# jorgeMFS/HYMET

Hardware: AMD Instinct MI355X
Metric: contigs/s + Mbp/s classified, CAMI-medium, 1/2/4/8 MI355X; % HBM roofline (higher is better)
Workload: dtype u64

## Files before the change

hymet_amd/_lib.py:

```python
from __future__ import annotations

import ctypes
import os

HERE = os.path.dirname(os.path.abspath(__file__))
LIB_PATH = os.path.join(HERE, "libhymet_gpu.so")

_c = ctypes
_i64, _u64, _i32, _u32, _vp = _c.c_int64, _c.c_uint64, _c.c_int, _c.c_uint32, _c.c_void_p

_SIGS = {
    "hymet_version": (_i32, []),
    "hymet_init": (_i32, [_i32, _c.POINTER(_vp)]),
    "hymet_destroy": (_i32, [_vp]),
    "hymet_last_error": (_c.c_char_p, []),
    "hymet_set_stream": (_i32, [_vp, _vp]),
    "hymet_sync": (_i32, [_vp]),
    "hymet_prof_enable": (_i32, [_vp, _i32]),
    "hymet_prof_reset": (_i32, [_vp]),
    "hymet_prof_query": (_i32, [_vp, _c.c_char_p, _c.POINTER(_c.c_double), _c.POINTER(_i64), _c.POINTER(_c.c_double)]),
    "hymet_prof_names": (_i32, [_vp, _c.c_char_p, _i64]),
    "hymet_scratch_trim": (_i32, [_vp, _c.POINTER(_i64)]),
    "hymet_scratch_cached": (_i32, [_vp, _c.POINTER(_i64)]),
    "hymet_scratch_stats": (_i32, [_vp, _vp]),
    "hymet_scratch_reserve": (_i32, [_vp, _i64]),
    "hymet_set_oom_hook": (_i32, [_vp, _vp]),
    "hymet_copy_to_host": (_i32, [_vp, _vp, _vp, _i64, _i32]),
    "hymet_copy_to_device": (_i32, [_vp, _vp, _vp, _i64, _i32]),
    "hymet_pack": (_i32, [_vp, _vp, _i64, _i32, _vp, _vp]),
    "hymet_fasta_index": (_i32, [_vp, _i64, _i32, _i64, _c.POINTER(_i64), _vp, _vp, _vp, _vp, _vp]),
    "hymet_fasta_names": (_i32, [_vp, _vp, _vp, _i64, _vp, _vp]),
    "hymet_fasta_compact": (_i32, [_vp, _vp, _i64, _i64, _vp, _vp, _vp, _i64, _vp, _i64, _vp]),
    "hymet_name_hash": (_i32, [_vp, _vp, _vp, _vp, _i64, _vp]),
    "hymet_sort_pairs_u64": (_i32, [_vp, _vp, _vp, _i64, _i32, _i32]),
    "hymet_scan_u32": (_i32, [_vp, _vp, _vp, _i64, _i32, _vp]),
    "hymet_msh_open": (_i32, [_c.c_char_p, _c.POINTER(_vp)]),
    "hymet_msh_info_get": (_i32, [_vp, _vp]),
    "hymet_msh_copy": (_i32, [_vp, _i32, _vp, _vp, _vp, _vp, _vp, _vp]),
    "hymet_msh_upload": (_i32, [_vp, _vp, _i32, _vp, _vp, _i32]),
    "hymet_msh_upload_range": (_i32, [_vp, _vp, _i32, _vp, _vp, _i32, _i64, _i64]),
    "hymet_msh_text_offsets": (_i32, [_vp, _vp, _vp]),
    "hymet_msh_close": (None, [_vp]),
    "hymet_screen_table_slots": (_i64, [_i64]),
    "hymet_screen_table_build": (_i32, [_vp, _vp, _i64, _vp, _i64, _vp, _vp, _i32]),
    "hymet_screen_count": (_i32, [_vp, _vp, _vp, _i64, _i64, _i64, _i32, _u32, _i32, _c.POINTER(_vp), _c.POINTER(_i64),
                                  _c.POINTER(_vp), _c.POINTER(_i64), _c.POINTER(_vp), _u64, _vp, _i64, _vp, _vp]),
    "hymet_screen_stats": (_i32, [_vp, _vp, _i64, _vp, _vp, _vp, _vp]),
    "hymet_screen_winner": (_i32, [_vp, _vp, _i64, _vp, _vp, _i64, _vp, _i64, _vp, _vp, _vp]),
    "hymet_sketch_max_size": (_i64, []),
    "hymet_sketch_batch": (_i32, [_vp, _vp, _vp, _i64, _i32, _u32, _i32, _i64, _vp, _vp, _vp, _i32, _vp, _vp]),
    "hymet_mash_dist": (_i32, [_vp, _vp, _i64, _vp, _i64, _vp, _i64, _vp, _i64, _i64, _i64, _i32, _vp]),
    "hymet_mash_dist_tile": (_i32, [_i32]),
    "hymet_mash_dist_tune": (_i32, [_i32, _i32]),
    "hymet_mash_dist_select": (_i32, [_vp, _vp, _i64, _i64, _vp, _i32, _vp, _vp, _vp, _i64, _c.POINTER(_i64)]),
    "hymet_mash_dist_tri": (_i32, [_vp, _vp, _i64, _vp, _i64, _i64, _i64, _i32, _vp]),
    "hymet_mash_link": (_i32, [_vp, _vp, _i64, _i64, _i64, _vp, _i32, _vp, _vp]),
    "hymet_mash_labels": (_i32, [_vp, _vp, _i64, _vp]),
    "hymet_mash_dist_sparse": (_i32, [_vp, _vp, _i64, _vp, _i64, _vp, _i64, _vp, _i64, _i64, _i64, _i32, _i32, _vp, _i32,
                                      _i64, _vp, _vp, _vp, _i64, _c.POINTER(_i64), _vp]),
    "hymet_mash_link_edges": (_i32, [_vp, _vp, _i64, _i64, _vp, _vp, _vp]),
    "hymet_mm_sketch": (_i32, [_vp, _vp, _vp, _vp, _vp, _i32, _i32, _i32, _i32, _vp, _vp, _i64, _c.POINTER(_i64)]),
    "hymet_mm_index_build": (_i32, [_vp, _vp, _vp, _vp, _vp, _i32, _i32, _i32, _c.POINTER(_vp)]),
    "hymet_mm_index_destroy": (_i32, [_vp]),
    "hymet_mm_index_info": (_i32, [_vp, _c.POINTER(_i32), _c.POINTER(_i32), _c.POINTER(_i32), _c.POINTER(_i64)]),
    "hymet_mm_index_max_occ": (_i32, [_vp, _vp, _c.c_float, _c.POINTER(_i32)]),
    "hymet_mm_index_save": (_i32, [_vp, _vp, _c.c_char_p, _i32, _c.POINTER(_i64)]),
    "hymet_mm_index_load": (_i32, [_vp, _c.c_char_p, _i64, _c.POINTER(_vp), _c.POINTER(_i64)]),
    "hymet_mm_index_export": (_i32, [_vp, _vp, _vp, _vp]),
    "hymet_mm_map": (_i32, [_vp, _vp, _vp, _vp, _vp, _vp, _vp, _vp, _i32, _c.POINTER(_vp)]),
    "hymet_mm_result_size": (_i32, [_vp, _c.POINTER(_i64)]),
    "hymet_mm_result_copy": (_i32, [_vp, _vp, _vp, _vp]),
    "hymet_mm_result_destroy": (_i32, [_vp]),
    "hymet_paf_acc_create": (_i32, [_vp, _c.POINTER(_vp)]),
    "hymet_paf_acc_reset": (_i32, [_vp]),
    "hymet_paf_acc_destroy": (_i32, [_vp]),
    "hymet_paf_acc_info": (_i32, [_vp, _c.POINTER(_i64), _c.POINTER(_vp), _c.POINTER(_vp), _c.POINTER(_vp),
                                  _c.POINTER(_vp), _c.POINTER(_vp)]),
    "hymet_paf_acc_append": (_i32, [_vp, _vp, _vp, _i64, _i64]),
    "hymet_paf_acc_copy": (_i32, [_vp, _vp, _vp, _vp, _vp]),
    "hymet_paf_acc_field": (_i32, [_vp, _vp, _i32, _vp]),
    "hymet_mm_map_acc": (_i32, [_vp, _vp, _vp, _vp, _vp, _vp, _vp, _vp, _i32, _i32, _i32, _i32, _vp]),
    "hymet_emit_paf": (_i32, [_vp, _vp, _vp, _vp, _vp, _vp, _vp, _vp, _vp, _i64, _c.POINTER(_i64), _vp]),
    "hymet_acc_ref_counts": (_i32, [_vp, _vp, _vp]),
    "hymet_acc_classify": (_i32, [_vp, _vp, _i32, _i32] + [_vp] * 15 + [_c.POINTER(_i32)]),
    "hymet_emit_tsv": (_i32, [_vp, _i32, _i32] + [_vp] * 14 + [_i64, _c.POINTER(_i64)]),
    "hymet_mm_chain_dp": (_i32, [_vp, _vp, _vp, _i64, _i32, _i32, _i32, _i32, _i32, _c.c_float, _c.c_float, _vp, _vp]),
    "hymet_mm_mark_compact": (_i32, [_vp, _vp, _vp, _vp, _i64, _vp, _vp, _i32, _vp, _vp, _vp, _c.POINTER(_i64)]),
    "hymet_mm_stamp_scratch": (_i32, [_vp, _c.POINTER(_i64), _c.POINTER(_i64)]),
    "hymet_mm_anchor_sort": (_i32, [_vp, _vp, _vp, _i64, _vp, _i32, _i32, _i32, _u64, _i64, _vp, _vp, _vp, _vp, _vp]),
    "hymet_lca_ref_counts": (_i32, [_vp, _vp, _i64, _vp]),
    "hymet_lca": (_i32, [_vp, _i32, _i32] + [_vp] * 17),
}

class SparseCounters(_c.Structure):
    _fields_ = [("postings", _i64), ("emitted", _i64), ("candidates", _i64)]


_lib = None
_oom_hook = None


def _release_torch_cache(_user):
    try:
        import torch
        torch.cuda.empty_cache()
    except Exception:
        pass


class HymetError(RuntimeError):
    pass


def load():
    global _lib
    if _lib is not None:
        return _lib
    path = os.environ.get("HYMET_LIB", LIB_PATH)
    if not os.path.exists(path):
        raise HymetError(f"{path} not found: build the HIP extension (python -m hymet_amd.build); "
                         "hymet_amd has no CPU fallback")
    lib = ctypes.CDLL(path)
    for name, (res, args) in _SIGS.items():
        fn = getattr(lib, name)
        fn.restype = res
        fn.argtypes = args
    global _oom_hook
    _oom_hook = _c.CFUNCTYPE(None, _vp)(_release_torch_cache)
    lib.hymet_set_oom_hook(_c.cast(_oom_hook, _vp), None)
    _lib = lib
    return lib


def exported_symbols():
    return list(_SIGS)


def check(rc: int, what: str):
    if rc != 0:
        msg = load().hymet_last_error()
        raise HymetError(f"{what} failed ({rc}): {msg.decode() if msg else ''}")


class Gpu:

    def __init__(self, device: int = 0, stream=None):
        import torch

        if not torch.cuda.is_available():
            raise HymetError("no GPU visible: hymet_amd runs on MI355X (gfx950) only")
        self.torch = torch
        self.device = device
        torch.cuda.set_device(device)
        self.dev = torch.device("cuda", device)
        self.lib = load()
        h = _vp()
        check(self.lib.hymet_init(device, _c.byref(h)), "hymet_init")
        self.ctx = h
        self.stream = stream
        self.children = []
        self.bind_stream(stream)

    def fork(self) -> "Gpu":
        child = Gpu(self.device, stream=self.torch.cuda.Stream(device=self.device))
        self.children.append(child)
        return child

    def bind_stream(self, stream=None):
        s = stream if stream is not None else self.torch.cuda.current_stream(self.device)
        check(self.lib.hymet_set_stream(self.ctx, _vp(s.cuda_stream)), "hymet_set_stream")
        self.bound_stream = s

    def call(self, name, *args):
        check(getattr(self.lib, name)(self.ctx, *args), name)

    def sync(self):
        check(self.lib.hymet_sync(self.ctx), "hymet_sync")
        for ch in self.children:
            ch.sync()

    def prof(self, on: bool = True):
        check(self.lib.hymet_prof_enable(self.ctx, int(on)), "hymet_prof_enable")
        for ch in self.children:
            ch.prof(on)

    def prof_reset(self):
        check(self.lib.hymet_prof_reset(self.ctx), "hymet_prof_reset")
        for ch in self.children:
            ch.prof_reset()

    def prof_table(self):
        buf = _c.create_string_buffer(1 << 16)
        check(self.lib.hymet_prof_names(self.ctx, buf, 1 << 16), "hymet_prof_names")
        out = {}
        for name in buf.value.decode().split():
            ms, n, b = _c.c_double(), _i64(), _c.c_double()
            check(self.lib.hymet_prof_query(self.ctx, name.encode(), _c.byref(ms), _c.byref(n), _c.byref(b)), "hymet_prof_query")
            out[name] = (ms.value, n.value, b.value)
        for ch in self.children:
            for name, (ms, n, b) in ch.prof_table().items():
                m0, n0, b0 = out.get(name, (0.0, 0, 0.0))
                out[name] = (m0 + ms, n0 + n, b0 + b)
        return out

    def trim(self) -> int:
        out = _i64()
        check(self.lib.hymet_scratch_trim(self.ctx, _c.byref(out)), "hymet_scratch_trim")
        return out.value

    def reserve(self, nbytes: int):
        check(self.lib.hymet_scratch_reserve(self.ctx, int(nbytes)), "hymet_scratch_reserve")

    def _alloc(self, fn, n, dtype):
        try:
            return fn(int(n), dtype=dtype, device=self.dev)
        except self.torch.OutOfMemoryError:
            if self.trim() == 0:
                raise
            return fn(int(n), dtype=dtype, device=self.dev)

    def empty(self, n, dtype):
        return self._alloc(self.torch.empty, n, dtype)

    def zeros(self, n, dtype):
        return self._alloc(self.torch.zeros, n, dtype)

    def close(self):
        if self.ctx:
            self.lib.hymet_destroy(self.ctx)
            self.ctx = None

    def __del__(self):
        try:
            self.close()
        except Exception:
            pass


def ptr(t) -> _vp:
    return _vp(t.data_ptr())
```

hymet_amd/csrc/mm_map.hip:

```cpp
#include "mm_stages.hpp"

#include <algorithm>
#include <atomic>
#include <type_traits>
#include <utility>

#include <chrono>
#include <cstdio>
#include <cstdlib>
#include <cstring>

struct hymet_mm_result {
    int n_q = 0;
    std::vector<int64_t> reg_off;
    std::vector<int32_t> rep_len;
    std::vector<hymet_mm_reg> regs;
};

namespace hymet {
namespace mm {

int launch_regions(hymet_ctx *ctx, const uint64_t *ax, const uint32_t *ay, int span, const int32_t *ids, const int64_t *cfirst,
                   const uint64_t *cu, const int64_t *cboff,
                   const int64_t *qc, const int64_t *qb, const uint64_t *mini_pos, const int64_t *mp_off, const int64_t *qlen,
                   const uint32_t *name_hash, const int32_t *rep_len, const int64_t *ref_len, int n_q, const hymet_mm_opt *o,
                   int k, void *z, hymet_mm_reg *regs, int32_t *w, uint64_t *cov, int32_t *tmp, int32_t *n_regs,
                   int64_t NB, int64_t NC, int64_t NM, const uint32_t *cq,
                   const MiniWord *mtab, const int64_t *qbase, const uint32_t *skip_q, uint64_t *sumk, bool sumk_done);

namespace {

__global__ void fill_qid_kernel(const int64_t *off, int n_q, int64_t n, uint32_t *qid, uint32_t *ones, int32_t *zq) {
    const int64_t i = (int64_t)blockIdx.x * blockDim.x + threadIdx.x;
    if (i < n) {
        qid[i] = (uint32_t)upper_idx(off, n_q, i);
        if (ones) ones[i] = 1u;
    }
    if (zq && i < n_q) zq[i] = 0;
}

__global__ void flagged_len_kernel(const uint32_t *flag, const int64_t *qb, int n_q, uint32_t *cnt, int64_t *any) {
    const int q = blockIdx.x * blockDim.x + threadIdx.x;
    if (q > n_q) return;
    if (q == n_q) {
        cnt[q] = 0;
        return;
    }
    const bool f = flag[q] != 0;
    cnt[q] = f ? (uint32_t)(qb[q + 1] - qb[q]) : 0u;
    if (f) *any = 1;
}


__global__ void mzflt_runs_kernel(const uint32_t *sq, const uint64_t *sx, const uint32_t *sidx, const int64_t *qm_off,
                                  int64_t n, int q_occ_max, float q_occ_frac, uint32_t *keep) {
    const int64_t p = (int64_t)blockIdx.x * blockDim.x + threadIdx.x;
    if (p >= n) return;
    if (p > 0 && sq[p] == sq[p - 1] && sx[p] == sx[p - 1]) return;
    int64_t e = p + 1;
    while (e < n && sq[e] == sq[p] && sx[e] == sx[p]) e++;
    const uint32_t q = sq[p];
    const int64_t nq = qm_off[q + 1] - qm_off[q];
    if (nq <= q_occ_max) return;
    const int32_t cnt = (int32_t)(e - p);
    if (cnt > q_occ_max && (float)cnt > (float)nq * q_occ_frac)
        for (int64_t j = p; j < e; j++) keep[sidx[j]] = 0;
}

constexpr int kMzBuckets = 4096;
__global__ __launch_bounds__(256) void mzflt_screen_kernel(const uint64_t *mx, const int64_t *qm_off, int n_q, int q_occ_max,
                                                           uint32_t *keep, uint32_t *cnt, int64_t *any) {
    __shared__ uint32_t h[kMzBuckets];
    __shared__ int hit;
    const int q = blockIdx.x;
    if (q == n_q) {
        if (threadIdx.x == 0) cnt[q] = 0;
        return;
    }
    const int64_t s = qm_off[q], nq = qm_off[q + 1] - s;
    for (int64_t e = threadIdx.x; e < nq; e += 256) keep[s + e] = 1u;
    if (nq <= q_occ_max) {
        if (threadIdx.x == 0) cnt[q] = 0;
        return;
    }
    for (int b = threadIdx.x; b < kMzBuckets; b += 256) h[b] = 0;
    if (threadIdx.x == 0) hit = 0;
    __syncthreads();
    bool over = false;
    for (int64_t e = threadIdx.x; e < nq; e += 256)
        over |= atomicAdd(&h[(uint32_t)(mx[s + e] >> 8) & (kMzBuckets - 1)], 1u) >= (uint32_t)q_occ_max;
    if (over) hit = 1;
    __syncthreads();
    if (threadIdx.x == 0) {
        cnt[q] = hit ? (uint32_t)nq : 0u;
        if (hit) *any = 1;
    }
}

__global__ __launch_bounds__(256) void mzflt_list_kernel(const int64_t *qm_off, const uint32_t *cnt, const int64_t *coff,
                                                         uint32_t *gidx, uint32_t *sq) {
    const int q = blockIdx.x;
    const uint32_t nq = cnt[q];
    if (nq == 0) return;
    const int64_t s = qm_off[q], d = coff[q];
    for (uint32_t e = threadIdx.x; e < nq; e += 256) {
        gidx[d + e] = (uint32_t)(s + e);
        sq[d + e] = (uint32_t)q;
    }
}

__global__ void mzflt_gather_kernel(const uint32_t *perm, const uint32_t *gidx, const uint64_t *mx, uint32_t *gout,
                                    uint64_t *xout, int64_t n) {
    const int64_t i = (int64_t)blockIdx.x * blockDim.x + threadIdx.x;
    if (i >= n) return;
    const uint32_t g = gidx[perm[i]];
    gout[i] = g;
    xout[i] = mx[g];
}

__global__ void compact_mz_kernel(const uint64_t *x, const uint64_t *y, const uint32_t *keep, int64_t *pos, int64_t n,
                                  uint64_t *ox, uint64_t *oy) {
    const int64_t i = (int64_t)blockIdx.x * blockDim.x + threadIdx.x;
    if (i == n - 1) pos[n] = pos[i] + keep[i];
    if (i < n && keep[i]) {
        ox[pos[i]] = x[i];
        oy[pos[i]] = y[i];
    }
}

__global__ void sample_off_kernel(const int64_t *pos, const int64_t *qm_off, int n_q, int64_t total, int64_t *out) {
    const int q = blockIdx.x * blockDim.x + threadIdx.x;
    if (q > n_q) return;
    out[q] = q == n_q ? total : pos[qm_off[q]];
}

__global__ void seed_count_kernel(const uint64_t *mx, int64_t n, const uint32_t *koff, int64_t n_buckets,
                                  uint32_t *seed_n) {
    const int64_t i = (int64_t)blockIdx.x * blockDim.x + threadIdx.x;
    if (i >= n) return;
    const uint64_t h = mx[i] >> 8;
    uint32_t c = 0;
    if ((int64_t)h < n_buckets) c = koff[h + 1] - koff[h];
    seed_n[i] = c;
}

constexpr uint32_t kFlt = 0x80000000u;

__global__ void seed_class_kernel(const uint32_t *seed_n, int64_t M, int max_occ, uint64_t *cls) {
    const int64_t i = (int64_t)blockIdx.x * blockDim.x + threadIdx.x;
    if (i > M) return;
    if (i == M) {
        cls[M] = 0;
        return;
    }
    const uint32_t n = seed_n[i];
    const bool hi = (int)n > max_occ, lo = n > 0 && !hi;
    cls[i] = (uint64_t)(hi ? 1u : 0u) << 32 | (lo ? 1u : 0u);
}

__global__ void seed_list_kernel(const uint32_t *seed_n, const uint64_t *rank, int64_t M, int max_occ, int32_t *low_idx,
                                 int32_t *high_idx) {
    const int64_t i = (int64_t)blockIdx.x * blockDim.x + threadIdx.x;
    if (i >= M) return;
    const uint32_t n = seed_n[i];
    if (!n) return;
    if ((int)n > max_occ) high_idx[rank[i] >> 32] = (int32_t)i;
    else low_idx[(uint32_t)rank[i]] = (int32_t)i;
}

struct StreakParams {
    const uint64_t *my;
    const uint32_t *qid;
    const int64_t *qm_off, *qlen;
    const uint64_t *rank;
    const int32_t *low_idx, *high_idx;
    int64_t n_low;
    int n_q;
    int max_occ, max_max_occ, dist;
    uint32_t *seed_n;
    uint32_t *flt_high;
};

__global__ void streak_kernel(StreakParams P) {
    const int64_t t = (int64_t)blockIdx.x * blockDim.x + threadIdx.x;
    if (t >= P.n_low + P.n_q) return;
    int q;
    int64_t e_idx = -1, p_idx = -1;
    uint64_t re, rp;
    if (t < P.n_low) {
        e_idx = P.low_idx[t];
        q = (int)P.qid[e_idx];
        re = P.rank[e_idx];
        if (t > 0 && P.qid[P.low_idx[t - 1]] == (uint32_t)q) p_idx = P.low_idx[t - 1];
    } else {
        q = (int)(t - P.n_low);
        re = P.rank[P.qm_off[q + 1]];
        const uint64_t r0 = P.rank[P.qm_off[q]];
        if ((uint32_t)re > (uint32_t)r0) p_idx = P.low_idx[(uint32_t)re - 1];
    }
    rp = p_idx >= 0 ? P.rank[p_idx] : P.rank[P.qm_off[q]];
    const int64_t h0 = (int64_t)(rp >> 32), h1 = (int64_t)(re >> 32);
    const int cnt = (int)(h1 - h0);
    if (cnt <= 0) return;
    const bool case_a = P.dist > 0 && P.max_max_occ > P.max_occ;
    bool keep_all = false, keep_none = false;
    uint64_t thr = 0;
    if (case_a) {
        const uint64_t rq0 = P.rank[P.qm_off[q]], rq1 = P.rank[P.qm_off[q + 1]];
        const int64_t n_seed = (int64_t)((uint32_t)rq1 - (uint32_t)rq0) + (int64_t)((rq1 >> 32) - (rq0 >> 32));
        if (n_seed <= 1) return;
        const int32_t ps = p_idx >= 0 ? (int32_t)((uint32_t)P.my[p_idx] >> 1) : 0;
        const int32_t pe = e_idx >= 0 ? (int32_t)((uint32_t)P.my[e_idx] >> 1) : (int32_t)P.qlen[q];
        int32_t mh = (int32_t)((double)(pe - ps) / P.dist + .499);
        if (mh > 128) mh = 128;
        keep_all = mh >= cnt, keep_none = mh <= 0;
        if (!keep_all && !keep_none) {
            uint64_t lo = 0, hi = ~0ull;
            while (lo < hi) {
                const uint64_t mid = lo + (hi - lo) / 2;
                int c = 0;
                for (int64_t r = h0; r < h1; r++) {
                    const int32_t a = P.high_idx[r];
                    c += ((uint64_t)P.seed_n[a] << 32 | (uint32_t)a) <= mid;
                }
                if (c >= mh) hi = mid;
                else lo = mid + 1;
            }
            thr = lo;
        }
    }
    for (int64_t r = h0; r < h1; r++) {
        const int32_t a = P.high_idx[r];
        const uint32_t n = P.seed_n[a];
        bool flt = true;
        if (case_a) {
            const bool chosen = keep_all || (!keep_none && ((uint64_t)n << 32 | (uint32_t)a) <= thr);
            flt = !chosen || (int)n > P.max_max_occ;
        }
        P.flt_high[r] = flt ? 1u : 0u;
    }
}

__global__ void flt_mark_kernel(const uint32_t *flt_high, int64_t n_high, int32_t *v) {
    const int64_t r = (int64_t)blockIdx.x * blockDim.x + threadIdx.x;
    if (r < n_high) v[r] = flt_high[r] ? (int32_t)r : -1;
}

__global__ void rep_len_kernel(const uint32_t *flt_high, const int32_t *prev_max, const int32_t *high_idx, int64_t n_high,
                               const uint64_t *mx, const uint64_t *my, const uint32_t *qid, int32_t *rep_len,
                               uint32_t *seed_n) {
    const int64_t r = (int64_t)blockIdx.x * blockDim.x + threadIdx.x;
    if (r >= n_high || !flt_high[r]) return;
    const int32_t a = high_idx[r];
    const uint32_t q = qid[a];
    const int32_t en = (int32_t)((uint32_t)my[a] >> 1) + 1, st = en - (int32_t)(mx[a] & 0xff);
    int32_t en_prev = 0;
    const int32_t pr = r > 0 ? prev_max[r - 1] : -1;
    if (pr >= 0) {
        const int32_t b = high_idx[pr];
        if (qid[b] == q) en_prev = (int32_t)((uint32_t)my[b] >> 1) + 1;
    }
    atomicAdd(rep_len + q, en - max(st, en_prev));
    seed_n[a] = 0;
}

__global__ void nz_flag_kernel(const uint32_t *v, int64_t n, uint32_t *flag) {
    const int64_t i = (int64_t)blockIdx.x * blockDim.x + threadIdx.x;
    if (i < n) flag[i] = v[i] ? 1u : 0u;
}

struct AnchorParams {
    const uint64_t *mx, *my;
    const uint32_t *seed_n;
    const int64_t *a_pos;
    const uint32_t *qid;
    const int64_t *qlen;
    const uint32_t *koff;
    const uint64_t *ipos;
    int64_t n;
    int rb;
    uint64_t *ax, *k1, *k2;
    uint32_t *ay;
    uint32_t *val;
    const int64_t *mp_pos;
    uint64_t *mini_pos;
};

__global__ void write_anchors_kernel(AnchorParams P) {
    const int64_t i = (int64_t)blockIdx.x * blockDim.x + threadIdx.x;
    if (i >= P.n) return;
    const uint32_t n = P.seed_n[i];
    if (!n) return;
    const uint64_t mx = P.mx[i], my = P.my[i];
    const uint32_t q_pos = (uint32_t)my, q_span = (uint32_t)(mx & 0xff);
    P.mini_pos[P.mp_pos[i]] = (uint64_t)q_span << 32 | (q_pos >> 1);
    const uint32_t q = P.qid[i];
    const int32_t qlen = (int32_t)P.qlen[q];
    const uint32_t *kp = P.koff + (mx >> 8);
    const uint64_t *r = P.ipos + kp[0];
    int64_t a = P.a_pos[i];
    for (uint32_t k = 0; k < n; k++, a++) {
        const uint64_t rk = r[k];
        const uint32_t rpos = (uint32_t)rk >> 1;
        const uint32_t rid = (uint32_t)(rk >> 32);
        uint64_t x, y;
        uint32_t rev;
        if ((rk & 1) == (q_pos & 1)) {
            rev = 0;
            x = (rk & 0xffffffff00000000ULL) | rpos;
            y = (uint64_t)q_span << 32 | (q_pos >> 1);
        } else {
            rev = 1;
            x = 1ULL << 63 | (rk & 0xffffffff00000000ULL) | rpos;
            y = (uint64_t)q_span << 32 | (uint32_t)(qlen - (int32_t)((q_pos >> 1) + 1 - q_span) - 1);
        }
        P.ax[a] = x;
        P.ay[a] = (uint32_t)y;
        P.k1[a] = (uint64_t)q << (1 + P.rb) | (uint64_t)rev << P.rb | rid;
        P.k2[a] = (uint64_t)rpos << 32 | (uint32_t)y;
        P.val[a] = (uint32_t)a;
    }
}

struct AnchorKeyParams {
    const uint64_t *mx, *my;
    const uint32_t *seed_n;
    const int64_t *a_pos;
    const uint32_t *qid;
    const int64_t *qlen;
    const uint32_t *koff;
    const uint64_t *ipos;
    int64_t n;
    int rb, pb;
    int ybits;
    uint64_t *key;
    const int64_t *mp_pos;
    uint64_t *mini_pos;
};

__global__ __launch_bounds__(256) void write_anchor_keys_kernel(AnchorKeyParams P) {
    __shared__ int64_t s_a[257];
    __shared__ uint64_t s_r[256];
    __shared__ uint32_t s_yf[256], s_yr[256], s_strand[256];
    const int tid = threadIdx.x;
    const int64_t m0 = (int64_t)blockIdx.x * 256;
    const int cnt = (int)min((int64_t)256, P.n - m0);
    if (tid < cnt) {
        const int64_t i = m0 + tid;
        const uint32_t n = P.seed_n[i];
        const uint64_t mx = P.mx[i], my = P.my[i];
        const uint32_t q_pos = (uint32_t)my, q_span = (uint32_t)(mx & 0xff);
        const uint32_t q = P.qid[i];
        if (n) P.mini_pos[P.mp_pos[i]] = (uint64_t)q_span << 32 | (q_pos >> 1);
        s_a[tid] = P.a_pos[i];
        s_r[tid] = P.koff[mx >> 8];
        s_yf[tid] = q_pos >> 1;
        s_yr[tid] = (uint32_t)((int32_t)P.qlen[q] - (int32_t)((q_pos >> 1) + 1 - q_span) - 1);
        s_strand[tid] = q_pos & 1;
    }
    if (tid == 0) s_a[cnt] = P.a_pos[m0 + cnt];
    __syncthreads();
    const int64_t a0 = s_a[0], a1 = s_a[cnt];
    const int sh_rev = P.rb + P.pb;
    for (int64_t a = a0 + tid; a < a1; a += 256) {
        int lo = 0, hi = cnt - 1;
        while (lo < hi) {
            const int mid = (lo + hi + 1) >> 1;
            if (s_a[mid] <= a) lo = mid;
            else hi = mid - 1;
        }
        const uint64_t rk = P.ipos[s_r[lo] + (a - s_a[lo])];
        const uint32_t rpos = (uint32_t)rk >> 1;
        const uint64_t rid = rk >> 32;
        const uint32_t rev = ((uint32_t)rk & 1) != s_strand[lo];
        const uint64_t k = (uint64_t)rev << sh_rev | rid << P.pb | rpos;
        const uint32_t y = rev ? s_yr[lo] : s_yf[lo];
        P.key[a] = k << P.ybits | y;
    }
}

__global__ __launch_bounds__(256) void mini_bits_kernel(const uint64_t *my, const uint32_t *seed_n, const uint32_t *qid,
                                                        const int64_t *qbase, int64_t M, MiniWord *tab) {
    const int64_t i = (int64_t)blockIdx.x * blockDim.x + threadIdx.x;
    const int lane = threadIdx.x & 63;
    const bool on = i < M && seed_n[i];
    const int64_t b = on ? qbase[qid[i]] + ((uint32_t)my[i] >> 1) : -64 * (int64_t)(lane + 1);
    const int64_t w = b >> 6;
    uint64_t bits = on ? 1ull << (b & 63) : 0;
#pragma unroll
    for (int d = 1; d < 64; d <<= 1) {
        const int64_t wo = __shfl_down(w, d, 64);
        const uint64_t bo = __shfl_down(bits, d, 64);
        if (lane + d < 64 && wo == w) bits |= bo;
    }
    const int64_t wp = __shfl_up(w, 1, 64);
    if (on && (lane == 0 || wp != w)) atomicOr((unsigned long long *)&tab[w].bits, bits);
}
__global__ void mini_base_kernel(const uint64_t *my, const uint32_t *seed_n, const uint32_t *qid, const int64_t *qm_off,
                                 const int64_t *mp_pos, const int64_t *qbase, int64_t M, MiniWord *tab) {
    const int64_t i = (int64_t)blockIdx.x * blockDim.x + threadIdx.x;
    if (i >= M || !seed_n[i]) return;
    const uint32_t q = qid[i];
    const int64_t b = qbase[q] + ((uint32_t)my[i] >> 1);
    const uint64_t bits = tab[b >> 6].bits;
    tab[b >> 6].base = (uint32_t)(mp_pos[i] - mp_pos[qm_off[q]]) - (uint32_t)__popcll(bits & ((1ull << (b & 63)) - 1));
}

__global__ void reg_count_kernel(const uint32_t *flag, const int32_t *n1, const int32_t *n2, int n_q, uint32_t *cnt) {
    const int q = blockIdx.x * blockDim.x + threadIdx.x;
    if (q < n_q) cnt[q] = (uint32_t)((flag && flag[q]) ? n2[q] : n1[q]);
}

struct RegOut {
    hymet_mm_reg *regs;
    int32_t *q, *part, *rl, *t;
    int32_t q_base, part_id, t_base;
};
__global__ void reg_gather_kernel(const uint32_t *flag, const int32_t *n1, const int32_t *n2, const int64_t *qc1,
                                  const int64_t *qc2, const hymet_mm_reg *r1, const hymet_mm_reg *r2, const int64_t *off,
                                  const int32_t *rep_len, int n_q, RegOut o) {
    const int q = blockIdx.x * blockDim.x + threadIdx.x;
    if (q >= n_q) return;
    const bool use2 = flag && flag[q];
    const hymet_mm_reg *src = use2 ? r2 + qc2[q] : r1 + qc1[q];
    const int nr = use2 ? n2[q] : n1[q];
    const int64_t d = off[q];
    for (int i = 0; i < nr; i++) {
        const hymet_mm_reg r = src[i];
        o.regs[d + i] = r;
        if (o.q) {
            o.q[d + i] = o.q_base + q;
            o.part[d + i] = o.part_id;
            o.rl[d + i] = rep_len[q];
            o.t[d + i] = o.t_base + r.rid;
        }
    }
}
}
}
}

using namespace hymet;
using namespace hymet::mm;

struct CallTrace {
    bool on = env_flag("HYMET_TRACE");
    std::chrono::steady_clock::time_point t = std::chrono::steady_clock::now();
    ~CallTrace() {
        if (on)
            fprintf(stderr, "[hymet_mm_map] %-22s %9.2f ms\n", "TOTAL (with frees)",
                    std::chrono::duration<double, std::milli>(std::chrono::steady_clock::now() - t).count());
    }
};
struct PhaseTrace {
    hymet_ctx *ctx;
    bool on;
    std::chrono::steady_clock::time_point t;
    explicit PhaseTrace(hymet_ctx *c) : ctx(c), on(env_flag("HYMET_TRACE")), t(std::chrono::steady_clock::now()) {}
    void mark(const char *what) {
        if (!on) return;
        (void)hipStreamSynchronize(ctx->stream);
        const auto n = std::chrono::steady_clock::now();
        fprintf(stderr, "[hymet_mm_map] %-22s %9.2f ms\n", what, std::chrono::duration<double, std::milli>(n - t).count());
        t = n;
    }
};

static int sort_anchor_set(hymet_ctx *ctx, DevBuf &x, DevBuf &y, DevBuf &k1, DevBuf &k2, DevBuf &val, int64_t n,
                           int key1_bits, int yhi, AnchorSet &out) {
    DevBuf k2b, valb, k1g, k1b;
    HY_HIP(k2b.alloc(8 * (size_t)n, ctx->stream));
    HY_HIP(valb.alloc(4 * (size_t)n, ctx->stream));
    uint64_t *kk = k2.as<uint64_t>(), *kka = k2b.as<uint64_t>();
    uint32_t *vv = val.as<uint32_t>(), *vva = valb.as<uint32_t>();
    int rc = sort_pairs(ctx, kk, kka, vv, vva, n, 0, 64, "radix_sort_anchor_pos");
    if (rc) return rc;
    HY_HIP(k1g.alloc(8 * (size_t)n, ctx->stream));
    HY_HIP(k1b.alloc(8 * (size_t)n, ctx->stream));
    LAUNCH1(gather_kernel<uint64_t>, n, k1.as<uint64_t>(), vv, k1g.as<uint64_t>(), n);
    uint64_t *k1p = k1g.as<uint64_t>(), *k1a = k1b.as<uint64_t>();
    rc = sort_pairs(ctx, k1p, k1a, vv, vva, n, 0, key1_bits, "radix_sort_anchor_group");
    if (rc) return rc;
    HY_HIP(out.ax.alloc(8 * (size_t)n, ctx->stream));
    HY_HIP(out.ay.alloc(4 * (size_t)n, ctx->stream));
    LAUNCH1(gather_kernel<uint64_t>, n, x.as<uint64_t>(), vv, out.ax.as<uint64_t>(), n);
    LAUNCH1(gather_kernel<uint32_t>, n, y.as<uint32_t>(), vv, out.ay.as<uint32_t>(), n);
    out.n = n;
    out.span = yhi & 0xff;
    return HYMET_OK;
}

static int sort_anchor_words(hymet_ctx *ctx, DevBuf &word, int64_t n, int rb, int pb, int yhi, const int64_t *d_qoff, int n_q,
                             int64_t max_qlen, AnchorSet &out) {
    DevBuf wb;
    HY_HIP(wb.alloc(8 * (size_t)n, ctx->stream));
    HY_HIP(out.ax.alloc(8 * (size_t)n, ctx->stream));
    HY_HIP(out.ay.alloc(4 * (size_t)n, ctx->stream));
    HY_HIP(out.hb.alloc(head_bits_bytes(n), ctx->stream));
    HY_HIP(out.ax32.alloc(4 * (size_t)n, ctx->stream));
    out.n = n;
    out.span = yhi & 0xff;
    const bool log_stats = env_flag("HYMET_ASORT_STATS");
    DevBuf sstat;
    if (log_stats) {
        HY_HIP(sstat.alloc(32, ctx->stream));
        HY_HIP(hipMemsetAsync(sstat.p, 0, 32, ctx->stream));
    }
    const int rc = grouped_anchor_sort(ctx, word.as<uint64_t>(), n, d_qoff, n_q, rb, pb, max_qlen,
                                       wb.as<uint64_t>(), out.ax.as<uint64_t>(), out.ay.as<uint32_t>(),
                                       out.hb.as<uint32_t>(), out.ax32.as<uint32_t>(),
                                       log_stats ? sstat.as<unsigned long long>() : nullptr);
    if (rc == 1) return hymet::fail(HYMET_E_INTERNAL, "sort_anchor_words: anchor words emitted for a layout without one");
    if (rc) return rc;
    if (log_stats) {
        unsigned long long h[4] = {};
        HY_HIP(hipMemcpyAsync(h, sstat.p, 32, hipMemcpyDeviceToHost, ctx->stream));
        HY_HIP(hipStreamSynchronize(ctx->stream));
        fprintf(stderr, "[asort] anchors %lld fast_segs %llu fast_anchors %llu full_segs %llu full_anchors %llu\n",
                (long long)n, h[0], h[1], h[2], h[3]);
    }
    out.has_hb = out.has_x32 = true;
    return HYMET_OK;
}

static int dump_anchors(hymet_ctx *ctx, const char *var, const AnchorSet &S, int n_q, std::atomic<bool> &dumped) {
    const char *path = env_str(var);
    if (!path || S.n == 0 || dumped.exchange(true)) return HYMET_OK;
    hipStream_t st = ctx->stream;
    const int64_t nd = std::min<int64_t>(S.n, env_int("HYMET_DUMP_MAX", 1 << 24, 0, INT64_MAX));
    std::vector<uint64_t> hx(nd);
    std::vector<uint32_t> hy(nd);
    std::vector<int64_t> qo(n_q + 1);
    HY_HIP(hipMemcpyAsync(hx.data(), S.ax.p, 8 * (size_t)nd, hipMemcpyDeviceToHost, st));
    HY_HIP(hipMemcpyAsync(hy.data(), S.ay.p, 4 * (size_t)nd, hipMemcpyDeviceToHost, st));
    HY_HIP(hipMemcpyAsync(qo.data(), S.d_off.p, 8 * (size_t)(n_q + 1), hipMemcpyDeviceToHost, st));
    HY_HIP(hipStreamSynchronize(st));
    if (FILE *fp = fopen(path, "wb")) {
        uint64_t gid = 0;
        int q = 0;
        std::vector<uint64_t> buf;
        buf.reserve(1 << 21);
        for (int64_t a = 0; a < nd; a++) {
            bool qs = false;
            while (q < n_q && qo[q + 1] <= a) q++, qs = true;
            if (a && (qs || (hx[a] >> 32) != (hx[a - 1] >> 32))) gid++;
            buf.push_back(gid << 32 | (uint32_t)hx[a]);
            buf.push_back((uint64_t)S.span << 32 | hy[a]);
            if (buf.size() >= (1u << 21)) fwrite(buf.data(), 8, buf.size(), fp), buf.clear();
        }
        fwrite(buf.data(), 8, buf.size(), fp);
        fclose(fp);
    }
    return HYMET_OK;
}

struct MapSink {
    hymet_mm_result *res = nullptr;
    hymet_paf_acc *acc = nullptr;
    int32_t q_base = 0, part_id = 0, t_base = 0;
};

static int acc_reserve(hymet_ctx *ctx, hymet_paf_acc *a, int64_t need) {
    if (need <= a->cap) return HYMET_OK;
    const int64_t cap = std::max<int64_t>(need, std::max<int64_t>(a->cap * 3 / 2, 1 << 16));
    hipStream_t st = ctx->stream;
    DevBuf nregs, nq, npart, nrl, nt;
    HY_HIP(nregs.alloc(sizeof(hymet_mm_reg) * (size_t)cap, st));
    HY_HIP(nq.alloc(4 * (size_t)cap, st));
    HY_HIP(npart.alloc(4 * (size_t)cap, st));
    HY_HIP(nrl.alloc(4 * (size_t)cap, st));
    HY_HIP(nt.alloc(4 * (size_t)cap, st));
    if (a->n) {
        HY_HIP(hipMemcpyAsync(nregs.p, a->regs.p, sizeof(hymet_mm_reg) * (size_t)a->n, hipMemcpyDeviceToDevice, st));
        HY_HIP(hipMemcpyAsync(nq.p, a->q.p, 4 * (size_t)a->n, hipMemcpyDeviceToDevice, st));
        HY_HIP(hipMemcpyAsync(npart.p, a->part.p, 4 * (size_t)a->n, hipMemcpyDeviceToDevice, st));
        HY_HIP(hipMemcpyAsync(nrl.p, a->rl.p, 4 * (size_t)a->n, hipMemcpyDeviceToDevice, st));
        HY_HIP(hipMemcpyAsync(nt.p, a->t.p, 4 * (size_t)a->n, hipMemcpyDeviceToDevice, st));
    }
    a->regs.swap(nregs);
    a->q.swap(nq);
    a->part.swap(npart);
    a->rl.swap(nrl);
    a->t.swap(nt);
    a->cap = cap;
    return HYMET_OK;
}

struct MapBatch {
    hymet_ctx *ctx;
    const hymet_mm_index *idx;
    const hymet_mm_opt *opt;
    const int64_t *h_lens;
    int32_t n_q;
    DevBuf mx, my, qm_off;
    int64_t M = 0;
    DevBuf d_qlen, d_hash_buf;
    const uint32_t *d_hash = nullptr;
    DevBuf seed_n, rep_len, qid;
    DevBuf mini_pos, mp_off;
    int64_t NM = 0;
    DevBuf d_qbase, pos_tab;
    std::vector<int64_t> qbase;
    int64_t max_qlen = 1;
};

static int sketch_queries(MapBatch &B, const uint32_t *d_2b, const uint32_t *d_mask, const int64_t *h_starts,
                          const uint32_t *h_name_hash, const uint32_t *d_name_hash) {
    hipStream_t st = B.ctx->stream;
    const int n_q = B.n_q;
    int rc = sketch_sequences(B.ctx, d_2b, d_mask, h_starts, B.h_lens, n_q, B.idx->w, B.idx->k, 0, B.mx, B.my, &B.M, &B.qm_off);
    if (rc) return rc;
    HY_HIP(B.d_qlen.alloc(8 * (size_t)n_q, st));
    HY_HIP(hipMemcpyAsync(B.d_qlen.p, B.h_lens, 8 * (size_t)n_q, hipMemcpyHostToDevice, st));
    B.d_hash = d_name_hash;
    if (!B.d_hash) {
        HY_HIP(B.d_hash_buf.alloc(4 * (size_t)n_q, st));
        HY_HIP(hipMemcpyAsync(B.d_hash_buf.p, h_name_hash, 4 * (size_t)n_q, hipMemcpyHostToDevice, st));
        B.d_hash = B.d_hash_buf.as<uint32_t>();
    }
    return HYMET_OK;
}

static int filter_minimizers(MapBatch &B) {
    hymet_ctx *ctx = B.ctx;
    hipStream_t st = ctx->stream;
    const hymet_mm_opt *opt = B.opt;
    const int n_q = B.n_q;
    const int64_t M = B.M;
    DevBuf &mx = B.mx, &my = B.my, &qm_off = B.qm_off;
    DevBuf keep, fcnt, fcoff;
    int64_t MF = 0;
    int rc;
    if (opt->q_occ_frac > 0.0f && M > 0 && opt->mid_occ > 0) {
        HY_HIP(keep.alloc(4 * (size_t)M, st));
        HY_HIP(fcnt.alloc(4 * (size_t)(n_q + 1), st));
        ctx->mbox_h[kMbFlag] = 0;
        hipLaunchKernelGGL(mzflt_screen_kernel, dim3((unsigned)n_q + 1), dim3(256), 0, st, mx.as<uint64_t>(), qm_off.as<int64_t>(),
                           n_q, opt->mid_occ, keep.as<uint32_t>(), fcnt.as<uint32_t>(), mb_dev(ctx, kMbFlag));
        HY_CHECK_LAUNCH("mzflt_screen_kernel");
        HY_HIP(hipStreamSynchronize(st));
        if (mb_read(ctx, kMbFlag) != 0) {
            HY_HIP(fcoff.alloc(8 * (size_t)(n_q + 1), st));
            rc = exclusive_scan_u32_i64(ctx, fcnt.as<uint32_t>(), fcoff.as<int64_t>(), n_q + 1, &MF);
            if (rc) return rc;
        }
    }
    if (MF == 0) return HYMET_OK;
    DevBuf gidx, sx, sx2, sidx, sidx2, sq0, sq, sq2, kpos, nx, ny, gx, gg;
    HY_HIP(gidx.alloc(4 * (size_t)MF, st));
    HY_HIP(sq0.alloc(4 * (size_t)MF, st));
    hipLaunchKernelGGL(mzflt_list_kernel, dim3((unsigned)n_q), dim3(256), 0, st, qm_off.as<int64_t>(), fcnt.as<uint32_t>(),
                       fcoff.as<int64_t>(), gidx.as<uint32_t>(), sq0.as<uint32_t>());
    HY_CHECK_LAUNCH("mzflt_list_kernel");
    HY_HIP(sx.alloc(8 * (size_t)MF, st));
    HY_HIP(sx2.alloc(8 * (size_t)MF, st));
    HY_HIP(sidx.alloc(4 * (size_t)MF, st));
    HY_HIP(sidx2.alloc(4 * (size_t)MF, st));
    LAUNCH1(gather_kernel<uint64_t>, MF, mx.as<uint64_t>(), gidx.as<uint32_t>(), sx.as<uint64_t>(), MF);
    LAUNCH1(iota_u32_kernel, MF, sidx.as<uint32_t>(), MF);
    uint64_t *kx = sx.as<uint64_t>(), *kxa = sx2.as<uint64_t>();
    uint32_t *vi = sidx.as<uint32_t>(), *via = sidx2.as<uint32_t>();
    rc = sort_pairs(ctx, kx, kxa, vi, via, MF, 0, 2 * B.idx->k + 8, "radix_sort_mz");
    if (rc) return rc;
    HY_HIP(sq.alloc(4 * (size_t)MF, st));
    HY_HIP(sq2.alloc(4 * (size_t)MF, st));
    LAUNCH1(gather_kernel<uint32_t>, MF, sq0.as<uint32_t>(), vi, sq.as<uint32_t>(), MF);
    uint32_t *kq = sq.as<uint32_t>(), *kqa = sq2.as<uint32_t>();
    rc = sort_pairs(ctx, kq, kqa, vi, via, MF, 0, bits_for(n_q), "radix_sort_mz");
    if (rc) return rc;
    HY_HIP(gx.alloc(8 * (size_t)MF, st));
    HY_HIP(gg.alloc(4 * (size_t)MF, st));
    LAUNCH1(mzflt_gather_kernel, MF, vi, gidx.as<uint32_t>(), mx.as<uint64_t>(), gg.as<uint32_t>(), gx.as<uint64_t>(), MF);
    LAUNCH1(mzflt_runs_kernel, MF, kq, gx.as<uint64_t>(), gg.as<uint32_t>(), qm_off.as<int64_t>(), MF, opt->mid_occ,
            opt->q_occ_frac, keep.as<uint32_t>());
    int64_t M2 = 0;
    rc = scan_flags(ctx, keep.as<uint32_t>(), M, kpos, &M2);
    if (rc) return rc;
    HY_HIP(nx.alloc(8 * (size_t)(M2 + 1), st));
    HY_HIP(ny.alloc(8 * (size_t)(M2 + 1), st));
    LAUNCH1(compact_mz_kernel, M, mx.as<uint64_t>(), my.as<uint64_t>(), keep.as<uint32_t>(), kpos.as<int64_t>(), M,
            nx.as<uint64_t>(), ny.as<uint64_t>());
    DevBuf nqm;
    HY_HIP(nqm.alloc(8 * (size_t)(n_q + 1), st));
    hipLaunchKernelGGL(sample_off_kernel, dim3((unsigned)cdiv(n_q + 1, 256)), dim3(256), 0, st, kpos.as<int64_t>(),
                       qm_off.as<int64_t>(), n_q, M2, nqm.as<int64_t>());
    HY_CHECK_LAUNCH("sample_off_kernel");
    mx.swap(nx);
    my.swap(ny);
    qm_off.swap(nqm);
    B.M = M2;
    return HYMET_OK;
}

static int select_seeds(MapBatch &B) {
    hymet_ctx *ctx = B.ctx;
    hipStream_t st = ctx->stream;
    const hymet_mm_opt *opt = B.opt;
    const int n_q = B.n_q;
    const int64_t M = B.M;
    DevBuf &mx = B.mx, &my = B.my, &qm_off = B.qm_off, &seed_n = B.seed_n, &rep_len = B.rep_len, &qid = B.qid;
    HY_HIP(seed_n.alloc(4 * (size_t)(M + 1), st));
    HY_HIP(rep_len.alloc(4 * (size_t)n_q, st));
    HY_HIP(qid.alloc(4 * (size_t)(M + 1), st));
    LAUNCH1(fill_qid_kernel, std::max<int64_t>(M, n_q), qm_off.as<int64_t>(), n_q, M, qid.as<uint32_t>(), nullptr,
            rep_len.as<int32_t>());
    {
        ProfScope _ps(ctx, "mm_seed_count", (double)M * (8.0 + 8.0 + 4.0));
        LAUNCH1(seed_count_kernel, M, mx.as<uint64_t>(), M, B.idx->d_koff, B.idx->n_buckets, seed_n.as<uint32_t>());
    }
    if (M == 0) return HYMET_OK;
    ProfScope _ps(ctx, "mm_seed_select", (double)M * (4.0 + 8.0 + 8.0 + 8.0));
    DevBuf cls, rank, spart;
    HY_HIP(cls.alloc(8 * (size_t)(M + 1), st));
    HY_HIP(rank.alloc(8 * (size_t)(M + 1), st));
    LAUNCH1(seed_class_kernel, M + 1, seed_n.as<uint32_t>(), M, opt->mid_occ, cls.as<uint64_t>());
    int rc = scan_u64(ctx, cls.as<uint64_t>(), rank.as<uint64_t>(), M + 1, spart, mb_dev(ctx, kMbScan));
    if (rc) return rc;
    HY_HIP(hipStreamSynchronize(st));
    const uint64_t tot = (uint64_t)mb_read(ctx, kMbScan);
    const int64_t n_low = (uint32_t)tot, n_high = (int64_t)(tot >> 32);
    if (n_high == 0) return HYMET_OK;
    DevBuf low_idx, high_idx, flt_high, vmax, pmax;
    HY_HIP(low_idx.alloc(4 * (size_t)(n_low + 1), st));
    HY_HIP(high_idx.alloc(4 * (size_t)n_high, st));
    HY_HIP(flt_high.alloc(4 * (size_t)n_high, st));
    LAUNCH1(seed_list_kernel, M, seed_n.as<uint32_t>(), rank.as<uint64_t>(), M, opt->mid_occ, low_idx.as<int32_t>(),
            high_idx.as<int32_t>());
    StreakParams S{my.as<uint64_t>(), qid.as<uint32_t>(), qm_off.as<int64_t>(), B.d_qlen.as<int64_t>(),
                   rank.as<uint64_t>(), low_idx.as<int32_t>(), high_idx.as<int32_t>(), n_low, n_q, opt->mid_occ,
                   opt->max_max_occ, opt->occ_dist, seed_n.as<uint32_t>(), flt_high.as<uint32_t>()};
    HY_HIP(hipMemsetAsync(flt_high.p, 0, 4 * (size_t)n_high, st));
    LAUNCH1(streak_kernel, n_low + n_q, S);
    HY_HIP(vmax.alloc(4 * (size_t)n_high, st));
    HY_HIP(pmax.alloc(4 * (size_t)n_high, st));
    LAUNCH1(flt_mark_kernel, n_high, flt_high.as<uint32_t>(), n_high, vmax.as<int32_t>());
    {
        DevBuf mpart;
        rc = inclusive_max_scan_i32(ctx, vmax.as<int32_t>(), pmax.as<int32_t>(), n_high, mpart);
        if (rc) return rc;
    }
    LAUNCH1(rep_len_kernel, n_high, flt_high.as<uint32_t>(), pmax.as<int32_t>(), high_idx.as<int32_t>(), n_high,
            mx.as<uint64_t>(), my.as<uint64_t>(), qid.as<uint32_t>(), rep_len.as<int32_t>(), seed_n.as<uint32_t>());
    return HYMET_OK;
}

static int build_mini_table(MapBatch &B, const DevBuf &mp_pos) {
    hymet_ctx *ctx = B.ctx;
    hipStream_t st = ctx->stream;
    const int n_q = B.n_q;
    B.qbase.assign(n_q + 1, 0);
    for (int q = 0; q < n_q; q++) {
        B.qbase[q + 1] = B.qbase[q] + ((B.h_lens[q] + 63) & ~(int64_t)63);
        B.max_qlen = std::max<int64_t>(B.max_qlen, B.h_lens[q]);
    }
    HY_HIP(B.d_qbase.alloc(8 * (size_t)(n_q + 1), st));
    HY_HIP(hipMemcpyAsync(B.d_qbase.p, B.qbase.data(), 8 * (size_t)(n_q + 1), hipMemcpyHostToDevice, st));
    const size_t n_words = (size_t)(B.qbase[n_q] >> 6) + 1;
    HY_HIP(B.pos_tab.alloc(sizeof(MiniWord) * n_words, st));
    HY_HIP(hipMemsetAsync(B.pos_tab.p, 0, sizeof(MiniWord) * n_words, st));
    LAUNCH1(mini_bits_kernel, B.M, B.my.as<uint64_t>(), B.seed_n.as<uint32_t>(), B.qid.as<uint32_t>(), B.d_qbase.as<int64_t>(),
            B.M, B.pos_tab.as<MiniWord>());
    LAUNCH1(mini_base_kernel, B.M, B.my.as<uint64_t>(), B.seed_n.as<uint32_t>(), B.qid.as<uint32_t>(), B.qm_off.as<int64_t>(),
            mp_pos.as<int64_t>(), B.d_qbase.as<int64_t>(), B.M, B.pos_tab.as<MiniWord>());
    return HYMET_OK;
}

static int first_pass_anchors(MapBatch &B, AnchorSet &S1) {
    hymet_ctx *ctx = B.ctx;
    hipStream_t st = ctx->stream;
    const hymet_mm_index *idx = B.idx;
    const int n_q = B.n_q;
    const int64_t M = B.M;
    DevBuf &mx = B.mx, &my = B.my, &qm_off = B.qm_off, &seed_n = B.seed_n, &qid = B.qid, &d_qlen = B.d_qlen;
    DevBuf a_pos, mflag, mp_pos;
    int64_t A = 0;
    int rc = scan_flags(ctx, seed_n.as<uint32_t>(), M, a_pos, &A);
    if (rc) return rc;
    HY_ARG(A <= anchor_cap(), "hymet_mm_map: the batch has more anchors than 32-bit chain links hold (map fewer bases per batch)");
    HY_HIP(mflag.alloc(4 * (size_t)(M + 1), st));
    LAUNCH1(nz_flag_kernel, M, seed_n.as<uint32_t>(), M, mflag.as<uint32_t>());
    rc = scan_flags(ctx, mflag.as<uint32_t>(), M, mp_pos, &B.NM);
    if (rc) return rc;
    HY_HIP(hipMemcpyAsync(a_pos.as<int64_t>() + M, &A, 8, hipMemcpyHostToDevice, st));
    HY_HIP(hipMemcpyAsync(mp_pos.as<int64_t>() + M, &B.NM, 8, hipMemcpyHostToDevice, st));
    HY_HIP(B.mini_pos.alloc(8 * (size_t)(B.NM + 1), st));
    HY_HIP(B.mp_off.alloc(8 * (size_t)(n_q + 1), st));
    hipLaunchKernelGGL(sample_off_kernel, dim3((unsigned)cdiv(n_q + 1, 256)), dim3(256), 0, st, mp_pos.as<int64_t>(),
                       qm_off.as<int64_t>(), n_q, B.NM, B.mp_off.as<int64_t>());
    HY_CHECK_LAUNCH("sample_off_kernel");
    rc = build_mini_table(B, mp_pos);
    if (rc) return rc;
    HY_HIP(S1.d_off.alloc(8 * (size_t)(n_q + 1), st));
    hipLaunchKernelGGL(sample_off_kernel, dim3((unsigned)cdiv(n_q + 1, 256)), dim3(256), 0, st, a_pos.as<int64_t>(),
                       qm_off.as<int64_t>(), n_q, A, S1.d_off.as<int64_t>());
    HY_CHECK_LAUNCH("sample_off_kernel");
    const int rb = bits_for(idx->n_seq), key1_bits = bits_for(n_q) + 1 + rb;
    HY_ARG(key1_bits <= 64, "hymet_mm_map: too many queries x targets for the sort key");
    int64_t max_len = 1;
    for (int64_t l : idx->h_len) max_len = std::max(max_len, l);
    const int pb = bits_for(max_len - 1);
    if (A == 0) {
        S1.span = idx->k & 0xff;
        return HYMET_OK;
    }
    const int ybits = env_flag("HYMET_ANCHOR_LEGACY") ? 0 : anchor_word_ybits(rb, pb, B.max_qlen);
    if (ybits > 0) {
        DevBuf word;
        HY_HIP(word.alloc(8 * (size_t)(A + 1), st));
        AnchorKeyParams P{mx.as<uint64_t>(), my.as<uint64_t>(), seed_n.as<uint32_t>(), a_pos.as<int64_t>(),
                          qid.as<uint32_t>(), d_qlen.as<int64_t>(), idx->d_koff, idx->d_pos, M, rb, pb,
                          ybits, word.as<uint64_t>(), mp_pos.as<int64_t>(), B.mini_pos.as<uint64_t>()};
        {
            ProfScope _ps(ctx, "mm_anchors", (double)A * (8.0 + 12.0));
            hipLaunchKernelGGL(write_anchor_keys_kernel, dim3((unsigned)cdiv(M, 256)), dim3(256), 0, st, P);
            HY_CHECK_LAUNCH("write_anchor_keys_kernel");
        }
        return sort_anchor_words(ctx, word, A, rb, pb, idx->k, S1.d_off.as<int64_t>(), n_q, B.max_qlen, S1);
    }
    DevBuf x, y, k1, k2, val;
    HY_HIP(x.alloc(8 * (size_t)(A + 1), st));
    HY_HIP(y.alloc(4 * (size_t)(A + 1), st));
    HY_HIP(k1.alloc(8 * (size_t)(A + 1), st));
    HY_HIP(k2.alloc(8 * (size_t)(A + 1), st));
    HY_HIP(val.alloc(4 * (size_t)(A + 1), st));
    AnchorParams P{mx.as<uint64_t>(), my.as<uint64_t>(), seed_n.as<uint32_t>(), a_pos.as<int64_t>(), qid.as<uint32_t>(),
                   d_qlen.as<int64_t>(), idx->d_koff, idx->d_pos, M, rb, x.as<uint64_t>(), k1.as<uint64_t>(),
                   k2.as<uint64_t>(), y.as<uint32_t>(), val.as<uint32_t>(), mp_pos.as<int64_t>(), B.mini_pos.as<uint64_t>()};
    ProfScope _ps(ctx, "mm_anchors", (double)A * (8.0 + 36.0));
    LAUNCH1(write_anchors_kernel, M, P);
    return sort_anchor_set(ctx, x, y, k1, k2, val, A, key1_bits, idx->k, S1);
}

static int long_join_anchors(MapBatch &B, const AnchorSet &S1, const LeanJoin &lj, const DevBuf &flag, AnchorSet &S2,
                             bool &any) {
    hymet_ctx *ctx = B.ctx;
    const int n_q = B.n_q;
    DevBuf fcnt;
    HY_HIP(fcnt.alloc(4 * (size_t)(n_q + 1), ctx->stream));
    ctx->mbox_h[kMbFlag] = 0;
    LAUNCH1(flagged_len_kernel, n_q + 1, flag.as<uint32_t>(), lj.qb2.as<int64_t>(), n_q, fcnt.as<uint32_t>(),
            mb_dev(ctx, kMbFlag));
    int64_t A2 = 0;
    int rc = scan_flags(ctx, fcnt.as<uint32_t>(), n_q + 1, S2.d_off, &A2);
    if (rc) return rc;
    any = mb_read(ctx, kMbFlag) != 0;
    if (!any) return HYMET_OK;
    HY_ARG(A2 <= anchor_cap(), "hymet_mm_map: the long join has more anchors than 32-bit chain links hold");
    rc = marked_anchor_set(ctx, S1, lj, flag.as<uint32_t>(), n_q, A2, S2);
    if (rc) return rc;
    static std::atomic<bool> dumped{false};
    return dump_anchors(ctx, "HYMET_DUMP_ANCHORS2", S2, n_q, dumped);
}

static int run_regions(MapBatch &B, ChainSet &C, DevBuf &rg, DevBuf &nr, const uint32_t *skip_q, DevBuf &sumk, bool &sumk_done) {
    hipStream_t st = B.ctx->stream;
    const int64_t NC = C.n_chain;
    DevBuf z, wv, cov, tmp;
    HY_HIP(z.alloc(16 * (size_t)(NC + 1), st));
    HY_HIP(rg.alloc(sizeof(hymet_mm_reg) * (size_t)(NC + 1), st));
    HY_HIP(wv.alloc(4 * (size_t)(NC + 1), st));
    HY_HIP(cov.alloc(8 * (size_t)(NC + 1), st));
    HY_HIP(tmp.alloc(4 * (size_t)(NC + 1), st));
    HY_HIP(nr.alloc(4 * (size_t)B.n_q, st));
    return launch_regions(B.ctx, C.ax, C.ay, C.span, C.ids.as<int32_t>(), C.cfirst.as<int64_t>(), C.cu.as<uint64_t>(),
                          C.cboff.as<int64_t>(), C.d_qc.as<int64_t>(), C.d_qb.as<int64_t>(), B.mini_pos.as<uint64_t>(),
                          B.mp_off.as<int64_t>(), B.d_qlen.as<int64_t>(), B.d_hash, B.rep_len.as<int32_t>(), B.idx->d_len,
                          B.n_q, B.opt, B.idx->k, z.p, rg.as<hymet_mm_reg>(), wv.as<int32_t>(), cov.as<uint64_t>(),
                          tmp.as<int32_t>(), nr.as<int32_t>(), C.n_anchor, NC, B.NM, C.cq.as<uint32_t>(),
                          B.pos_tab.as<MiniWord>(), B.d_qbase.as<int64_t>(), skip_q, sumk.as<uint64_t>(),
                          std::exchange(sumk_done, true));
}

struct RegSet {
    const int32_t *n;
    const int64_t *qc;
    const hymet_mm_reg *r;
};

static int emit_records(MapBatch &B, const uint32_t *fl, const RegSet &s1, const RegSet &s2, MapSink &sink) {
    hymet_ctx *ctx = B.ctx;
    hipStream_t st = ctx->stream;
    const int n_q = B.n_q;
    hymet_mm_result *res = sink.res;
    DevBuf cnt, off;
    HY_HIP(cnt.alloc(4 * (size_t)(n_q + 1), st));
    LAUNCH1(reg_count_kernel, n_q, fl, s1.n, s2.n, n_q, cnt.as<uint32_t>());
    int64_t N = 0;
    int rc = scan_flags(ctx, cnt.as<uint32_t>(), n_q, off, &N);
    if (rc) return rc;
    HY_HIP(hipMemcpyAsync(off.as<int64_t>() + n_q, &N, 8, hipMemcpyHostToDevice, st));
    RegOut o{};
    DevBuf tmp_regs;
    if (sink.acc) {
        hymet_paf_acc *a = sink.acc;
        rc = acc_reserve(ctx, a, a->n + N);
        if (rc) return rc;
        o = RegOut{a->regs.as<hymet_mm_reg>() + a->n, a->q.as<int32_t>() + a->n, a->part.as<int32_t>() + a->n,
                   a->rl.as<int32_t>() + a->n, a->t.as<int32_t>() + a->n, sink.q_base, sink.part_id, sink.t_base};
    } else {
        HY_HIP(tmp_regs.alloc(sizeof(hymet_mm_reg) * (size_t)(N + 1), st));
        o.regs = tmp_regs.as<hymet_mm_reg>();
    }
    {
        ProfScope _ps(ctx, "mm_paf_records", (double)N * (2.0 * sizeof(hymet_mm_reg) + 16.0));
        LAUNCH1(reg_gather_kernel, n_q, fl, s1.n, s2.n, s1.qc, s2.qc, s1.r, s2.r, off.as<int64_t>(), B.rep_len.as<int32_t>(),
                n_q, o);
    }
    if (sink.acc) {
        sink.acc->n += N;
    } else {
        res->regs.resize(N);
        if (N) HY_HIP(hipMemcpyAsync(res->regs.data(), tmp_regs.p, sizeof(hymet_mm_reg) * (size_t)N, hipMemcpyDeviceToHost, st));
        HY_HIP(hipMemcpyAsync(res->reg_off.data(), off.p, 8 * (size_t)(n_q + 1), hipMemcpyDeviceToHost, st));
        HY_HIP(hipMemcpyAsync(res->rep_len.data(), B.rep_len.p, 4 * (size_t)n_q, hipMemcpyDeviceToHost, st));
    }
    HY_HIP(hipStreamSynchronize(st));
    return HYMET_OK;
}

static int mm_map_impl(hymet_ctx *ctx, const hymet_mm_index *idx, const hymet_mm_opt *opt, const uint32_t *d_2b,
                       const uint32_t *d_mask, const int64_t *h_starts, const int64_t *h_lens, const uint32_t *h_name_hash,
                       const uint32_t *d_name_hash, int32_t n_q, MapSink &sink) {
    CallTrace call_trace;
    HY_ARG(ctx && idx && opt && d_2b && d_mask, "hymet_mm_map: null argument");
    HY_ARG(n_q >= 0, "hymet_mm_map: n_q < 0");
    HY_ARG(h_name_hash || d_name_hash, "hymet_mm_map: no query name hashes");
    HY_ARG(opt->mid_occ > 0, "hymet_mm_map: opt->mid_occ must be resolved (hymet_mm_index_max_occ + clamps)");
    HY_HIP(hipSetDevice(ctx->device));
    if (sink.res) {
        sink.res->n_q = n_q;
        sink.res->reg_off.assign(n_q + 1, 0);
        sink.res->rep_len.assign(n_q, 0);
    }
    if (n_q == 0) return HYMET_OK;
    const float pen_gap = (float)(opt->chain_gap_scale * 0.01 * idx->k);
    const float pen_skip = (float)(opt->chain_skip_scale * 0.01 * idx->k);
    PhaseTrace tr(ctx);
    MapBatch B{ctx, idx, opt, h_lens, n_q};
    int rc = sketch_queries(B, d_2b, d_mask, h_starts, h_name_hash, d_name_hash);
    if (rc) return rc;
    tr.mark("sketch");
    rc = filter_minimizers(B);
    if (rc) return rc;
    tr.mark("mz_flt");
    rc = select_seeds(B);
    if (rc) return rc;
    tr.mark("seeds");
    AnchorSet S1;
    rc = first_pass_anchors(B, S1);
    if (rc) return rc;
    tr.mark("anchors+sort");
    static std::atomic<bool> dumped1{false};
    rc = dump_anchors(ctx, "HYMET_DUMP_ANCHORS", S1, n_q, dumped1);
    if (rc) return rc;
    ChainSet C1;
    const bool long_join = opt->bw_long > opt->bw;
    LeanJoin lj{B.d_qlen.as<int64_t>(), opt->rmq_rescue_size, opt->rmq_rescue_ratio};
    rc = chain_set(ctx, opt, pen_gap, pen_skip, opt->bw, S1, n_q, C1, long_join ? &lj : nullptr);
    if (rc) return rc;
    tr.mark("chain_set 1");
    ChainSet C2;
    AnchorSet S2;
    DevBuf flag;
    bool joined = false;
    if (long_join && C1.n_chain > 0) {
        flag.swap(lj.flag);
        rc = long_join_anchors(B, S1, lj, flag, S2, joined);
        if (rc) return rc;
        if (joined) {
            rc = chain_set(ctx, opt, pen_gap, pen_skip, opt->bw_long, S2, n_q, C2);
            if (rc) return rc;
        }
    }
    tr.mark("long join");
    DevBuf sumk, rg1, nr1, rg2, nr2;
    HY_HIP(sumk.alloc(8 * (size_t)(n_q + 1), ctx->stream));
    bool sumk_done = false;
    const uint32_t *fl = joined ? flag.as<uint32_t>() : nullptr;
    rc = run_regions(B, C1, rg1, nr1, fl, sumk, sumk_done);
    if (rc) return rc;
    if (joined) {
        rc = run_regions(B, C2, rg2, nr2, nullptr, sumk, sumk_done);
        if (rc) return rc;
    }
    const RegSet r1{nr1.as<int32_t>(), C1.d_qc.as<int64_t>(), rg1.as<hymet_mm_reg>()};
    const RegSet r2{nr2.as<int32_t>(), C2.d_qc.as<int64_t>(), rg2.as<hymet_mm_reg>()};
    rc = emit_records(B, fl, r1, joined ? r2 : r1, sink);
    if (rc) return rc;
    tr.mark("regions");
    return HYMET_OK;
}

extern "C" {

int hymet_mm_map(hymet_ctx *ctx, const hymet_mm_index *idx, const hymet_mm_opt *opt, const uint32_t *d_2b,
                 const uint32_t *d_mask, const int64_t *h_starts, const int64_t *h_lens, const uint32_t *h_name_hash,
                 int32_t n_q, hymet_mm_result **out) {
    HY_ARG(out != nullptr, "hymet_mm_map: null argument");
    MapSink sink;
    sink.res = new hymet_mm_result();
    *out = sink.res;
    return mm_map_impl(ctx, idx, opt, d_2b, d_mask, h_starts, h_lens, h_name_hash, nullptr, n_q, sink);
}

int hymet_paf_acc_create(hymet_ctx *ctx, hymet_paf_acc **out) {
    HY_ARG(ctx && out, "hymet_paf_acc_create: null argument");
    hymet_paf_acc *a = new hymet_paf_acc();
    a->device = ctx->device;
    *out = a;
    return HYMET_OK;
}

int hymet_paf_acc_reset(hymet_paf_acc *acc) {
    HY_ARG(acc, "hymet_paf_acc_reset: null argument");
    acc->n = 0;
    return HYMET_OK;
}

int hymet_paf_acc_destroy(hymet_paf_acc *acc) {
    if (acc) {
        (void)hipSetDevice(acc->device);
        delete acc;
    }
    return HYMET_OK;
}

int hymet_paf_acc_info(const hymet_paf_acc *acc, int64_t *n_lines, void **d_regs, void **d_q, void **d_part, void **d_rl,
                       void **d_t) {
    HY_ARG(acc && n_lines, "hymet_paf_acc_info: null argument");
    *n_lines = acc->n;
    if (d_regs) *d_regs = acc->regs.p;
    if (d_q) *d_q = acc->q.p;
    if (d_part) *d_part = acc->part.p;
    if (d_rl) *d_rl = acc->rl.p;
    if (d_t) *d_t = acc->t.p;
    return HYMET_OK;
}

int hymet_paf_acc_append(hymet_ctx *ctx, hymet_paf_acc *dst, const hymet_paf_acc *src, int64_t begin, int64_t end) {
    HY_ARG(ctx && dst && src && dst != src, "hymet_paf_acc_append: null or aliased argument");
    HY_ARG(begin >= 0 && end >= begin && end <= src->n, "hymet_paf_acc_append: line range outside the source");
    const int64_t m = end - begin;
    if (m == 0) return HYMET_OK;
    HY_HIP(hipSetDevice(ctx->device));
    int rc = acc_reserve(ctx, dst, dst->n + m);
    if (rc) return rc;
    hipStream_t st = ctx->stream;
    const int64_t d = dst->n;
    HY_HIP(hipMemcpyAsync(dst->regs.as<hymet_mm_reg>() + d, src->regs.as<hymet_mm_reg>() + begin, sizeof(hymet_mm_reg) * (size_t)m,
                          hipMemcpyDeviceToDevice, st));
    HY_HIP(hipMemcpyAsync(dst->q.as<int32_t>() + d, src->q.as<int32_t>() + begin, 4 * (size_t)m, hipMemcpyDeviceToDevice, st));
    HY_HIP(hipMemcpyAsync(dst->part.as<int32_t>() + d, src->part.as<int32_t>() + begin, 4 * (size_t)m, hipMemcpyDeviceToDevice,
                          st));
    HY_HIP(hipMemcpyAsync(dst->rl.as<int32_t>() + d, src->rl.as<int32_t>() + begin, 4 * (size_t)m, hipMemcpyDeviceToDevice, st));
    HY_HIP(hipMemcpyAsync(dst->t.as<int32_t>() + d, src->t.as<int32_t>() + begin, 4 * (size_t)m, hipMemcpyDeviceToDevice, st));
    dst->n += m;
    return HYMET_OK;
}

int hymet_paf_acc_copy(hymet_ctx *ctx, const hymet_paf_acc *acc, int32_t *h_q, int32_t *h_part, int32_t *h_t) {
    HY_ARG(ctx && acc, "hymet_paf_acc_copy: null argument");
    if (acc->n <= 0) return HYMET_OK;
    HY_HIP(hipSetDevice(ctx->device));
    hipStream_t st = ctx->stream;
    if (h_q) HY_HIP(hipMemcpyAsync(h_q, acc->q.p, 4 * (size_t)acc->n, hipMemcpyDeviceToHost, st));
    if (h_part) HY_HIP(hipMemcpyAsync(h_part, acc->part.p, 4 * (size_t)acc->n, hipMemcpyDeviceToHost, st));
    if (h_t) HY_HIP(hipMemcpyAsync(h_t, acc->t.p, 4 * (size_t)acc->n, hipMemcpyDeviceToHost, st));
    HY_HIP(hipStreamSynchronize(st));
    return HYMET_OK;
}

int hymet_paf_acc_field(hymet_ctx *ctx, const hymet_paf_acc *acc, int field, int32_t *h_out) {
    HY_ARG(ctx && acc && h_out && field >= 0 && field < (int)(sizeof(hymet_mm_reg) / 4), "hymet_paf_acc_field: bad argument");
    if (acc->n <= 0) return HYMET_OK;
    HY_HIP(hipSetDevice(ctx->device));
    const char *src = static_cast<const char *>(acc->regs.p) + 4 * (size_t)field;
    HY_HIP(hipMemcpy2DAsync(h_out, 4, src, sizeof(hymet_mm_reg), 4, (size_t)acc->n, hipMemcpyDeviceToHost, ctx->stream));
    HY_HIP(hipStreamSynchronize(ctx->stream));
    return HYMET_OK;
}

int hymet_mm_map_acc(hymet_ctx *ctx, const hymet_mm_index *idx, const hymet_mm_opt *opt, const uint32_t *d_2b,
                     const uint32_t *d_mask, const int64_t *h_starts, const int64_t *h_lens, const uint32_t *d_name_hash,
                     int32_t n_q, int32_t q_base, int32_t part_id, int32_t t_base, hymet_paf_acc *acc) {
    HY_ARG(acc && d_name_hash, "hymet_mm_map_acc: null argument");
    MapSink sink;
    sink.acc = acc;
    sink.q_base = q_base;
    sink.part_id = part_id;
    sink.t_base = t_base;
    return mm_map_impl(ctx, idx, opt, d_2b, d_mask, h_starts, h_lens, nullptr, d_name_hash, n_q, sink);
}

int hymet_mm_result_size(const hymet_mm_result *res, int64_t *n_regs) {
    HY_ARG(res && n_regs, "hymet_mm_result_size: null argument");
    *n_regs = (int64_t)res->regs.size();
    return HYMET_OK;
}

int hymet_mm_result_copy(const hymet_mm_result *res, int64_t *h_off, int32_t *h_rep_len, hymet_mm_reg *h_regs) {
    HY_ARG(res, "hymet_mm_result_copy: null result");
    if (h_off) memcpy(h_off, res->reg_off.data(), 8 * (size_t)(res->n_q + 1));
    if (h_rep_len && res->n_q) memcpy(h_rep_len, res->rep_len.data(), 4 * (size_t)res->n_q);
    if (h_regs && !res->regs.empty()) memcpy(h_regs, res->regs.data(), sizeof(hymet_mm_reg) * res->regs.size());
    return HYMET_OK;
}

int hymet_mm_result_destroy(hymet_mm_result *res) {
    delete res;
    return HYMET_OK;
}

}
```

hymet_amd/csrc/mm_regs.hip:

```cpp
#include "mm_common.hpp"

#include <cstdio>
#include <cstdlib>

namespace hymet {
namespace mm {
namespace {

__device__ __forceinline__ uint32_t wang32(uint32_t key) {
    key += ~(key << 15);
    key ^= (key >> 10);
    key += (key << 3);
    key ^= (key >> 6);
    key += ~(key << 11);
    key ^= (key >> 16);
    return key;
}

struct U128 {
    uint64_t x, y;
};
__device__ __forceinline__ bool lt128(const U128 &a, const U128 &b) { return a.x < b.x || (a.x == b.x && a.y < b.y); }

template <typename T, typename Less>
__device__ void heap_sort(T *a, int64_t n, Less less) {
    auto sift = [&](int64_t i, int64_t m) {
        for (;;) {
            int64_t l = 2 * i + 1, r = l + 1, b = i;
            if (l < m && less(a[b], a[l])) b = l;
            if (r < m && less(a[b], a[r])) b = r;
            if (b == i) return;
            T t = a[b];
            a[b] = a[i];
            a[i] = t;
            i = b;
        }
    };
    for (int64_t i = n / 2 - 1; i >= 0; --i) sift(i, n);
    for (int64_t e = n - 1; e > 0; --e) {
        T t = a[0];
        a[0] = a[e];
        a[e] = t;
        sift(0, e);
    }
}

struct RegParams {
    const uint64_t *ax;
    const uint32_t *ay;
    int span;
    const int32_t *ids;
    const int64_t *cfirst;
    const uint64_t *cu;
    const int64_t *cboff;
    const int64_t *qc;
    const int64_t *qb;
    const uint64_t *mini_pos;
    const int64_t *mp_off;
    const int64_t *qlen;
    const uint32_t *name_hash;
    const int32_t *rep_len;
    const int64_t *ref_len;
    int n_q;
    int seed, k;
    float mask_level, pri_ratio;
    int mask_len, best_n, max_gap, min_chain_score;
    U128 *z;
    hymet_mm_reg *regs;
    int32_t *w;
    uint64_t *cov;
    int32_t *tmp;
    int32_t *n_regs;
    const int32_t *c_mlen, *c_blen, *c_st, *c_last, *c_fv;
    const uint64_t *q_sumk;
    const uint32_t *skip_q;
    int wave_min;
    int lds_max;
    unsigned long long *prof;
    int prim_regs;
};

__device__ void set_coor(hymet_mm_reg *r, int32_t qlen, uint64_t x0, uint32_t y0, uint64_t x1, uint32_t y1, int32_t q_span,
                         int32_t mlen, int32_t blen) {
    r->rev = (int32_t)(x0 >> 63);
    r->rid = (int32_t)(x0 << 1 >> 33);
    r->rs = (int32_t)x0 + 1 > q_span ? (int32_t)x0 + 1 - q_span : 0;
    r->re = (int32_t)x1 + 1;
    if (!r->rev) {
        r->qs = (int32_t)y0 + 1 - q_span;
        r->qe = (int32_t)y1 + 1;
    } else {
        r->qs = qlen - ((int32_t)y1 + 1);
        r->qe = qlen - ((int32_t)y0 + 1 - q_span);
    }
    r->mlen = mlen;
    r->blen = blen;
}

struct AnchorStatParams {
    const uint64_t *ax, *cu;
    const uint32_t *ay;
    int span;
    const int32_t *ids;
    const int64_t *cfirst;
    const int64_t *cboff, *qb, *qlen, *mp_off;
    const uint64_t *mini_pos;
    int64_t NB, NC;
    int n_q;
    const uint32_t *cq;
    int32_t *c_mlen, *c_blen, *c_st, *c_last;
    const MiniWord *mtab;
    const int64_t *qbase;
    const uint32_t *skip_q;
};

__device__ __forceinline__ int32_t mini_idx_at(const AnchorStatParams &P, int64_t q, int qlen, uint64_t ax, uint32_t ay) {
    int32_t x = (int32_t)ay;
    if (ax >> 63) x = qlen - 1 - (int32_t)ay + P.span - 1;
    return (x >= 0 && x < qlen) ? mini_word_idx(P.mtab[(P.qbase[q] + x) >> 6], x) : -1;
}

#ifndef HYMET_STAT_ITEMS
#define HYMET_STAT_ITEMS 2
#endif
constexpr int kStatItems = HYMET_STAT_ITEMS;
constexpr int kStatSpan = 256 * kStatItems;

__global__ void block_chain_kernel(const int64_t *cboff, int64_t NC, int64_t NB, int32_t *blk_c0) {
    const int64_t c = (int64_t)blockIdx.x * blockDim.x + threadIdx.x;
    if (c >= NC) return;
    const int64_t s = cboff[c], e = c + 1 < NC ? cboff[c + 1] : NB;
    for (int64_t b = (s + kStatSpan - 1) / kStatSpan; b * kStatSpan < e; ++b) blk_c0[b] = (int32_t)c;
}

__global__ __launch_bounds__(256) void chain_stats_flat_kernel(AnchorStatParams P, const int32_t *blk_c0, int32_t *c_fv) {
    constexpr int K = kStatItems;
    __shared__ int32_t s_st[kStatSpan + 1];
    const int64_t b0 = (int64_t)blockIdx.x * kStatSpan;
    const int64_t cb0 = blk_c0[blockIdx.x];
    for (int i = threadIdx.x; i <= kStatSpan; i += blockDim.x) {
        const int64_t cc = cb0 + i;
        s_st[i] = cc < P.NC ? (int32_t)min(P.cboff[cc] - b0, (int64_t)kStatSpan) : kStatSpan;
    }
    __syncthreads();
    const int lane = threadIdx.x & 63;
    int64_t c[K], q[K], f0[K];
    bool act[K];
    int32_t cnt[K], j[K], qlen[K], cur[K];
    uint64_t x[K];
    uint32_t y[K];
    const bool one_chain = s_st[1] >= kStatSpan;
    int32_t t_dm = 0, t_db = 0, t_fv = INT32_MAX;
    int64_t qb[K];
    if (one_chain) {
        const int64_t qq = (int64_t)P.cq[cb0];
        const int32_t cn = (int32_t)P.cu[cb0];
        const int64_t cbs = P.cboff[cb0], f00 = P.cfirst[cb0] + cn - 1;
        const int ql = (int)P.qlen[qq];
        const int64_t qbb = P.qbase[qq];
        const bool sk = P.skip_q && P.skip_q[qq];
#pragma unroll
        for (int k = 0; k < K; k++) {
            const int64_t b = b0 + 256 * k + threadIdx.x;
            c[k] = b < P.NB ? cb0 : -1;
            q[k] = qq, cnt[k] = cn, f0[k] = f00, qlen[k] = ql, qb[k] = qbb;
            act[k] = b < P.NB && !sk;
            j[k] = act[k] ? (int32_t)(b - cbs) : 0;
        }
    } else {
#pragma unroll
        for (int k = 0; k < K; k++) {
            const int r = 256 * k + (int)threadIdx.x;
            const int64_t b = b0 + r;
            c[k] = -1;
            if (b < P.NB) {
                int lo = 0, hi = kStatSpan;
                while (lo < hi) {
                    const int mid = (lo + hi + 1) >> 1;
                    if (s_st[mid] <= r) lo = mid;
                    else hi = mid - 1;
                }
                c[k] = cb0 + lo;
                if (lo == kStatSpan) {
                    int64_t l2 = c[k], h2 = P.NC - 1;
                    while (l2 < h2) {
                        const int64_t mid = (l2 + h2 + 1) >> 1;
                        if (P.cboff[mid] <= b) l2 = mid;
                        else h2 = mid - 1;
                    }
                    c[k] = l2;
                }
            }
        }
#pragma unroll
        for (int k = 0; k < K; k++) q[k] = (int64_t)P.cq[c[k] >= 0 ? c[k] : 0];
#pragma unroll
        for (int k = 0; k < K; k++) {
            const int64_t cc = c[k] >= 0 ? c[k] : 0;
            cnt[k] = (int32_t)P.cu[cc];
            const int64_t cb = P.cboff[cc];
            f0[k] = P.cfirst[cc] + cnt[k] - 1;
            j[k] = (int32_t)(b0 + 256 * k + threadIdx.x - cb);
            qlen[k] = (int)P.qlen[q[k]];
            qb[k] = P.qbase[q[k]];
        }
#pragma unroll
        for (int k = 0; k < K; k++) {
            act[k] = c[k] >= 0;
            if (P.skip_q) act[k] = act[k] && !P.skip_q[q[k]];
            if (!act[k]) j[k] = 0;
        }
    }
#pragma unroll
    for (int k = 0; k < K; k++) {
        const int64_t a = P.ids[f0[k] - j[k]];
        x[k] = P.ax[a], y[k] = P.ay[a];
    }
#pragma unroll
    for (int k = 0; k < K; k++) {
        int32_t xq = (int32_t)y[k];
        if (x[k] >> 63) xq = qlen[k] - 1 - (int32_t)y[k] + P.span - 1;
        const bool inq = xq >= 0 && xq < qlen[k];
        const int32_t xc = inq ? xq : 0;
        const int32_t v = mini_word_idx(P.mtab[(qb[k] + xc) >> 6], xc);
        cur[k] = act[k] && inq ? v : -1;
    }
#pragma unroll
    for (int k = 0; k < K; k++) {
        const int32_t ci = (int32_t)c[k];
        const int32_t cprev = __shfl_up(ci, 1, 64), cnext = __shfl_down(ci, 1, 64);
        uint64_t xp = __shfl_up(x[k], 1, 64), xn = __shfl_down(x[k], 1, 64);
        uint32_t yp = __shfl_up(y[k], 1, 64), yn = __shfl_down(y[k], 1, 64);
        const int32_t cur_p = __shfl_up(cur[k], 1, 64), cur_n = __shfl_down(cur[k], 1, 64);
        int dm = 0, db = 0, fv = INT32_MAX;
        if (act[k]) {
            const bool rev = x[k] >> 63;
            const bool own_p = lane > 0 && cprev == ci, own_n = lane < 63 && cnext == ci;
            if (j[k] > 0 && !own_p) {
                const int64_t a = P.ids[f0[k] - j[k] + 1];
                xp = P.ax[a], yp = P.ay[a];
            }
            if (rev && j[k] + 1 < cnt[k] && !own_n) {
                const int64_t a = P.ids[f0[k] - j[k] - 1];
                xn = P.ax[a], yn = P.ay[a];
            }
            const int32_t span = P.span;
            if (j[k] == 0) {
                dm = db = span;
            } else {
                const int32_t tl = (int32_t)x[k] - (int32_t)xp;
                const int32_t ql = (int32_t)y[k] - (int32_t)yp;
                db = tl > ql ? tl : ql;
                dm = tl > span && ql > span ? span : tl < ql ? tl : ql;
            }
            const int32_t kk = rev ? cnt[k] - 1 - j[k] : j[k];
            fv = cnt[k];
            if (kk >= 1) {
                const int32_t prev = rev ? (own_n ? cur_n : mini_idx_at(P, q[k], qlen[k], xn, yn))
                                         : (own_p ? cur_p : mini_idx_at(P, q[k], qlen[k], xp, yp));
                if (cur[k] < 0 || cur[k] <= prev) fv = kk;
            }
            if (kk == 0) P.c_st[c[k]] = cur[k];
            if (kk == cnt[k] - 1) P.c_last[c[k]] = cur[k];
        }
        if (one_chain) {
            t_dm += dm, t_db += db, t_fv = min(t_fv, fv);
            continue;
        }
        const int32_t cr = act[k] ? ci : -1;
#pragma unroll
        for (int d = 1; d < 64; d <<= 1) {
            const int32_t co = __shfl_up(cr, d, 64);
            const int dmo = __shfl_up(dm, d, 64), dbo = __shfl_up(db, d, 64), fvo = __shfl_up(fv, d, 64);
            if (lane >= d && co == cr) dm += dmo, db += dbo, fv = min(fv, fvo);
        }
        const int32_t cn = __shfl_down(cr, 1, 64);
        if (act[k] && (lane == 63 || cn != cr)) {
            atomicAdd(P.c_mlen + c[k], dm);
            atomicAdd(P.c_blen + c[k], db);
            atomicMin(c_fv + c[k], fv);
        }
    }
    if (one_chain) {
        __shared__ int32_t r_dm[4], r_db[4], r_fv[4];
#pragma unroll
        for (int o = 32; o > 0; o >>= 1) {
            t_dm += __shfl_xor(t_dm, o, 64);
            t_db += __shfl_xor(t_db, o, 64);
            t_fv = min(t_fv, __shfl_xor(t_fv, o, 64));
        }
        const int w = threadIdx.x >> 6;
        if (lane == 0) r_dm[w] = t_dm, r_db[w] = t_db, r_fv[w] = t_fv;
        __syncthreads();
        if (threadIdx.x == 0 && act[0]) {
            atomicAdd(P.c_mlen + cb0, r_dm[0] + r_dm[1] + r_dm[2] + r_dm[3]);
            atomicAdd(P.c_blen + cb0, r_db[0] + r_db[1] + r_db[2] + r_db[3]);
            atomicMin(c_fv + cb0, min(min(r_fv[0], r_fv[1]), min(r_fv[2], r_fv[3])));
        }
    }
}

__global__ __launch_bounds__(64) void query_sumk_kernel(const uint64_t *mini_pos, const int64_t *mp_off, int n_q,
                                                        unsigned long long *sumk) {
    for (int q = blockIdx.x; q < n_q; q += gridDim.x) {
        unsigned long long sk = 0;
        const int64_t m1 = mp_off[q + 1];
        for (int64_t m = mp_off[q] + threadIdx.x; m < m1; m += 256) {
            uint64_t v[4];
#pragma unroll
            for (int j = 0; j < 4; j++) v[j] = m + 64 * j < m1 ? mini_pos[m + 64 * j] : 0;
#pragma unroll
            for (int j = 0; j < 4; j++) sk += v[j] >> 32 & 0xff;
        }
        for (int o = 32; o > 0; o >>= 1) sk += __shfl_xor(sk, o, 64);
        if (threadIdx.x == 0) sumk[q] = sk;
    }
}

constexpr int kRegWave = 16;
constexpr int kRegSmall = 256;
constexpr int kRegEntryBytes = 16 + 16 + 4 * 3 + 8;
constexpr int kRegScrStride = 2 * ((kRegEntryBytes + 15) & ~15) - 16;
static_assert(kRegScrStride % 16 == 0 && kRegScrStride >= 2 * kRegEntryBytes, "regions scratch stride");

__device__ __forceinline__ bool wave_query(const RegParams &P, int q, int n, int32_t qlen) {
    return n > P.wave_min && qlen != 0 && !(P.skip_q && P.skip_q[q]);
}

__device__ void regions_seq(const RegParams &P, int q) {
    const int64_t c0 = P.qc[q], c1 = P.qc[q + 1];
    int n = (int)(c1 - c0);
    const int32_t qlen = (int32_t)P.qlen[q];
    if (n == 0 || qlen == 0 || (P.skip_q && P.skip_q[q])) {
        P.n_regs[q] = 0;
        return;
    }
    const int64_t b0 = P.qb[q];
    U128 *z = P.z + c0;
    hymet_mm_reg *r = P.regs + c0;
    uint32_t hash = P.name_hash[q];
    hash ^= wang32((uint32_t)qlen) + wang32((uint32_t)P.seed);
    hash = wang32(hash);
    for (int i = 0; i < n; ++i) {
        const int64_t k = P.cboff[c0 + i] - b0;
        const uint64_t u = P.cu[c0 + i];
        const int64_t a = P.ids[P.cfirst[c0 + i] + (int32_t)u - 1];
        const uint32_t h = (uint32_t)hash64((hash64(P.ax[a]) + hash64((uint64_t)P.span << 32 | P.ay[a])) ^ hash);
        z[i].x = u ^ h;
        z[i].y = (uint64_t)k << 32 | (uint32_t)i;
    }
    heap_sort(z, n, [](const U128 &a, const U128 &b) { return lt128(a, b); });
    for (int i = 0; i < n >> 1; ++i) {
        U128 t = z[i];
        z[i] = z[n - 1 - i];
        z[n - 1 - i] = t;
    }
    for (int i = 0; i < n; ++i) {
        hymet_mm_reg *ri = &r[i];
        ri->id = i;
        ri->parent = -1;
        ri->score = (int32_t)(z[i].x >> 32);
        ri->hash = (uint32_t)z[i].x;
        const int64_t c = c0 + (uint32_t)z[i].y;
        ri->cnt = (int32_t)P.cu[c];
        ri->as = (int32_t)(z[i].y >> 32);
        ri->div = -1.0f;
        ri->subsc = 0;
        ri->n_sub = 0;
        ri->strand_retained = 0;
        ri->mapq = 0;
        ri->pad = (int32_t)(c - c0);
        const int64_t a0 = P.ids[P.cfirst[c] + ri->cnt - 1], a1 = P.ids[P.cfirst[c]];
        set_coor(ri, qlen, P.ax[a0], P.ay[a0], P.ax[a1], P.ay[a1], P.span, P.c_mlen[c], P.c_blen[c]);
    }
    {
        int32_t *w = P.w + c0;
        uint64_t *cov = P.cov + c0;
        for (int i = 0; i < n; ++i) r[i].id = i;
        int i, j, k;
        w[0] = 0, r[0].parent = 0;
        for (i = 1, k = 1; i < n; ++i) {
            hymet_mm_reg *ri = &r[i];
            const int si = ri->qs, ei = ri->qe;
            int n_cov = 0, uncov_len = 0;
            for (j = 0; j < k; ++j) {
                const hymet_mm_reg *rp = &r[w[j]];
                int sj = rp->qs, ej = rp->qe;
                if (ej <= si || sj >= ei) continue;
                if (sj < si) sj = si;
                if (ej > ei) ej = ei;
                cov[n_cov++] = (uint64_t)(uint32_t)sj << 32 | (uint32_t)ej;
            }
            if (n_cov == 0) goto set_parent_test;
            {
                int x = si;
                heap_sort(cov, n_cov, [](uint64_t a, uint64_t b) { return a < b; });
                for (int jj = 0; jj < n_cov; ++jj) {
                    if ((int)(cov[jj] >> 32) > x) uncov_len += (int)(cov[jj] >> 32) - x;
                    x = (int32_t)cov[jj] > x ? (int32_t)cov[jj] : x;
                }
                if (ei > x) uncov_len += ei - x;
            }
            for (j = 0; j < k; ++j) {
                hymet_mm_reg *rp = &r[w[j]];
                const int sj = rp->qs, ej = rp->qe;
                if (ej <= si || sj >= ei) continue;
                const int mn = ej - sj < ei - si ? ej - sj : ei - si;
                const int mx = ej - sj > ei - si ? ej - sj : ei - si;
                const int ol = si < sj ? (ei < sj ? 0 : ei < ej ? ei - sj : ej - sj) : (ej < si ? 0 : ej < ei ? ej - si : ei - si);
                if (__fsub_rn(__fdiv_rn((float)ol, (float)mn), __fdiv_rn((float)uncov_len, (float)mx)) > P.mask_level &&
                    uncov_len <= P.mask_len) {
                    const int sci = ri->score;
                    ri->parent = rp->parent;
                    rp->subsc = rp->subsc > sci ? rp->subsc : sci;
                    if (ri->cnt >= rp->cnt) ++rp->n_sub;
                    break;
                }
            }
        set_parent_test:
            if (j == k) w[k++] = i, ri->parent = i, ri->n_sub = 0;
        }
    }
    {
        const int min_diff = P.k * 2;
        const int min_strand_sc = (int)(P.max_gap * 0.8);
        int i, k, n_2nd = 0;
        for (i = k = 0; i < n; ++i) {
            const int p = r[i].parent;
            if (p == i) {
                r[k++] = r[i];
            } else if (((float)r[i].score >= __fmul_rn((float)r[p].score, P.pri_ratio) || r[i].score + min_diff >= r[p].score) &&
                       n_2nd < P.best_n) {
                if (!(r[i].qs == r[p].qs && r[i].qe == r[p].qe && r[i].rid == r[p].rid && r[i].rs == r[p].rs && r[i].re == r[p].re))
                    r[k++] = r[i], ++n_2nd;
            } else if (n_2nd < P.best_n && r[i].score > min_strand_sc && r[i].rev != r[p].rev) {
                r[i].strand_retained = 1;
                r[k++] = r[i], ++n_2nd;
            }
        }
        if (k != n) {
            int32_t *tmp = P.tmp + c0;
            int max_id = -1;
            for (i = 0; i < k; ++i) max_id = max_id > r[i].id ? max_id : r[i].id;
            for (i = 0; i <= max_id; ++i) tmp[i] = -1;
            for (i = 0; i < k; ++i)
                if (r[i].id >= 0) tmp[r[i].id] = i;
            for (i = 0; i < k; ++i) {
                r[i].id = i;
                if (r[i].parent >= 0 && tmp[r[i].parent] >= 0) r[i].parent = tmp[r[i].parent];
                else r[i].parent = -1;
            }
        }
        n = k;
    }
    {
        const int64_t m0 = P.mp_off[q];
        const int32_t nm = (int32_t)(P.mp_off[q + 1] - m0);
        if (nm > 0) {
            const uint64_t sum_k = P.q_sumk[q];
            const float avg_k = __fdiv_rn((float)sum_k, (float)nm);
            for (int i = 0; i < n; ++i) {
                hymet_mm_reg *ri = &r[i];
                ri->div = -1.0f;
                if (ri->cnt == 0) continue;
                const int64_t c = c0 + ri->pad;
                const int32_t st = P.c_st[c];
                if (st < 0) continue;
                const int32_t fv = P.c_fv[c] < ri->cnt ? P.c_fv[c] : ri->cnt;
                const int32_t n_match = fv;
                const int32_t en = fv == ri->cnt ? P.c_last[c] : nm - 1;
                const int32_t l_ref = (int32_t)P.ref_len[ri->rid];
                int32_t n_tot = en - st + 1;
                if ((float)ri->qs > avg_k && (float)ri->rs > avg_k) ++n_tot;
                if ((float)(qlen - ri->qe) > avg_k && (float)(l_ref - ri->re) > avg_k) ++n_tot;
                ri->div = n_match >= n_tot ? 0.0f : (float)(1.0 - pow((double)n_match / n_tot, 1.0 / (double)avg_k));
            }
        }
    }
    {
        int i, k;
        for (i = k = 0; i < n; ++i) {
            const int p = r[i].parent;
            if (!r[i].strand_retained || r[i].div < __fmul_rn(r[p].div, 5.0f) || r[i].div < 0.01f) {
                if (k < i) r[k++] = r[i];
                else ++k;
            }
        }
        n = k;
    }
    {
        const float q_coef = 40.0f;
        int64_t sum_sc = 0;
        for (int i = 0; i < n; ++i)
            if (r[i].parent == r[i].id) sum_sc += r[i].score;
        const float uniq_ratio = __fdiv_rn((float)sum_sc, (float)(sum_sc + P.rep_len[q]));
        for (int i = 0; i < n; ++i) {
            hymet_mm_reg *ri = &r[i];
            ri->pad = 0;
            if (ri->parent == ri->id) {
                const float pen_s1 = __fmul_rn(ri->score > 100 ? 1.0f : __fmul_rn(0.01f, (float)ri->score), uniq_ratio);
                float pen_cm = ri->cnt > 10 ? 1.0f : __fmul_rn(0.1f, (float)ri->cnt);
                pen_cm = pen_s1 < pen_cm ? pen_s1 : pen_cm;
                const int subsc = ri->subsc > P.min_chain_score ? ri->subsc : P.min_chain_score;
                const float x = __fdiv_rn((float)subsc, (float)ri->score);
                int mapq = (int)__fmul_rn(__fmul_rn(__fmul_rn(pen_cm, q_coef), __fsub_rn(1.0f, x)), logf((float)ri->score));
                mapq -= (int)__fadd_rn(__fmul_rn(4.343f, logf((float)(ri->n_sub + 1))), .499f);
                mapq = mapq > 0 ? mapq : 0;
                ri->mapq = mapq < 60 ? mapq : 60;
            } else
                ri->mapq = 0;
        }
    }
    P.n_regs[q] = n;
}

__device__ __forceinline__ void list_append(bool pred, int q, int32_t *list, int32_t *cnt) {
    const uint64_t m = __ballot(pred);
    if (!m) return;
    const int lane = threadIdx.x & 63, leader = __ffsll((unsigned long long)m) - 1;
    int base = 0;
    if (lane == leader) base = atomicAdd(cnt, __popcll(m));
    base = __shfl(base, leader, 64);
    if (pred) list[base + __popcll(m & ((1ull << lane) - 1))] = q;
}

__global__ __launch_bounds__(64) void regions_kernel(RegParams P, int32_t *big, int32_t *n_big) {
    const int q = blockIdx.x * blockDim.x + threadIdx.x;
    const int n = q < P.n_q ? (int)(P.qc[q + 1] - P.qc[q]) : 0;
    const bool wq = q < P.n_q && wave_query(P, q, n, (int32_t)P.qlen[q]);
    list_append(wq, q, big, n_big);
    if (q >= P.n_q || wq) return;
    regions_seq(P, q);
}

__device__ __forceinline__ void wsync() { __syncthreads(); }

__device__ __forceinline__ uint64_t shfl_xor64(uint64_t v, int m) {
    const int lo = __shfl_xor((int)(uint32_t)v, m, 64), hi = __shfl_xor((int)(uint32_t)(v >> 32), m, 64);
    return (uint64_t)(uint32_t)hi << 32 | (uint32_t)lo;
}
__device__ __forceinline__ uint64_t wave_sort_u64(uint64_t v) {
    const int lane = threadIdx.x;
#pragma unroll
    for (int s = 2; s <= 64; s <<= 1)
#pragma unroll
        for (int d = s >> 1; d > 0; d >>= 1) {
            const uint64_t o = shfl_xor64(v, d);
            const bool up = (lane & s) == 0, low = (lane & d) == 0;
            v = (low == up) ? (o < v ? o : v) : (o > v ? o : v);
        }
    return v;
}
__device__ __forceinline__ int wave_excl_max(int v, int init) {
    const int lane = threadIdx.x;
    int x = __shfl_up(v, 1, 64);
    if (lane == 0) x = init;
#pragma unroll
    for (int d = 1; d < 64; d <<= 1) {
        const int o = __shfl_up(x, d, 64);
        if (lane >= d) x = max(x, o);
    }
    return x;
}
__device__ __forceinline__ int wave_max_i(int v) {
#pragma unroll
    for (int d = 32; d > 0; d >>= 1) v = max(v, __shfl_xor(v, d, 64));
    return v;
}
__device__ __forceinline__ int wave_sum_i(int v) {
#pragma unroll
    for (int d = 32; d > 0; d >>= 1) v += __shfl_xor(v, d, 64);
    return v;
}
__device__ __forceinline__ int64_t wave_sum_l(int64_t v) {
#pragma unroll
    for (int d = 32; d > 0; d >>= 1) v += __shfl_xor(v, d, 64);
    return v;
}
constexpr int kSortU = 4;
__device__ __forceinline__ int bitonic_lo(int t, int d) { return (t / d) * 2 * d + (t % d); }
__device__ void lds_sort_desc(U128 *a, int m) {
    const int half = m >> 1;
    for (int s = 2; s <= m; s <<= 1)
        for (int d = s >> 1; d > 0; d >>= 1) {
            for (int t0 = threadIdx.x; t0 < half; t0 += 64 * kSortU) {
                U128 x[kSortU], y[kSortU];
#pragma unroll
                for (int u = 0; u < kSortU; u++) {
                    const int t = t0 + 64 * u, i = bitonic_lo(t < half ? t : 0, d);
                    x[u] = a[i], y[u] = a[i + d];
                }
#pragma unroll
                for (int u = 0; u < kSortU; u++) {
                    const int t = t0 + 64 * u, i = bitonic_lo(t < half ? t : 0, d);
                    if (t < half && (((i & s) == 0) ? lt128(x[u], y[u]) : lt128(y[u], x[u]))) a[i] = y[u], a[i + d] = x[u];
                }
            }
            wsync();
        }
}
__device__ void lds_sort_asc_u64(uint64_t *a, int m) {
    const int half = m >> 1;
    for (int s = 2; s <= m; s <<= 1)
        for (int d = s >> 1; d > 0; d >>= 1) {
            for (int t0 = threadIdx.x; t0 < half; t0 += 64 * kSortU) {
                uint64_t x[kSortU], y[kSortU];
#pragma unroll
                for (int u = 0; u < kSortU; u++) {
                    const int t = t0 + 64 * u, i = bitonic_lo(t < half ? t : 0, d);
                    x[u] = a[i], y[u] = a[i + d];
                }
#pragma unroll
                for (int u = 0; u < kSortU; u++) {
                    const int t = t0 + 64 * u, i = bitonic_lo(t < half ? t : 0, d);
                    if (t < half && (((i & s) == 0) ? y[u] < x[u] : x[u] < y[u])) a[i] = y[u], a[i + d] = x[u];
                }
            }
            wsync();
        }
}

__device__ __forceinline__ void regions_wave(const RegParams &P, int q, unsigned char *rsm, int cap);

__global__ __launch_bounds__(64) void regions_wave_kernel(RegParams P, const int32_t *big, int32_t *n_big, int64_t *mail,
                                                          unsigned char *gscratch) {
    extern __shared__ __attribute__((aligned(16))) unsigned char rsm[];
    const int nb = __builtin_amdgcn_readfirstlane(*n_big);
    for (int w = blockIdx.x; w < nb; w += gridDim.x) {
        const int q = __builtin_amdgcn_readfirstlane(big[w]);
        const int n = (int)(P.qc[q + 1] - P.qc[q]);
        if (n <= P.lds_max) {
            regions_wave(P, q, rsm, kRegSmall);
        } else {
            int m = 64;
            while (m < n) m <<= 1;
            regions_wave(P, q, gscratch + (size_t)P.qc[q] * kRegScrStride, m);
        }
        __threadfence_block();
        wsync();
    }
    publish_counters(n_big, 1, mail);
}

__device__ __forceinline__ void regions_wave(const RegParams &P, int q, unsigned char *rsm, const int CAP) {
    const int lane = threadIdx.x;
    uint64_t rp_t = P.prof ? clock64() : 0;
#define RPROF(k)                                                                       \
    if (P.prof) {                                                                      \
        const uint64_t rp_n = clock64();                                               \
        if ((k) > 0) atomicAdd(P.prof + (k) - 1, lane == 0 ? (unsigned long long)(rp_n - rp_t) : 0ull); \
        rp_t = rp_n;                                                                   \
    }
    const int64_t c0 = P.qc[q], c1 = P.qc[q + 1];
    int n = (int)(c1 - c0);
    const int32_t qlen = (int32_t)P.qlen[q];
    U128 *zs = reinterpret_cast<U128 *>(rsm);
    int4 *slot = reinterpret_cast<int4 *>(rsm);
    int4 *aux = reinterpret_cast<int4 *>(rsm + 16 * CAP);
    int32_t *wl = reinterpret_cast<int32_t *>(rsm + 32 * CAP);
    int32_t *psub = wl + CAP, *pns = psub + CAP;
    uint64_t *covb = reinterpret_cast<uint64_t *>(pns + CAP);
    const int64_t b0 = P.qb[q];
    hymet_mm_reg *r = P.regs + c0;
    uint32_t hash = P.name_hash[q];
    hash ^= wang32((uint32_t)qlen) + wang32((uint32_t)P.seed);
    hash = wang32(hash);
    RPROF(0);
    int m = 64;
    while (m < n) m <<= 1;
    for (int i = lane; i < m; i += 64) {
        U128 zz{0, 0};
        if (i < n) {
            const int64_t k = P.cboff[c0 + i] - b0;
            const uint64_t u = P.cu[c0 + i];
            const int64_t a = P.ids[P.cfirst[c0 + i] + (int32_t)u - 1];
            const uint32_t h = (uint32_t)hash64((hash64(P.ax[a]) + hash64((uint64_t)P.span << 32 | P.ay[a])) ^ hash);
            zz.x = u ^ h;
            zz.y = (uint64_t)k << 32 | (uint32_t)i;
        }
        zs[i] = zz;
    }
    wsync();
    RPROF(1);
    lds_sort_desc(zs, m);
    for (int i = lane; i < n; i += 64) {
        const U128 zi = zs[i];
        hymet_mm_reg ri;
        ri.id = i;
        ri.parent = -1;
        ri.score = (int32_t)(zi.x >> 32);
        ri.hash = (uint32_t)zi.x;
        const int64_t c = c0 + (uint32_t)zi.y;
        ri.cnt = (int32_t)P.cu[c];
        ri.as = (int32_t)(zi.y >> 32);
        ri.div = -1.0f;
        ri.subsc = 0;
        ri.n_sub = 0;
        ri.strand_retained = 0;
        ri.mapq = 0;
        ri.pad = (int32_t)(c - c0);
        const int64_t a0 = P.ids[P.cfirst[c] + ri.cnt - 1], a1 = P.ids[P.cfirst[c]];
        set_coor(&ri, qlen, P.ax[a0], P.ay[a0], P.ax[a1], P.ay[a1], P.span, P.c_mlen[c], P.c_blen[c]);
        r[i] = ri;
        slot[i] = make_int4(ri.qs, ri.qe, ri.score, ri.cnt);
        aux[i] = make_int4(ri.rid | ri.rev << 31, ri.rs, ri.re, 0);
    }
    wsync();
    RPROF(2);
    {
        const int R = P.prim_regs;
        int ps = 0, pe = 0, pc = 0, pw = 0, psb = 0, pnb = 0;
        if (lane == 0) {
            const int4 s0 = slot[0];
            ps = s0.x, pe = s0.y, pc = s0.w;
            r[0].parent = 0;
            if (R == 0) wl[0] = 0, psub[0] = 0, pns[0] = 0;
        }
        if (R == 0) wsync();
        int k = 1;
        int4 my = make_int4(0, 0, 0, 0);
        for (int i = 1; i < n; ++i) {
            if (i == 1 || (i & 63) == 0) my = slot[min((i & ~63) + lane, n - 1)];
            const int li = i & 63;
            const int si = __builtin_amdgcn_readlane(my.x, li), ei = __builtin_amdgcn_readlane(my.y, li);
            const int sci = __builtin_amdgcn_readlane(my.z, li), cnti = __builtin_amdgcn_readlane(my.w, li);
            int jfound = -1;
            if (k <= R) {
                const bool ov = lane < k && !(pe <= si || ps >= ei);
                const uint64_t mov = __ballot(ov);
                if (mov) {
                    const uint64_t kvl = ov ? (uint64_t)(uint32_t)max(ps, si) << 32 | (uint32_t)min(pe, ei) : ~0ull;
                    const int ncov = __popcll(mov);
                    int uncov = 0, carry = si;
                    if (ncov == 1) {
                        const int l1 = __ffsll((unsigned long long)mov) - 1;
                        const int s_ = (int)__builtin_amdgcn_readlane((int)(kvl >> 32), l1);
                        const int e_ = (int)__builtin_amdgcn_readlane((int)(uint32_t)kvl, l1);
                        uncov = s_ > si ? s_ - si : 0;
                        carry = max(si, e_);
                    } else {
                        const uint64_t kv = wave_sort_u64(kvl);
                        const int s_ = (int)(kv >> 32), e_ = lane < ncov ? (int)(uint32_t)kv : INT32_MIN;
                        const int x = wave_excl_max(e_, si);
                        uncov = wave_sum_i(lane < ncov && s_ > x ? s_ - x : 0);
                        carry = max(si, wave_max_i(e_));
                    }
                    if (ei > carry) uncov += ei - carry;
                    bool hit = false;
                    if (ov) {
                        const int sj = ps, ej = pe;
                        const int mn = ej - sj < ei - si ? ej - sj : ei - si;
                        const int mx = ej - sj > ei - si ? ej - sj : ei - si;
                        const int ol = si < sj ? (ei < sj ? 0 : ei < ej ? ei - sj : ej - sj)
                                               : (ej < si ? 0 : ej < ei ? ej - si : ei - si);
                        hit = __fsub_rn(__fdiv_rn((float)ol, (float)mn), __fdiv_rn((float)uncov, (float)mx)) > P.mask_level &&
                              uncov <= P.mask_len;
                    }
                    const uint64_t mh = __ballot(hit);
                    if (mh) jfound = __ffsll((unsigned long long)mh) - 1;
                }
            } else {
                int ncov = 0;
                for (int jb = 0; jb < k; jb += 64) {
                    const int j = jb + lane;
                    int sj = ps, ej = pe;
                    if (j >= R) {
                        sj = 0, ej = 0;
                        if (j < k) {
                            const int4 o = slot[wl[j]];
                            sj = o.x, ej = o.y;
                        }
                    }
                    const bool ov = j < k && !(ej <= si || sj >= ei);
                    const uint64_t mov = __ballot(ov);
                    if (ov) covb[ncov + __popcll(mov & ((1ull << lane) - 1))] = (uint64_t)(uint32_t)max(sj, si) << 32 | (uint32_t)min(ej, ei);
                    ncov += __popcll(mov);
                }
                wsync();
                if (ncov > 0) {
                    int uncov = 0, carry = si;
                    if (ncov == 1) {
                        const uint64_t kv = covb[0];
                        const int s_ = (int)(kv >> 32), e_ = (int)(uint32_t)kv;
                        uncov = s_ > si ? s_ - si : 0;
                        carry = max(si, e_);
                    } else if (ncov <= 64) {
                        const uint64_t kv = wave_sort_u64(lane < ncov ? covb[lane] : ~0ull);
                        const int s_ = (int)(kv >> 32), e_ = lane < ncov ? (int)(uint32_t)kv : INT32_MIN;
                        const int x = wave_excl_max(e_, si);
                        uncov = wave_sum_i(lane < ncov && s_ > x ? s_ - x : 0);
                        carry = max(si, wave_max_i(e_));
                    } else {
                        int mm = 64;
                        while (mm < ncov) mm <<= 1;
                        for (int t = ncov + lane; t < mm; t += 64) covb[t] = ~0ull;
                        wsync();
                        lds_sort_asc_u64(covb, mm);
                        for (int tb = 0; tb < ncov; tb += 64) {
                            const int t = tb + lane;
                            const uint64_t kv = t < ncov ? covb[t] : ~0ull;
                            const int s_ = (int)(kv >> 32), e_ = t < ncov ? (int)(uint32_t)kv : INT32_MIN;
                            const int x = wave_excl_max(e_, carry);
                            uncov += wave_sum_i(t < ncov && s_ > x ? s_ - x : 0);
                            carry = max(carry, wave_max_i(e_));
                        }
                    }
                    if (ei > carry) uncov += ei - carry;
                    for (int jb = 0; jb < k && jfound < 0; jb += 64) {
                        const int j = jb + lane;
                        bool hit = false;
                        int sj = ps, ej = pe;
                        bool in = true;
                        if (j >= R) {
                            in = j < k;
                            if (in) {
                                const int4 o = slot[wl[j]];
                                sj = o.x, ej = o.y;
                            }
                        }
                        if (in && !(ej <= si || sj >= ei)) {
                            const int mn = ej - sj < ei - si ? ej - sj : ei - si;
                            const int mx = ej - sj > ei - si ? ej - sj : ei - si;
                            const int ol = si < sj ? (ei < sj ? 0 : ei < ej ? ei - sj : ej - sj)
                                                   : (ej < si ? 0 : ej < ei ? ej - si : ei - si);
                            hit = __fsub_rn(__fdiv_rn((float)ol, (float)mn), __fdiv_rn((float)uncov, (float)mx)) > P.mask_level &&
                                  uncov <= P.mask_len;
                        }
                        const uint64_t mh = __ballot(hit);
                        if (mh) jfound = jb + __ffsll((unsigned long long)mh) - 1;
                    }
                }
            }
            if (jfound >= 0) {
                if (jfound < R) {
                    const int p = __builtin_amdgcn_readlane(pw, jfound);
                    if (lane == 0) r[i].parent = p;
                    if (lane == jfound) {
                        psb = psb > sci ? psb : sci;
                        if (cnti >= pc) ++pnb;
                    }
                } else {
                    const int p = wl[jfound];
                    if (lane == 0) {
                        r[i].parent = p;
                        psub[jfound] = psub[jfound] > sci ? psub[jfound] : sci;
                        if (cnti >= slot[p].w) ++pns[jfound];
                    }
                    wsync();
                }
            } else {
                if (k < R) {
                    if (lane == k) ps = si, pe = ei, pc = cnti, pw = i, psb = 0, pnb = 0;
                } else {
                    if (lane == 0) wl[k] = i, psub[k] = 0, pns[k] = 0;
                }
                if (lane == 0) r[i].parent = i;
                ++k;
                if (k > R) wsync();
            }
        }
        if (lane < k && lane < R) {
            r[pw].subsc = psb;
            r[pw].n_sub = pnb;
        }
        for (int j = R + lane; j < k; j += 64) {
            r[wl[j]].subsc = psub[j];
            r[wl[j]].n_sub = pns[j];
        }
    }
    __threadfence_block();
    wsync();
    RPROF(3);
    int nk = 0;
    {
        const int min_diff = P.k * 2;
        const int min_strand_sc = (int)(P.max_gap * 0.8);
        int n_2nd = 0;
        int32_t *kept = wl;
        uint64_t *sflag = covb;
        for (int t = lane; t < (n + 63) / 64; t += 64) sflag[t] = 0;
        wsync();
        for (int base = 0; base < n; base += 64) {
            const int i = base + lane;
            const int pl = i < n ? r[i].parent : 0;
            uint64_t keepm = 0, strm = 0;
            const int cnt_chunk = min(64, n - base);
            for (int l = 0; l < cnt_chunk; ++l) {
                const int ii = base + l, p = __builtin_amdgcn_readlane(pl, l);
                bool keep = false, str = false;
                if (p == ii) {
                    keep = true;
                } else {
                    const int src = nk > p ? kept[p] : p;
                    const int4 mi = slot[ii], xi = aux[ii], mp = slot[src], xp = aux[src];
                    if (((float)mi.z >= __fmul_rn((float)mp.z, P.pri_ratio) || mi.z + min_diff >= mp.z) && n_2nd < P.best_n) {
                        if (!(mi.x == mp.x && mi.y == mp.y && (xi.x & 0x7fffffff) == (xp.x & 0x7fffffff) && xi.y == xp.y &&
                              xi.z == xp.z))
                            keep = true, ++n_2nd;
                    } else if (n_2nd < P.best_n && mi.z > min_strand_sc && ((uint32_t)xi.x >> 31) != ((uint32_t)xp.x >> 31)) {
                        keep = str = true, ++n_2nd;
                    }
                }
                if (keep) {
                    if (lane == 0) kept[nk] = ii;
                    keepm |= 1ull << l;
                    ++nk;
                }
                if (str) strm |= 1ull << l;
                wsync();
            }
            if (lane == 0) sflag[base >> 6] = strm;
            wsync();
        }
        if (nk != n) {
            for (int ob = 0; ob < nk; ob += 64) {
                const int o = ob + lane;
                hymet_mm_reg v;
                if (o < nk) {
                    const int src = kept[o];
                    v = r[src];
                    if (sflag[src >> 6] >> (src & 63) & 1) v.strand_retained = 1;
                }
                __threadfence_block();
                wsync();
                if (o < nk) r[o] = v;
                __threadfence_block();
                wsync();
            }
            int32_t *pos_of = psub;
            for (int j = lane; j < n; j += 64) pos_of[j] = -1;
            wsync();
            for (int o = lane; o < nk; o += 64) pos_of[kept[o]] = o;
            wsync();
            for (int o = lane; o < nk; o += 64) {
                const int par = r[o].parent;
                r[o].id = o;
                r[o].parent = par >= 0 && pos_of[par] >= 0 ? pos_of[par] : -1;
            }
        } else {
            for (int o = lane; o < n; o += 64)
                if (sflag[o >> 6] >> (o & 63) & 1) r[o].strand_retained = 1;
        }
        n = nk;
    }
    __threadfence_block();
    wsync();
    RPROF(4);
    {
        const int64_t m0 = P.mp_off[q];
        const int32_t nm = (int32_t)(P.mp_off[q + 1] - m0);
        if (nm > 0) {
            const uint64_t sum_k = P.q_sumk[q];
            const float avg_k = __fdiv_rn((float)sum_k, (float)nm);
            for (int i = lane; i < n; i += 64) {
                hymet_mm_reg *ri = &r[i];
                float div = -1.0f;
                if (ri->cnt != 0) {
                    const int64_t c = c0 + ri->pad;
                    const int32_t st = P.c_st[c];
                    if (st >= 0) {
                        const int32_t fv = P.c_fv[c] < ri->cnt ? P.c_fv[c] : ri->cnt;
                        const int32_t n_match = fv;
                        const int32_t en = fv == ri->cnt ? P.c_last[c] : nm - 1;
                        const int32_t l_ref = (int32_t)P.ref_len[ri->rid];
                        int32_t n_tot = en - st + 1;
                        if ((float)ri->qs > avg_k && (float)ri->rs > avg_k) ++n_tot;
                        if ((float)(qlen - ri->qe) > avg_k && (float)(l_ref - ri->re) > avg_k) ++n_tot;
                        div = n_match >= n_tot ? 0.0f : (float)(1.0 - pow((double)n_match / n_tot, 1.0 / (double)avg_k));
                    }
                }
                ri->div = div;
            }
        }
    }
    __threadfence_block();
    wsync();
    RPROF(5);
    {
        int first_drop = n;
        for (int base = 0; base < n && first_drop == n; base += 64) {
            const int i = base + lane;
            bool drop = false;
            if (i < n && r[i].strand_retained) {
                const int p = r[i].parent;
                drop = !(r[i].div < __fmul_rn(r[p].div, 5.0f) || r[i].div < 0.01f);
            }
            const uint64_t md = __ballot(drop);
            if (md) first_drop = base + __ffsll((unsigned long long)md) - 1;
        }
        if (first_drop < n) {
            if (lane == 0) {
                int i, k = first_drop;
                for (i = first_drop + 1; i < n; ++i) {
                    const int p = r[i].parent;
                    if (!r[i].strand_retained || r[i].div < __fmul_rn(r[p].div, 5.0f) || r[i].div < 0.01f) r[k++] = r[i];
                }
                psub[0] = k;
            }
            __threadfence_block();
            wsync();
            n = psub[0];
        }
    }
    __threadfence_block();
    wsync();
    {
        const float q_coef = 40.0f;
        int64_t sum_sc = 0;
        for (int i = lane; i < n; i += 64)
            if (r[i].parent == r[i].id) sum_sc += r[i].score;
        sum_sc = wave_sum_l(sum_sc);
        const float uniq_ratio = __fdiv_rn((float)sum_sc, (float)(sum_sc + P.rep_len[q]));
        for (int i = lane; i < n; i += 64) {
            hymet_mm_reg *ri = &r[i];
            ri->pad = 0;
            if (ri->parent == ri->id) {
                const float pen_s1 = __fmul_rn(ri->score > 100 ? 1.0f : __fmul_rn(0.01f, (float)ri->score), uniq_ratio);
                float pen_cm = ri->cnt > 10 ? 1.0f : __fmul_rn(0.1f, (float)ri->cnt);
                pen_cm = pen_s1 < pen_cm ? pen_s1 : pen_cm;
                const int subsc = ri->subsc > P.min_chain_score ? ri->subsc : P.min_chain_score;
                const float x = __fdiv_rn((float)subsc, (float)ri->score);
                int mapq = (int)__fmul_rn(__fmul_rn(__fmul_rn(pen_cm, q_coef), __fsub_rn(1.0f, x)), logf((float)ri->score));
                mapq -= (int)__fadd_rn(__fmul_rn(4.343f, logf((float)(ri->n_sub + 1))), .499f);
                mapq = mapq > 0 ? mapq : 0;
                ri->mapq = mapq < 60 ? mapq : 60;
            } else
                ri->mapq = 0;
        }
    }
    RPROF(6);
    if (P.prof) {
        atomicAdd(P.prof + 6, lane == 0 ? 1ull : 0ull);
        atomicAdd(P.prof + 7, lane == 0 ? (unsigned long long)(c1 - c0) : 0ull);
    }
#undef RPROF
    if (lane == 0) P.n_regs[q] = n;
}

__global__ void chain_stats_init_kernel(int32_t *c_mlen, int32_t *c_blen, int32_t *c_fv, int64_t n) {
    const int64_t i = (int64_t)blockIdx.x * blockDim.x + threadIdx.x;
    if (i < n) c_mlen[i] = 0, c_blen[i] = 0, c_fv[i] = 0x7f7f7f7f;
}

}

int launch_regions(hymet_ctx *ctx, const uint64_t *ax, const uint32_t *ay, int span, const int32_t *ids, const int64_t *cfirst,
                   const uint64_t *cu, const int64_t *cboff,
                   const int64_t *qc, const int64_t *qb, const uint64_t *mini_pos, const int64_t *mp_off, const int64_t *qlen,
                   const uint32_t *name_hash, const int32_t *rep_len, const int64_t *ref_len, int n_q, const hymet_mm_opt *o,
                   int k, void *z, hymet_mm_reg *regs, int32_t *w, uint64_t *cov, int32_t *tmp, int32_t *n_regs,
                   int64_t NB, int64_t NC, int64_t NM, const uint32_t *cq,
                   const MiniWord *mtab, const int64_t *qbase, const uint32_t *skip_q, uint64_t *sumk, bool sumk_done) {
    if (n_q <= 0) return HYMET_OK;
    hipStream_t st = ctx->stream;
    DevBuf cst, blk;
    HY_HIP(cst.alloc(4 * 5 * (size_t)(NC + 1), st));
    int32_t *c_mlen = cst.as<int32_t>(), *c_blen = c_mlen + (NC + 1), *c_st = c_blen + (NC + 1), *c_last = c_st + (NC + 1),
            *c_fv = c_last + (NC + 1);
    {
        ProfScope _ps(ctx, "mm_chain_stats", (double)NB * (4.0 + 12.0 + 4.0) + (double)NM * 8.0);
        AnchorStatParams A{ax, cu, ay, span, ids, cfirst, cboff, qb, qlen, mp_off, mini_pos, NB, NC, n_q, cq,
                           c_mlen, c_blen, c_st, c_last, mtab, qbase, skip_q};
        if (NB > 0) {
            hipLaunchKernelGGL(chain_stats_init_kernel, dim3((unsigned)cdiv(NC + 1, 256)), dim3(256), 0, st, c_mlen, c_blen,
                               c_fv, NC + 1);
            HY_CHECK_LAUNCH("chain_stats_init_kernel");
            HY_HIP(blk.alloc(4 * (size_t)(cdiv(NB, kStatSpan) + 1), st));
            hipLaunchKernelGGL(block_chain_kernel, dim3((unsigned)cdiv(NC, 256)), dim3(256), 0, st, cboff, NC, NB,
                               blk.as<int32_t>());
            HY_CHECK_LAUNCH("block_chain_kernel");
            hipLaunchKernelGGL(chain_stats_flat_kernel, dim3((unsigned)cdiv(NB, kStatSpan)), dim3(256), 0, st, A,
                               (const int32_t *)blk.as<int32_t>(), c_fv);
            HY_CHECK_LAUNCH("chain_stats_flat_kernel");
        }
        if (!sumk_done) {
            const int nqb = n_q < ctx->n_cu * 64 ? n_q : ctx->n_cu * 64;
            hipLaunchKernelGGL(query_sumk_kernel, dim3((unsigned)nqb), dim3(64), 0, st, mini_pos, mp_off, n_q,
                               (unsigned long long *)sumk);
            HY_CHECK_LAUNCH("query_sumk_kernel");
        }
    }
    RegParams P{ax, ay, span, ids, cfirst, cu, cboff, qc, qb, mini_pos, mp_off, qlen, name_hash, rep_len, ref_len, n_q, o->seed, k,
                o->mask_level, o->pri_ratio, o->mask_len, o->best_n, o->max_gap, o->min_chain_score, (U128 *)z, regs, w, cov,
                tmp, n_regs, c_mlen, c_blen, c_st, c_last, c_fv, sumk, skip_q, kRegWave, kRegSmall, nullptr, 64};
    P.wave_min = (int)env_int("HYMET_REG_WAVE", P.wave_min, 0, INT32_MAX);
    P.lds_max = (int)env_int("HYMET_REG_LDS", P.lds_max, 32, kRegSmall);
    P.prim_regs = (int)env_int("HYMET_REG_PRIM", P.prim_regs, 0, 64);
    ProfScope _ps(ctx, "mm_regions", (double)NC * (8.0 + 8.0 + 4.0 * 5) + (double)n_q * 64.0);
    if (env_flag("HYMET_REG_STATS")) {
        std::vector<int64_t> hq(n_q + 1);
        HY_HIP(hipMemcpyAsync(hq.data(), qc, 8 * (size_t)(n_q + 1), hipMemcpyDeviceToHost, st));
        HY_HIP(hipStreamSynchronize(st));
        int64_t h[8] = {0}, mx = 0, tot = 0, big_tot = 0;
        for (int q = 0; q < n_q; q++) {
            const int64_t c = hq[q + 1] - hq[q];
            const int b = c <= 48 ? 0 : c <= 256 ? 1 : c <= 1024 ? 2 : c <= 2048 ? 3 : c <= 8192 ? 4 : 5;
            h[b]++, mx = c > mx ? c : mx, tot += c;
            if (c > 2048) big_tot += c;
        }
        fprintf(stderr, "[regions] n_q %d anchors %lld chains %lld max %lld | <=48 %lld <=256 %lld <=1k %lld <=2k %lld <=8k %lld >8k %lld (chains in >2k: %lld)\n",
                n_q, (long long)NB, (long long)tot, (long long)mx, (long long)h[0], (long long)h[1], (long long)h[2], (long long)h[3],
                (long long)h[4], (long long)h[5], (long long)big_tot);
    }
    if (env_flag("HYMET_REG_PROF")) {
        HY_HIP(hipMalloc((void **)&P.prof, 8 * 8));
        HY_HIP(hipMemsetAsync(P.prof, 0, 8 * 8, st));
    }
    DevBuf big, gscr;
    HY_HIP(big.alloc(4 * (size_t)n_q, st));
    HY_HIP(gscr.alloc((size_t)kRegScrStride * (size_t)(NC + 1), st));
    int32_t *n_big = ctx->dctr + kCtrRegBig;
    hipLaunchKernelGGL(regions_kernel, dim3((unsigned)cdiv(n_q, 64)), dim3(64), 0, st, P, big.as<int32_t>(), n_big);
    HY_CHECK_LAUNCH("regions_kernel");
    hipLaunchKernelGGL(regions_wave_kernel, dim3((unsigned)std::min<int64_t>(n_q, 12 * (int64_t)ctx->n_cu)), dim3(64),
                       (size_t)kRegSmall * kRegEntryBytes, st, P, (const int32_t *)big.as<int32_t>(), n_big,
                       mb_dev(ctx, kMbRegBig), gscr.as<unsigned char>());
    HY_CHECK_LAUNCH("regions_wave_kernel");
    if (P.prof) {
        unsigned long long h[8];
        HY_HIP(hipMemcpyAsync(h, P.prof, sizeof h, hipMemcpyDeviceToHost, st));
        HY_HIP(hipStreamSynchronize(st));
        fprintf(stderr, "[regprof] queries %llu chains %llu | Mcycles keys %.1f sort+fill %.1f parent %.1f select %.1f est %.1f filter+mapq %.1f\n",
                h[6], h[7], h[0] / 1e6, h[1] / 1e6, h[2] / 1e6, h[3] / 1e6, h[4] / 1e6, h[5] / 1e6);
        (void)hipFree(P.prof);
    }
    return HYMET_OK;
}

}
}
```

hymet_amd/pipeline.py:

```python
from __future__ import annotations

import ctypes
import hashlib
import os
import time
from dataclasses import dataclass, field
from typing import Dict, List, Optional, Sequence

import numpy as np

from . import classify as cls
from . import mapper as mp
from . import screen as scr
from . import select as sel
from ._lib import check, ptr
from .ingest import FastaIndex, QueryShard, shard_bytes
from .msh import SketchDB, read_msh
from .seqio import SeqSet

_c = ctypes
TSV_HEADER = b"Query\tLineage\tTaxonomic Level\tConfidence\r\n"


@dataclass
class Config:
    mash_thresh: str = "0.9"
    cand_max: int = 5000
    dedupe: bool = False
    split_idx: str = "2g"
    index_mini_batch: float = 50e6
    w: int = 10
    k: int = 15
    map_batch_bases: int = 40_000_000
    map_streams: int = 2
    n_input_files: int = 1
    limit: bool = True
    screen_winner: bool = False
    reload_inputs: bool = True


@dataclass
class IndexSet:
    names: List[str]
    lens: np.ndarray
    parts: List[mp.IndexPart]
    part_first: List[int]
    opt: mp.MapOpt
    dev: Dict[str, object] = field(default_factory=dict)


class HostText:

    def __init__(self, buf, n: int):
        self._buf, self.n, self._bytes = buf, int(n), None

    def view(self) -> memoryview:
        if self._bytes is not None:
            return memoryview(self._bytes)
        return memoryview(self._buf)[:self.n]

    def bytes(self) -> bytes:
        if self._bytes is None:
            self._bytes = bytes(memoryview(self._buf)[:self.n])
            self._buf = None
        return self._bytes

    detach = bytes


@dataclass
class RunResult:
    selected: List[str]
    screen_rows: List[List[str]]
    thresholds: List[str]
    tsv: bytes
    n_queries: int
    n_classified: int
    n_paf_lines: int
    paf_text: Optional[object] = None
    screen: Optional[list] = None

    @property
    def paf_bytes(self) -> Optional[bytes]:
        t = self.paf_text
        return t.bytes() if isinstance(t, HostText) else t

    @property
    def paf(self) -> Optional[List[str]]:
        if self.paf_bytes is None:
            return None
        return self.paf_bytes.decode().split("\n")[:-1] if self.paf_bytes else []


class PafAcc:

    def __init__(self, gpu):
        self.gpu = gpu
        h = _c.c_void_p()
        check(gpu.lib.hymet_paf_acc_create(gpu.ctx, _c.byref(h)), "hymet_paf_acc_create")
        self.h = h

    def reset(self):
        check(self.gpu.lib.hymet_paf_acc_reset(self.h), "hymet_paf_acc_reset")

    @property
    def n(self) -> int:
        n = _c.c_int64()
        check(self.gpu.lib.hymet_paf_acc_info(self.h, _c.byref(n), None, None, None, None, None), "hymet_paf_acc_info")
        return n.value

    def columns(self):
        n = self.n
        q, part, t = (np.zeros(max(n, 1), np.int32) for _ in range(3))
        check(self.gpu.lib.hymet_paf_acc_copy(self.gpu.ctx, self.h, q.ctypes.data_as(_c.c_void_p),
                                              part.ctypes.data_as(_c.c_void_p), t.ctypes.data_as(_c.c_void_p)),
              "hymet_paf_acc_copy")
        return q[:n], part[:n], t[:n]

    def close(self):
        if getattr(self, "h", None):
            self.gpu.lib.hymet_paf_acc_destroy(self.h)
            self.h = None

    def __del__(self):
        try:
            self.close()
        except Exception:
            pass


def make_index_set(gpu, names, lens, parts, first) -> IndexSet:
    torch = gpu.torch
    opt = mp.MapOpt.asm10()
    opt.resolve_mid_occ(parts[0])
    ix = IndexSet(list(names), np.asarray(lens, np.int64), list(parts), list(first), opt)
    tb = [n.encode() for n in ix.names]
    toff = np.zeros(len(tb) + 1, np.int64)
    np.cumsum([len(b) for b in tb], out=toff[1:])
    ix.dev = {"tname": torch.frombuffer(bytearray(b"".join(tb) or b"\0"), dtype=torch.uint8).to(gpu.dev),
              "tname_off": torch.from_numpy(toff).to(gpu.dev),
              "tlen": torch.from_numpy(ix.lens.copy()).to(gpu.dev)}
    return ix


def map_shard(gpu, ix: IndexSet, sh: QueryShard, acc: PafAcc) -> int:
    acc.reset()
    starts = np.ascontiguousarray(sh.starts, np.int64)
    lens = np.ascontiguousarray(sh.lengths, np.int64)
    hbase = sh.name_hash.data_ptr()
    for pi, part in enumerate(ix.parts):
        for b0, b1 in sh.batches:
            n = b1 - b0
            if n <= 0:
                continue
            gpu.call("hymet_mm_map_acc", part.h, _c.byref(ix.opt), ptr(sh.mm.w2b), ptr(sh.mm.wmask),
                     _c.c_void_p(starts.ctypes.data + 8 * b0), _c.c_void_p(lens.ctypes.data + 8 * b0),
                     _c.c_void_p(hbase + 4 * b0), n, b0, pi, ix.part_first[pi], acc.h)
    return acc.n


def map_shard_streams(gpus, accs, ix: IndexSet, sh: QueryShard, acc: PafAcc) -> int:
    import threading
    tasks = [(pi, b0, b1) for pi in range(len(ix.parts)) for b0, b1 in sh.batches if b1 > b0]
    segs = [None] * len(tasks)
    errs = []
    starts = np.ascontiguousarray(sh.starts, np.int64)
    lens = np.ascontiguousarray(sh.lengths, np.int64)
    hbase = sh.name_hash.data_ptr()

    def work(w):
        g, a = gpus[w], accs[w]
        try:
            a.reset()
            for ti in range(w, len(tasks), len(gpus)):
                pi, b0, b1 = tasks[ti]
                before = a.n
                g.call("hymet_mm_map_acc", ix.parts[pi].h, _c.byref(ix.opt), ptr(sh.mm.w2b), ptr(sh.mm.wmask),
                       _c.c_void_p(starts.ctypes.data + 8 * b0), _c.c_void_p(lens.ctypes.data + 8 * b0),
                       _c.c_void_p(hbase + 4 * b0), b1 - b0, b0, pi, ix.part_first[pi], a.h)
                segs[ti] = (w, before, a.n)
        except Exception as e:
            errs.append(e)

    th = [threading.Thread(target=work, args=(w,)) for w in range(len(gpus))]
    for t in th:
        t.start()
    for t in th:
        t.join()
    if errs:
        raise errs[0]
    acc.reset()
    g0 = acc.gpu
    for w, b, e in segs:
        g0.call("hymet_paf_acc_append", acc.h, accs[w].h, b, e)
    return acc.n


def _dev_buf(gpu, bufs, key, nbytes):
    b = bufs.get(key)
    if b is None or b.numel() < nbytes:
        bufs.pop(key, None)
        b = gpu.empty(max(int(nbytes), 16), gpu.torch.uint8)
        bufs[key] = b
    return b


_bytes_new = _c.pythonapi.PyBytes_FromStringAndSize
_bytes_new.restype = _c.py_object
_bytes_new.argtypes = [_c.c_void_p, _c.c_ssize_t]


def _to_host(gpu, bufs, key, dev, n, prefix: bytes = b"") -> bytes:
    if n == 0:
        return bytes(prefix)
    m = len(prefix)
    b = _bytes_new(None, int(n) + m)
    addr = _c.cast(_c.c_char_p(b), _c.c_void_p).value
    if m:
        _c.memmove(addr, prefix, m)
    check(gpu.lib.hymet_copy_to_host(gpu.ctx, addr + m, ptr(dev), int(n), 16), "hymet_copy_to_host")
    return b


def emit_paf_bytes(gpu, ix: IndexSet, sh: QueryShard, acc: PafAcc, bufs) -> bytes:
    n = acc.n
    if n == 0:
        return b""
    nb = _c.c_int64()
    cap = 200 * n
    while True:
        out = _dev_buf(gpu, bufs, "paf", cap)
        rc = gpu.lib.hymet_emit_paf(gpu.ctx, acc.h, ptr(sh.qname), ptr(sh.qname_off), ptr(sh.qlen), ptr(ix.dev["tname"]),
                                    ptr(ix.dev["tname_off"]), ptr(ix.dev["tlen"]), ptr(out), cap, _c.byref(nb), None)
        if rc == -3:
            cap = nb.value
            continue
        check(rc, "hymet_emit_paf")
        break
    return _to_host(gpu, bufs, "paf_h", out, nb.value)


def run_beside(loader, main):
    if loader is None:
        return main()
    import threading
    err = []

    def body():
        try:
            loader()
        except BaseException as e:
            err.append(e)
    th = threading.Thread(target=body, name="hymet-inputs")
    th.start()
    try:
        out = main()
    finally:
        th.join()
    if err:
        raise err[0]
    return out


class Pipeline:
    def __init__(self, gpu, dbs: Sequence[SketchDB], ref_lookup, taxonomy, hierarchy, cfg: Config = None, comm=None,
                 variant: int = cls.CAMI):
        """dbs: SketchDB objects (tables built once) or .msh paths (read by the native
        reader and rebuilt into HBM tables on every run when cfg.reload_inputs, as `mash
        screen` reads its DB per call)."""
        self.gpu, self.cfg, self.comm = gpu, cfg or Config(), comm
        self.db_paths = [str(d) for d in dbs] if dbs and all(isinstance(d, (str, os.PathLike)) for d in dbs) else None
        self.dbs = [] if self.db_paths else list(dbs)
        self.tables = [scr.ScreenTable(gpu, db) for db in self.dbs]
        self.ref_lookup = ref_lookup
        self.taxonomy, self.hierarchy, self.variant = taxonomy, hierarchy, variant
        self.timings: Dict[str, float] = {}
        self._pin: Dict[int, object] = {}
        self._load_classifier()
        if self.db_paths:
            self._load_dbs()
        self.index_cache: Dict[str, IndexSet] = {}
        self.opt: Optional[mp.MapOpt] = None
        self.acc = PafAcc(gpu)
        self.map_gpus = [gpu.fork() for _ in range(self.cfg.map_streams)] if self.cfg.map_streams > 1 else []
        self.map_accs = [PafAcc(g) for g in self.map_gpus]
        self._bufs: Dict[str, object] = {}
        self._paf_pin = [None, None]
        self._paf_holders = [None, None]
        self._ran = False

    def _pinned_hashes(self, i, n):
        torch = self.gpu.torch
        b = self._pin.get(i)
        if b is None or b.numel() < n:
            b = torch.empty(int(n), dtype=torch.int64, pin_memory=True)
            self._pin[i] = b
        return b

    def _load_dbs(self):
        self._read_dbs()
        self._build_tables()

    def _read_dbs(self, side=None):
        self.tables, self.dbs = [], []
        t0 = time.perf_counter()
        dbs = []
        shard = (self.rank, self.world) if side is not None and self.world > 1 else None
        for i, p in enumerate(self.db_paths):
            pin = lambda n, i=i: self._pinned_hashes(i, n).numpy().view(np.uint64)[:n]
            if side is None:
                dbs.append(read_msh(p, alloc=pin))
            else:
                with self.gpu.torch.cuda.stream(side.stream):
                    dbs.append(read_msh(p, alloc=pin, upload=(side, lambda n: side.empty(n, side.torch.int64)),
                                        shard=shard, defer_meta=True))
        self.dbs = dbs
        self.timings["msh_read_s"] = time.perf_counter() - t0
        for k in ("open", "meta", "hashes"):
            self.timings[f"msh_{k}_s"] = sum(getattr(db, "load_s", {}).get(k, 0.0) for db in dbs)

    def _build_tables(self, side=None):
        t1 = time.perf_counter()
        if side is None:
            self._finish_meta()
            self.tables = [scr.ScreenTable(self.gpu, db, pinned=self._pin[i]) for i, db in enumerate(self.dbs)]
            self.gpu.sync()
        else:
            with self.gpu.torch.cuda.stream(side.stream):
                self.tables = [scr.ScreenTable(side, db, pinned=self._pin[i]) for i, db in enumerate(self.dbs)]
            self.timings["screen_table_enqueue_s"] = time.perf_counter() - t1
            self._finish_meta()
            side.stream.synchronize()
        self.timings["screen_table_s"] = time.perf_counter() - t1

    def _finish_meta(self):
        for db in self.dbs:
            if getattr(db, "finish_meta", None) is not None:
                db.finish_meta()

    def _read_inputs(self, side=None):
        import threading
        err = []

        def classifier():
            try:
                self._load_classifier(side)
            except BaseException as e:
                err.append(e)
        th = threading.Thread(target=classifier, name="hymet-taxonomy")
        th.start()
        try:
            if self.db_paths:
                self._read_dbs(side)
                if side is not None and self._sliced():
                    if not self._db_gather_main():
                        self._join_slices(side)
                elif side is not None:
                    self._build_tables(side)
        finally:
            self._finish_meta()
            th.join()
        if err:
            raise err[0]

    def _sliced(self):
        return any(getattr(db, "dev_slice", None) is not None for db in self.dbs)

    @staticmethod
    def _db_gather_main() -> bool:
        return os.environ.get("HYMET_DB_GATHER", "loader") == "main"

    def _join_slices(self, side):
        t0 = time.perf_counter()
        with self.comm.owned():
            with self.gpu.torch.cuda.stream(side.stream):
                for i, db in enumerate(self.dbs):
                    if db.dev_slice is not None and db.dev_hashes is not None:
                        self.comm.allgather_slices_(db.dev_hashes, db.dev_slice[2], key=i)
            self.timings["msh_allgather_s"] = time.perf_counter() - t0
            self._build_tables(side)

    def _load_classifier(self, side=None):
        t0 = time.perf_counter()
        try:
            self.classifier = cls.Classifier(self.gpu, self.taxonomy, self.hierarchy, self.variant)
            self.classifier_error = None
        except Exception as e:
            self.classifier, self.classifier_error = None, e
        if self.classifier is not None and side is not None:
            torch = self.gpu.torch
            with torch.cuda.stream(side.stream):
                self.classifier.device_tables(None)
            side.stream.synchronize()
        self.timings["classifier_load_s"] = time.perf_counter() - t0

    def load_inputs(self):
        if self.db_paths:
            self._load_dbs()
        self._load_classifier()

    @property
    def world(self) -> int:
        return self.comm.world if self.comm is not None else 1

    @property
    def rank(self) -> int:
        return self.comm.rank if self.comm is not None else 0

    def ingest(self, queries, defer_base: bool = False) -> QueryShard:
        if isinstance(queries, QueryShard):
            return queries
        d_all = None
        if isinstance(queries, (bytes, bytearray, memoryview)):
            data = bytes(queries)
            if self.world > 1:
                b0, b1 = shard_bytes(data, self.rank, self.world)
                d_rng, fx = self._upload_while(data, b0, b1, lambda: FastaIndex(data, byte_range=(b0, b1)))
                sh = QueryShard.from_fasta(self.gpu, fx, 0, fx.n, self.cfg.map_batch_bases, q_base=0,
                                           d_all=d_rng, d_base=b0)
                sh.fasta, sh.fasta_r0 = fx, 0
                sh.byte_sharded = True
                sh.q_base = None
                if not defer_base:
                    self.shard_base(sh)
                return sh
            if len(data):
                d_all, queries = self._upload_while(data, 0, len(data), lambda: FastaIndex(data))
            else:
                queries = FastaIndex(data)
        if isinstance(queries, FastaIndex):
            r0, r1 = queries.shard(self.rank, self.world)
            sh = QueryShard.from_fasta(self.gpu, queries, r0, r1, self.cfg.map_batch_bases,
                                       d_all=d_all if (r0, r1) == (0, queries.n) else None)
            sh.fasta, sh.fasta_r0 = queries, r0
            return sh
        if isinstance(queries, SeqSet):
            if self.world > 1:
                raise ValueError("multi-rank runs take the FASTA bytes (every rank shards the same input)")
            return QueryShard.from_seqset(self.gpu, queries, 0, self.cfg.map_batch_bases)
        raise TypeError(f"unsupported query input {type(queries)!r}")

    prepare = ingest

    def shard_base(self, sh: QueryShard) -> int:
        if sh.q_base is None:
            counts = self.comm.allgather_np(np.array([sh.n], np.int64), tag="shard_records")
            sh.q_base = int(sum(int(c[0]) for c in counts[:self.rank]))
        return sh.q_base

    def _upload_while(self, data: bytes, b0: int, b1: int, scan):
        import threading
        torch = self.gpu.torch
        d = self.gpu.empty(max(b1 - b0, 1), torch.uint8)
        up_err = []

        def upload():
            try:
                if b1 > b0:
                    src = ctypes.cast(ctypes.c_char_p(data), ctypes.c_void_p).value + b0
                    check(self.gpu.lib.hymet_copy_to_device(self.gpu.ctx, ptr(d), ctypes.c_void_p(src), b1 - b0, 16),
                          "hymet_copy_to_device")
            except BaseException as e:
                up_err.append(e)
        up = threading.Thread(target=upload, name="hymet-upload")
        up.start()
        try:
            out = scan()
        finally:
            up.join()
        if up_err:
            raise up_err[0]
        return d, out

    def screen_select(self, pool):
        t0 = time.perf_counter()
        res = scr.screen(self.gpu, pool, self.dbs, self.tables, self.comm, winner=self.cfg.screen_winner)
        self.last_screen = res
        ph = getattr(self, "phases", None)
        if ph is not None:
            ph["screen_only_s"] = ph.get("screen_only_s", 0.0) + time.perf_counter() - t0
        rows, thr, selections = [], [], []
        for r in res:
            s = sel.sort_gr(sel.sort_unique_k5(r.lines(v_max=0.9)))
            t, top, names = sel.select_threshold(s, self.cfg.mash_thresh, self.cfg.n_input_files)
            rows.append(s)
            thr.append(t)
            selections.append(names)
        selected = sel.union_sorted(*selections)
        if not self.cfg.limit:
            return selected, rows, thr
        scores = sel.best_scores(rows)
        limited = sel.limit(selected, scores, self.cfg.cand_max, self.cfg.dedupe)
        return limited, rows, thr

    def index_for(self, selected: List[str]) -> IndexSet:
        key = hashlib.sha1(("".join(n + "\n" for n in selected)).encode()).hexdigest()
        if key in self.index_cache:
            return self.index_cache[key]
        refs: SeqSet = self.ref_lookup(selected)
        parts_idx = mp.split_parts(refs.lengths, float(mp.parse_num(self.cfg.split_idx)), self.cfg.index_mini_batch)
        parts, first = [], []
        for p in parts_idx:
            sub = refs.subset(p) if len(parts_idx) > 1 else refs
            parts.append(mp.IndexPart(self.gpu, sub, self.cfg.w, self.cfg.k))
            first.append(int(p[0]))
        ix = make_index_set(self.gpu, list(refs.names), refs.lengths, parts, first)
        self.index_cache = {key: ix}
        return ix

    def map_all(self, ix: IndexSet, sh: QueryShard) -> int:
        self.opt = ix.opt
        if self.map_gpus:
            self.gpu.sync()
            return map_shard_streams(self.map_gpus, self.map_accs, ix, sh, self.acc)
        return map_shard(self.gpu, ix, sh, self.acc)

    def classify_rows(self, ix: IndexSet, sh: QueryShard):
        gpu, torch = self.gpu, self.gpu.torch
        tabs = self.classifier.device_tables(ix.names)
        counts = gpu.zeros(max(len(ix.names), 1), torch.int32)
        gpu.call("hymet_acc_ref_counts", self.acc.h, ptr(counts))
        if self.world > 1:
            self.comm.allreduce_sum_(counts)
        n_q = max(sh.n, 1)
        rq, rp, rd, rt = (gpu.zeros(n_q, torch.int32) for _ in range(4))
        rn = gpu.zeros(n_q * 8, torch.int32)
        rc = gpu.zeros(n_q, torch.float64)
        nr = _c.c_int32()
        legacy = self.variant == cls.LEGACY
        gpu.call("hymet_acc_classify", self.acc.h, self.variant, sh.n, ptr(sh.qlen), ptr(counts), ptr(tabs["t_tax"]),
                 ptr(tabs["tax_names"]), ptr(tabs["in_hier"]), ptr(sh.qname) if legacy else None,
                 ptr(sh.qname_off) if legacy else None, ptr(ix.dev["tname"]) if legacy else None,
                 ptr(ix.dev["tname_off"]) if legacy else None, ptr(rq), ptr(rp), ptr(rd), ptr(rn), ptr(rc), ptr(rt),
                 _c.byref(nr))
        R = nr.value
        return {"q": rq[:R], "part": rp[:R], "depth": rd[:R], "names": rn[:R * 8], "conf": rc[:R], "tax": rt[:R]}, R

    def emit_tsv(self, rows, R, qname, qname_off) -> bytes:
        gpu = self.gpu
        tabs = self.classifier.device_tables(None)
        legacy = self.variant == cls.LEGACY
        nb = _c.c_int64()
        cap = max(256 * R, 1 << 16)
        while True:
            out = self._dev_buf("tsv", cap)
            rc = gpu.lib.hymet_emit_tsv(gpu.ctx, self.variant, R, ptr(rows["q"]), ptr(rows["depth"]), ptr(rows["names"]),
                                        ptr(rows["conf"]), ptr(rows["tax"]), ptr(qname), ptr(qname_off), ptr(tabs["label"]),
                                        ptr(tabs["label_off"]), ptr(tabs["taxlin"]) if legacy else None,
                                        ptr(tabs["taxlin_off"]) if legacy else None,
                                        ptr(tabs["taxlvl"]) if legacy else None,
                                        ptr(tabs["taxlvl_off"]) if legacy else None, ptr(out), cap, _c.byref(nb))
            if rc == -3:
                cap = nb.value
                continue
            check(rc, "hymet_emit_tsv")
            break
        return self._to_host("tsv_h", out, nb.value, prefix=TSV_HEADER)

    def emit_paf(self, ix: IndexSet, sh: QueryShard) -> HostText:
        gpu, torch = self.gpu, self.gpu.torch
        if getattr(self, "_paf_copy", None) is not None:
            self._paf_copy.synchronize()
            self._paf_copy = None
        n = self.acc.n
        if n == 0:
            return HostText(b"", 0)
        nb = _c.c_int64()
        cap = 200 * n
        while True:
            out = self._dev_buf("paf", cap)
            rc = gpu.lib.hymet_emit_paf(gpu.ctx, self.acc.h, ptr(sh.qname), ptr(sh.qname_off), ptr(sh.qlen),
                                        ptr(ix.dev["tname"]), ptr(ix.dev["tname_off"]), ptr(ix.dev["tlen"]), ptr(out), cap,
                                        _c.byref(nb), None)
            if rc == -3:
                cap = nb.value
                continue
            check(rc, "hymet_emit_paf")
            break
        m = nb.value
        slot = self._paf_slot = (getattr(self, "_paf_slot", 1) + 1) % 2
        holder = self._paf_holders[slot]() if self._paf_holders[slot] is not None else None
        if holder is not None:
            holder.detach()
        buf = self._paf_pin[slot]
        if buf is None or buf.numel() < m:
            for s_ in (slot, 1 - slot):
                b_ = self._paf_pin[s_]
                if b_ is None or b_.numel() < m:
                    h_ = self._paf_holders[s_]() if self._paf_holders[s_] is not None else None
                    if h_ is not None:
                        h_.detach()
                    self._paf_pin[s_] = None
                    self._paf_pin[s_] = torch.empty(int(m * 1.25) + 4096, dtype=torch.uint8, pin_memory=True)
            buf = self._paf_pin[slot]
        if self.map_gpus:
            side = self.map_gpus[0].stream
            ev = torch.cuda.Event()
            ev.record(gpu.bound_stream)
            side.wait_event(ev)
            with torch.cuda.stream(side):
                buf[:m].copy_(out[:m], non_blocking=True)
            self._paf_copy = side
        else:
            gpu.sync()
            buf[:m].copy_(out[:m])
        t = HostText(buf.numpy(), m)
        import weakref
        self._paf_holders[slot] = weakref.ref(t)
        return t

    def _dev_buf(self, key, nbytes):
        return _dev_buf(self.gpu, self._bufs, key, nbytes)

    def _to_host(self, key, dev, n, prefix: bytes = b"") -> bytes:
        return _to_host(self.gpu, self._bufs, key, dev, n, prefix)

    def run(self, queries, with_paf=False) -> RunResult:
        side = self.map_gpus[0] if self.map_gpus else None
        reader = self.cfg.reload_inputs and self._ran
        self._ran = True
        ph = self.phases = {}
        tp = [time.perf_counter()]

        def lap(name):
            t = time.perf_counter()
            ph[name] = ph.get(name, 0.0) + t - tp[0]
            tp[0] = t

        def read():
            t0 = time.perf_counter()
            try:
                self._read_inputs(side)
            finally:
                self.timings["reader_s"] = time.perf_counter() - t0

        def ingest():
            sh_ = self.ingest(queries, defer_base=True)
            lap("ingest_s")
            return sh_
        sh = run_beside(read if reader else None, ingest)
        lap("input_wait_s")
        if getattr(sh, "byte_sharded", False):
            self.shard_base(sh)
        if reader and self.db_paths and side is None:
            self._build_tables()
        elif reader and side is not None and not self.tables and self._sliced():
            self._join_slices(side)
            lap("db_join_s")
        selected, rows, thr = self.screen_select(sh.mash)
        if not selected:
            raise RuntimeError("candidate list empty after applying limit")
        lap("screen_select_s")
        ix = self.index_for(selected)
        n_lines = self.map_all(ix, sh)
        lap("map_s")
        paf_text = self.emit_paf(ix, sh) if with_paf else None
        lap("emit_paf_s")
        tsv, n_rows, n_cls = b"", 0, 0
        if self.classifier is not None:
            rws, R = self.classify_rows(ix, sh)
            lap("classify_s")
            if self.world > 1:
                rws, R = self.comm.gather_rows(rws, sh.q_base, self.gpu)
                qname, qname_off = self._global_names(sh)
            else:
                qname, qname_off = sh.qname, sh.qname_off
            lap("gather_rows_s")
            if self.rank == 0:
                tsv = self.emit_tsv(rws, R, qname, qname_off)
                n_rows = R
                n_cls = int((rws["depth"] != 0).sum().item()) if R else 0
            lap("emit_tsv_s")
        total_rows = self.comm.broadcast_obj(n_rows) if self.world > 1 else n_rows
        if total_rows < 1:
            tsv = self._fallback(ix, sh)
            n_rows = n_cls = 0
        if getattr(self, "_paf_copy", None) is not None:
            self._paf_copy.synchronize()
            self._paf_copy = None
        lap("finish_s")
        return RunResult(selected, rows, thr, tsv, n_rows, n_cls, n_lines, paf_text, self.last_screen)

    def _global_names(self, sh: QueryShard):
        fx = sh.fasta
        if getattr(sh, "byte_sharded", False):
            return self.comm.gather_name_pools(sh.qname, sh.qname_off, sh.n)
        if self._bufs.get("names_of") is not fx:
            torch = self.gpu.torch
            pool, off = fx.name_pool()
            self._bufs["names"] = (torch.from_numpy(pool.copy() if len(pool) else np.zeros(1, np.uint8)).to(self.gpu.dev),
                                   torch.from_numpy(off).to(self.gpu.dev))
            self._bufs["names_of"] = fx
        return self._bufs["names"]

    def _fallback(self, ix: IndexSet, sh: QueryShard) -> bytes:
        from . import fallback
        q, part, t = self.acc.columns()
        if sh.names_host is not None:
            names = sh.names_host
        else:
            names = sh.fasta.names()[sh.fasta_r0:sh.fasta_r0 + sh.n]
        pairs = [(names[int(a)], ix.names[int(b)]) for a, b in zip(q, t)]
        if self.world > 1:
            got = self.comm.gather_obj([(int(p_), sh.q_base + int(a), j, pa[0], pa[1])
                                        for j, (p_, a, pa) in enumerate(zip(part, q, pairs))])
            if self.rank != 0:
                return b""
            pairs = [(x[3], x[4]) for x in sorted(y for g in got for y in g)]
        tsv = fallback.fallback_tsv(pairs, self.taxonomy)
        if tsv.count(b"\n") < 2:
            raise RuntimeError("classification still empty after fallback")
        return tsv
```

include/hymet_gpu.h:

```cpp
#ifndef HYMET_GPU_H
#define HYMET_GPU_H

#include <stdint.h>

#ifdef __cplusplus
extern "C" {
#endif

#define HYMET_OK 0
#define HYMET_E_HIP (-1)
#define HYMET_E_ARG (-2)
#define HYMET_E_CAPACITY (-3)
#define HYMET_E_INTERNAL (-4)

typedef struct hymet_ctx hymet_ctx;

int hymet_init(int device, hymet_ctx **out);
int hymet_destroy(hymet_ctx *ctx);
const char *hymet_last_error(void);
int hymet_set_stream(hymet_ctx *ctx, void *hip_stream);
int hymet_sync(hymet_ctx *ctx);
int hymet_version(void);
int hymet_prof_enable(hymet_ctx *ctx, int on);
int hymet_prof_reset(hymet_ctx *ctx);
int hymet_prof_query(hymet_ctx *ctx, const char *name, double *total_ms, int64_t *count, double *alg_bytes);
int hymet_prof_names(hymet_ctx *ctx, char *buf, int64_t cap);
int hymet_scratch_trim(hymet_ctx *ctx, int64_t *freed_bytes);
int hymet_scratch_cached(hymet_ctx *ctx, int64_t *bytes);
int hymet_scratch_reserve(hymet_ctx *ctx, int64_t bytes);
int hymet_set_oom_hook(void (*hook)(void *user), void *user);
int hymet_scratch_stats(hymet_ctx *ctx, int64_t *counts);
int hymet_copy_to_host(hymet_ctx *ctx, void *dst, const void *src, int64_t n, int threads);
int hymet_copy_to_device(hymet_ctx *ctx, void *dst, const void *src, int64_t n, int threads);

int hymet_pack(hymet_ctx *ctx, const uint8_t *d_ascii, int64_t n, int alphabet,
               uint32_t *d_2b, uint32_t *d_mask);

int hymet_fasta_index(const char *h_buf, int64_t n, int threads, int64_t cap, int64_t *n_rec, int64_t *h_name_off,
                      int32_t *h_name_len, int64_t *h_seq_off, int64_t *h_seq_end, int64_t *h_nbases);
int hymet_fasta_names(const char *h_buf, const int64_t *h_name_off, const int32_t *h_name_len, int64_t n, char *h_pool,
                      int64_t *h_pool_off);
int hymet_fasta_compact(hymet_ctx *ctx, const uint8_t *d_raw, int64_t raw_len, int64_t raw_base, const int64_t *h_seq_off,
                        const int64_t *h_seq_end, const int64_t *h_nbases, int64_t n_rec, uint8_t *d_pool,
                        int64_t pool_len, int64_t *d_pool_start);
int hymet_name_hash(hymet_ctx *ctx, const uint8_t *d_raw, const int64_t *d_name_off, const int32_t *d_name_len, int64_t n,
                    uint32_t *d_hash);

int64_t hymet_screen_table_slots(int64_t n_hashes);
int hymet_screen_table_build(hymet_ctx *ctx, const uint64_t *d_hashes, int64_t n_hashes,
                             uint64_t *d_table, int64_t n_slots, int64_t *d_scratch, int32_t *d_canon_of,
                             int key_bits);
int hymet_sort_pairs_u64(hymet_ctx *ctx, uint64_t *d_keys, uint32_t *d_vals, int64_t n, int begin_bit, int end_bit);

int hymet_scan_u32(hymet_ctx *ctx, const uint32_t *d_in, int64_t *d_out, int64_t n, int mode, int64_t *total);

typedef struct hymet_msh hymet_msh;
typedef struct {
    int32_t k, window_size, sketch_size;
    uint32_t seed;
    int32_t noncanonical, preserve_case, use64;
    int64_t n_refs, n_hashes, names_bytes, comments_bytes, alphabet_len;
} hymet_msh_info;
int hymet_msh_open(const char *path, hymet_msh **out);
int hymet_msh_info_get(const hymet_msh *m, hymet_msh_info *info);
int hymet_msh_copy(const hymet_msh *m, int threads, uint64_t *hashes, int64_t *offsets, int64_t *lengths,
                   char *names, char *comments, char *alphabet);
int hymet_msh_text_offsets(const hymet_msh *m, int64_t *name_start, int64_t *comment_start);
int hymet_msh_upload(hymet_ctx *ctx, const hymet_msh *m, int threads, uint64_t *pinned, uint64_t *d_hashes,
                     int n_chunks);
int hymet_msh_upload_range(hymet_ctx *ctx, const hymet_msh *m, int threads, uint64_t *pinned, uint64_t *d_hashes,
                           int n_chunks, int64_t lo_h, int64_t hi_h);
void hymet_msh_close(hymet_msh *m);
int hymet_screen_count(hymet_ctx *ctx, const uint32_t *d_2b, const uint32_t *d_mask,
                       int64_t n_bases, int64_t pos_begin, int64_t pos_end, int k, uint32_t seed,
                       int ndb, const uint64_t *const *h_d_tables, const int64_t *h_n_slots,
                       const uint64_t *const *h_d_hashes, const int64_t *h_n_hashes,
                       uint32_t *const *h_d_counts, uint64_t cand_thr, uint64_t *d_cand,
                       int64_t cand_cap, unsigned long long *d_cand_n,
                       unsigned long long *d_nkmers);
int hymet_screen_stats(hymet_ctx *ctx, const int64_t *d_ref_off, int64_t n_refs,
                       const int32_t *d_canon_of, const uint32_t *d_counts, uint32_t *d_shared,
                       uint32_t *d_median);
int hymet_screen_winner(hymet_ctx *ctx, const int64_t *d_ref_off, int64_t n_refs,
                        const int32_t *d_canon_of, const uint32_t *d_counts, int64_t n_hashes,
                        const int32_t *d_comp, int64_t n_comp, uint32_t *d_win, uint32_t *d_shared,
                        uint32_t *d_median);

int64_t hymet_sketch_max_size(void);
int hymet_sketch_batch(hymet_ctx *ctx, const uint32_t *d_2b, const uint32_t *d_mask, int64_t n_bases,
                       int k, uint32_t seed, int32_t s, int64_t n_chunks, const int32_t *h_chunk_sketch,
                       const int64_t *h_chunk_begin, const int64_t *h_chunk_end, int32_t n_sketches,
                       uint64_t *d_out, int32_t *d_out_n);

int hymet_mash_dist(hymet_ctx *ctx, const uint64_t *d_ref_hashes, int64_t n_ref_hashes, const int64_t *d_ref_off,
                    int64_t n_ref, const uint64_t *d_qry_hashes, int64_t n_qry_hashes, const int64_t *d_qry_off,
                    int64_t n_qry, int64_t q_begin, int64_t q_end, int32_t s, uint32_t *d_out);
int hymet_mash_dist_tile(int32_t s);
int hymet_mash_dist_tune(int path, int tq);
int hymet_mash_dist_select(hymet_ctx *ctx, const uint32_t *d_block, int64_t n_rows, int64_t n_ref,
                           const uint16_t *d_min_common, int32_t s, int64_t *d_row_off, int32_t *d_ref_idx,
                           uint32_t *d_val, int64_t cap, int64_t *total);
int hymet_mash_dist_tri(hymet_ctx *ctx, const uint64_t *d_hashes, int64_t n_hashes, const int64_t *d_off, int64_t n,
                        int64_t q_begin, int64_t q_end, int32_t s, uint32_t *d_out);
int hymet_mash_link(hymet_ctx *ctx, const uint32_t *d_block, int64_t n_rows, int64_t n, int64_t q_begin,
                    const uint16_t *d_min_common, int32_t s, int32_t *d_parent, uint64_t *d_n_links);
int hymet_mash_labels(hymet_ctx *ctx, int32_t *d_parent, int64_t n, int32_t *d_label);
typedef struct hymet_sparse_counters {
    int64_t postings, emitted, candidates;
} hymet_sparse_counters;
int hymet_mash_dist_sparse(hymet_ctx *ctx, const uint64_t *d_ref_hashes, int64_t n_ref_hashes, const int64_t *d_ref_off,
                           int64_t n_ref, const uint64_t *d_qry_hashes, int64_t n_qry_hashes, const int64_t *d_qry_off,
                           int64_t n_qry, int64_t q_begin, int64_t q_end, int32_t s, int tri,
                           const uint16_t *d_min_common, int32_t cmin, int64_t max_pairs, int64_t *d_row_off,
                           int32_t *d_ref_idx, uint32_t *d_val, int64_t cap, int64_t *total,
                           hymet_sparse_counters *counters);
int hymet_mash_link_edges(hymet_ctx *ctx, const int64_t *d_row_off, int64_t n_rows, int64_t q_begin,
                          const int32_t *d_ref_idx, int32_t *d_parent, uint64_t *d_n_links);

typedef struct hymet_mm_index hymet_mm_index;
int hymet_mm_sketch(hymet_ctx *ctx, const uint32_t *d_2b, const uint32_t *d_mask, const int64_t *h_starts,
                    const int64_t *h_lens, int32_t n_seq, int w, int k, int rid_mode, uint64_t *h_x,
                    uint64_t *h_y, int64_t cap, int64_t *n_out);
int hymet_mm_index_build(hymet_ctx *ctx, const uint32_t *d_2b, const uint32_t *d_mask, const int64_t *h_starts,
                         const int64_t *h_lens, int32_t n_seq, int w, int k, hymet_mm_index **out);
int hymet_mm_index_destroy(hymet_mm_index *idx);
int hymet_mm_index_info(const hymet_mm_index *idx, int32_t *w, int32_t *k, int32_t *n_seq, int64_t *n_pos);
int hymet_mm_index_max_occ(hymet_ctx *ctx, const hymet_mm_index *idx, float frac, int32_t *out);
int hymet_mm_index_save(hymet_ctx *ctx, const hymet_mm_index *idx, const char *path, int append, int64_t *end_offset);
int hymet_mm_index_load(hymet_ctx *ctx, const char *path, int64_t offset, hymet_mm_index **out, int64_t *end_offset);
int hymet_mm_index_export(hymet_ctx *ctx, const hymet_mm_index *idx, uint32_t *h_hash, uint64_t *h_pos);

typedef struct {
    int32_t mid_occ;
    float q_occ_frac;
    int32_t max_max_occ, occ_dist;
    int32_t min_cnt, min_chain_score;
    int32_t bw, bw_long, max_gap, max_chain_skip;
    int32_t rmq_inner_dist, rmq_size_cap, rmq_rescue_size;
    float rmq_rescue_ratio;
    float chain_gap_scale, chain_skip_scale;
    float mask_level, pri_ratio;
    int32_t mask_len, best_n, a, b, seed;
} hymet_mm_opt;

typedef struct {
    int32_t qs, qe, rs, re, rid, rev;
    int32_t mlen, blen, mapq, cnt, score, subsc, parent, id, n_sub, strand_retained;
    float div;
    int32_t as;
    uint32_t hash;
    int32_t pad;
} hymet_mm_reg;

typedef struct hymet_mm_result hymet_mm_result;
int hymet_mm_map(hymet_ctx *ctx, const hymet_mm_index *idx, const hymet_mm_opt *opt,
                 const uint32_t *d_2b, const uint32_t *d_mask, const int64_t *h_starts,
                 const int64_t *h_lens, const uint32_t *h_name_hash, int32_t n_q,
                 hymet_mm_result **out);
int hymet_mm_result_size(const hymet_mm_result *res, int64_t *n_regs);
int hymet_mm_result_copy(const hymet_mm_result *res, int64_t *h_off, int32_t *h_rep_len,
                         hymet_mm_reg *h_regs);
int hymet_mm_result_destroy(hymet_mm_result *res);
typedef struct hymet_paf_acc hymet_paf_acc;
int hymet_paf_acc_create(hymet_ctx *ctx, hymet_paf_acc **out);
int hymet_paf_acc_reset(hymet_paf_acc *acc);
int hymet_paf_acc_destroy(hymet_paf_acc *acc);
int hymet_paf_acc_info(const hymet_paf_acc *acc, int64_t *n_lines, void **d_regs, void **d_q, void **d_part, void **d_rl,
                       void **d_t);
int hymet_paf_acc_append(hymet_ctx *ctx, hymet_paf_acc *dst, const hymet_paf_acc *src, int64_t begin, int64_t end);
int hymet_paf_acc_copy(hymet_ctx *ctx, const hymet_paf_acc *acc, int32_t *h_q, int32_t *h_part, int32_t *h_t);
int hymet_paf_acc_field(hymet_ctx *ctx, const hymet_paf_acc *acc, int field, int32_t *h_out);
int hymet_mm_map_acc(hymet_ctx *ctx, const hymet_mm_index *idx, const hymet_mm_opt *opt, const uint32_t *d_2b,
                     const uint32_t *d_mask, const int64_t *h_starts, const int64_t *h_lens, const uint32_t *d_name_hash,
                     int32_t n_q, int32_t q_base, int32_t part_id, int32_t t_base, hymet_paf_acc *acc);
int hymet_emit_paf(hymet_ctx *ctx, const hymet_paf_acc *acc, const uint8_t *d_qname, const int64_t *d_qname_off,
                   const int64_t *d_qlen, const uint8_t *d_tname, const int64_t *d_tname_off, const int64_t *d_tlen,
                   char *d_out, int64_t cap, int64_t *n_bytes, int64_t *d_line_off);
int hymet_mm_chain_dp(hymet_ctx *ctx, const uint64_t *h_x, const uint64_t *h_y, int64_t n, int max_dist,
                      int max_dist_inner, int bw, int max_chn_skip, int cap_rmq_size, float pen_gap,
                      float pen_skip, int32_t *h_f, int64_t *h_p);
int hymet_mm_mark_compact(hymet_ctx *ctx, const uint64_t *h_x, const uint64_t *h_y, const int32_t *h_mark, int64_t n,
                          const int64_t *h_qoff, const uint32_t *h_qflag, int32_t n_q, uint64_t *h_ox, uint64_t *h_oy,
                          uint32_t *h_ohb, int64_t *n_kept);
int hymet_mm_stamp_scratch(hymet_ctx *ctx, int64_t *capacity, int64_t *nonzero);
int hymet_mm_anchor_sort(hymet_ctx *ctx, const uint64_t *h_key, const uint32_t *h_val, int64_t n,
                         const int64_t *h_qoff, int32_t n_q, int32_t rb, int32_t pb, uint64_t yhi, int64_t max_qlen,
                         uint64_t *h_ax, uint64_t *h_ay, uint32_t *h_ax32, uint32_t *h_hb, int64_t *h_stats);

int hymet_lca_ref_counts(hymet_ctx *ctx, const int32_t *d_line_t, int64_t n_lines, int32_t *d_counts);
int hymet_acc_ref_counts(hymet_ctx *ctx, const hymet_paf_acc *acc, int32_t *d_counts);
int hymet_acc_classify(hymet_ctx *ctx, const hymet_paf_acc *acc, int mode, int32_t n_q, const int64_t *d_qlen,
                       const int32_t *d_ref_counts, const int32_t *d_t_tax, const int32_t *d_tax_names,
                       const uint8_t *d_tax_in_hier, const uint8_t *d_qname_pool, const int64_t *d_qname_off,
                       const uint8_t *d_tname_pool, const int64_t *d_tname_off, int32_t *d_row_q, int32_t *d_row_part,
                       int32_t *d_row_depth, int32_t *d_row_names, double *d_row_conf, int32_t *d_row_tax,
                       int32_t *n_rows);
int hymet_emit_tsv(hymet_ctx *ctx, int mode, int32_t n_rows, const int32_t *d_row_q, const int32_t *d_row_depth,
                   const int32_t *d_row_names, const double *d_row_conf, const int32_t *d_row_tax, const uint8_t *d_qname,
                   const int64_t *d_qname_off, const uint8_t *d_label, const int64_t *d_label_off, const uint8_t *d_taxlin,
                   const int64_t *d_taxlin_off, const uint8_t *d_taxlvl, const int64_t *d_taxlvl_off, char *d_out,
                   int64_t cap, int64_t *n_bytes);
int hymet_lca(hymet_ctx *ctx, int mode, int32_t n_q, const int64_t *d_q_off, const int32_t *d_line_t,
              const int64_t *d_line_blen, const int64_t *d_line_qlen, const uint8_t *d_line_exact,
              const int32_t *d_ref_counts, const int32_t *d_t_tax, const int32_t *d_tax_names,
              const uint8_t *d_tax_in_hier, int32_t *d_scr_tid, double *d_scr_w, int32_t *d_scr_nm,
              double *d_scr_nw, int32_t *d_out_depth, int32_t *d_out_names, double *d_out_conf,
              int32_t *d_out_tax);

#ifdef __cplusplus
}
#endif
#endif
```

Baseline: 134,200.

## Sketch and filter each query batch once and reuse it across index parts

Adds a prepared query-batch object that holds the minimizer sketch, the filtered minimizers, qid and qbase. Mapping against each index part now reuses this object, so sketching and filtering run once per batch instead of once per (part, batch). The Python pipeline loops batches outer and parts inner, writing into a temporary accumulator that is reordered by (part, batch) afterwards, and multi-stream workers claim whole batches dynamically. This costs an extra accumulator copy pass and a host sync per batch, and it drops the cached sumk kernel path from the region stage.

```diff
diff --git a/hymet_amd/_lib.py b/hymet_amd/_lib.py
--- a/hymet_amd/_lib.py
+++ b/hymet_amd/_lib.py
@@ -80,6 +80,11 @@
     "hymet_paf_acc_copy": (_i32, [_vp, _vp, _vp, _vp, _vp]),
     "hymet_paf_acc_field": (_i32, [_vp, _vp, _i32, _vp]),
     "hymet_mm_map_acc": (_i32, [_vp, _vp, _vp, _vp, _vp, _vp, _vp, _vp, _i32, _i32, _i32, _i32, _vp]),
+    "hymet_mm_qbatch_create": (_i32, [_vp, _vp, _vp, _vp, _vp, _vp, _vp, _i32, _i32, _i32, _i32, _c.c_float, _c.POINTER(_vp)]),
+    "hymet_mm_qbatch_info": (_i32, [_vp, _c.POINTER(_i32), _c.POINTER(_i64), _c.POINTER(_i64)]),
+    "hymet_mm_qbatch_destroy": (_i32, [_vp]),
+    "hymet_mm_map_batch": (_i32, [_vp, _vp, _vp, _vp, _c.POINTER(_vp)]),
+    "hymet_mm_map_acc_batch": (_i32, [_vp, _vp, _vp, _vp, _i32, _i32, _i32, _vp]),
     "hymet_emit_paf": (_i32, [_vp, _vp, _vp, _vp, _vp, _vp, _vp, _vp, _vp, _i64, _c.POINTER(_i64), _vp]),
     "hymet_acc_ref_counts": (_i32, [_vp, _vp, _vp]),
     "hymet_acc_classify": (_i32, [_vp, _vp, _i32, _i32] + [_vp] * 15 + [_c.POINTER(_i32)]),
diff --git a/hymet_amd/csrc/mm_map.hip b/hymet_amd/csrc/mm_map.hip
--- a/hymet_amd/csrc/mm_map.hip
+++ b/hymet_amd/csrc/mm_map.hip
@@ -26,7 +26,7 @@
                    const uint32_t *name_hash, const int32_t *rep_len, const int64_t *ref_len, int n_q, const hymet_mm_opt *o,
                    int k, void *z, hymet_mm_reg *regs, int32_t *w, uint64_t *cov, int32_t *tmp, int32_t *n_regs,
                    int64_t NB, int64_t NC, int64_t NM, const uint32_t *cq,
-                   const MiniWord *mtab, const int64_t *qbase, const uint32_t *skip_q, uint64_t *sumk, bool sumk_done);
+                   const MiniWord *mtab, const int64_t *qbase, const uint32_t *skip_q);
 
 namespace {
 
@@ -586,32 +586,54 @@
     return HYMET_OK;
 }
 
+struct hymet_mm_qbatch {
+    hymet_ctx *ctx = nullptr;
+    hipStream_t stream = nullptr;
+    int device = 0;
+    int32_t n_q = 0;
+    int w = 0, k = 0;
+    int32_t mid_occ = 0;
+    float q_occ_frac = 0.0f;
+    std::vector<int64_t> h_lens;
+    hymet::mm::DevBuf mx, my, qm_off;
+    int64_t M = 0, M_sketch = 0;
+    hymet::mm::DevBuf d_qlen, d_hash_buf;
+    const uint32_t *d_hash = nullptr;
+    hymet::mm::DevBuf qid;
+    hymet::mm::DevBuf d_qbase;
+    std::vector<int64_t> qbase;
+    int64_t max_qlen = 1;
+};
+
 struct MapBatch {
     hymet_ctx *ctx;
     const hymet_mm_index *idx;
     const hymet_mm_opt *opt;
-    const int64_t *h_lens;
     int32_t n_q;
-    DevBuf mx, my, qm_off;
-    int64_t M = 0;
-    DevBuf d_qlen, d_hash_buf;
-    const uint32_t *d_hash = nullptr;
-    DevBuf seed_n, rep_len, qid;
+    const uint64_t *mx, *my;
+    const int64_t *qm_off;
+    int64_t M;
+    const int64_t *d_qlen;
+    const uint32_t *d_hash;
+    const uint32_t *qid;
+    const int64_t *d_qbase;
+    const int64_t *qbase;
+    int64_t max_qlen;
+    DevBuf seed_n, rep_len;
     DevBuf mini_pos, mp_off;
     int64_t NM = 0;
-    DevBuf d_qbase, pos_tab;
-    std::vector<int64_t> qbase;
-    int64_t max_qlen = 1;
+    DevBuf pos_tab;
 };
 
-static int sketch_queries(MapBatch &B, const uint32_t *d_2b, const uint32_t *d_mask, const int64_t *h_starts,
+static int sketch_queries(hymet_mm_qbatch &B, const uint32_t *d_2b, const uint32_t *d_mask, const int64_t *h_starts,
                           const uint32_t *h_name_hash, const uint32_t *d_name_hash) {
     hipStream_t st = B.ctx->stream;
     const int n_q = B.n_q;
-    int rc = sketch_sequences(B.ctx, d_2b, d_mask, h_starts, B.h_lens, n_q, B.idx->w, B.idx->k, 0, B.mx, B.my, &B.M, &B.qm_off);
-    if (rc) return rc;
+    int rc = sketch_sequences(B.ctx, d_2b, d_mask, h_starts, B.h_lens.data(), n_q, B.w, B.k, 0, B.mx, B.my, &B.M, &B.qm_off);
+    if (rc) return rc;
+    B.M_sketch = B.M;
     HY_HIP(B.d_qlen.alloc(8 * (size_t)n_q, st));
-    HY_HIP(hipMemcpyAsync(B.d_qlen.p, B.h_lens, 8 * (size_t)n_q, hipMemcpyHostToDevice, st));
+    HY_HIP(hipMemcpyAsync(B.d_qlen.p, B.h_lens.data(), 8 * (size_t)n_q, hipMemcpyHostToDevice, st));
     B.d_hash = d_name_hash;
     if (!B.d_hash) {
         HY_HIP(B.d_hash_buf.alloc(4 * (size_t)n_q, st));
@@ -621,10 +643,10 @@
     return HYMET_OK;
 }
 
-static int filter_minimizers(MapBatch &B) {
+static int filter_minimizers(hymet_mm_qbatch &B) {
     hymet_ctx *ctx = B.ctx;
     hipStream_t st = ctx->stream;
-    const hymet_mm_opt *opt = B.opt;
+    const hymet_mm_qbatch *opt = &B;
     const int n_q = B.n_q;
     const int64_t M = B.M;
     DevBuf &mx = B.mx, &my = B.my, &qm_off = B.qm_off;
@@ -660,7 +682,7 @@
     LAUNCH1(iota_u32_kernel, MF, sidx.as<uint32_t>(), MF);
     uint64_t *kx = sx.as<uint64_t>(), *kxa = sx2.as<uint64_t>();
     uint32_t *vi = sidx.as<uint32_t>(), *via = sidx2.as<uint32_t>();
-    rc = sort_pairs(ctx, kx, kxa, vi, via, MF, 0, 2 * B.idx->k + 8, "radix_sort_mz");
+    rc = sort_pairs(ctx, kx, kxa, vi, via, MF, 0, 2 * B.k + 8, "radix_sort_mz");
     if (rc) return rc;
     HY_HIP(sq.alloc(4 * (size_t)MF, st));
     HY_HIP(sq2.alloc(4 * (size_t)MF, st));
@@ -698,15 +720,16 @@
     const hymet_mm_opt *opt = B.opt;
     const int n_q = B.n_q;
     const int64_t M = B.M;
-    DevBuf &mx = B.mx, &my = B.my, &qm_off = B.qm_off, &seed_n = B.seed_n, &rep_len = B.rep_len, &qid = B.qid;
+    const uint64_t *mx = B.mx, *my = B.my;
+    const int64_t *qm_off = B.qm_off;
+    const uint32_t *qid = B.qid;
+    DevBuf &seed_n = B.seed_n, &rep_len = B.rep_len;
     HY_HIP(seed_n.alloc(4 * (size_t)(M + 1), st));
     HY_HIP(rep_len.alloc(4 * (size_t)n_q, st));
-    HY_HIP(qid.alloc(4 * (size_t)(M + 1), st));
-    LAUNCH1(fill_qid_kernel, std::max<int64_t>(M, n_q), qm_off.as<int64_t>(), n_q, M, qid.as<uint32_t>(), nullptr,
-            rep_len.as<int32_t>());
+    HY_HIP(hipMemsetAsync(rep_len.p, 0, 4 * (size_t)n_q, st));
     {
         ProfScope _ps(ctx, "mm_seed_count", (double)M * (8.0 + 8.0 + 4.0));
-        LAUNCH1(seed_count_kernel, M, mx.as<uint64_t>(), M, B.idx->d_koff, B.idx->n_buckets, seed_n.as<uint32_t>());
+        LAUNCH1(seed_count_kernel, M, mx, M, B.idx->d_koff, B.idx->n_buckets, seed_n.as<uint32_t>());
     }
     if (M == 0) return HYMET_OK;
     ProfScope _ps(ctx, "mm_seed_select", (double)M * (4.0 + 8.0 + 8.0 + 8.0));
@@ -726,7 +749,7 @@
     HY_HIP(flt_high.alloc(4 * (size_t)n_high, st));
     LAUNCH1(seed_list_kernel, M, seed_n.as<uint32_t>(), rank.as<uint64_t>(), M, opt->mid_occ, low_idx.as<int32_t>(),
             high_idx.as<int32_t>());
-    StreakParams S{my.as<uint64_t>(), qid.as<uint32_t>(), qm_off.as<int64_t>(), B.d_qlen.as<int64_t>(),
+    StreakParams S{my, qid, qm_off, B.d_qlen,
                    rank.as<uint64_t>(), low_idx.as<int32_t>(), high_idx.as<int32_t>(), n_low, n_q, opt->mid_occ,
                    opt->max_max_occ, opt->occ_dist, seed_n.as<uint32_t>(), flt_high.as<uint32_t>()};
     HY_HIP(hipMemsetAsync(flt_high.p, 0, 4 * (size_t)n_high, st));
@@ -740,28 +763,19 @@
         if (rc) return rc;
     }
     LAUNCH1(rep_len_kernel, n_high, flt_high.as<uint32_t>(), pmax.as<int32_t>(), high_idx.as<int32_t>(), n_high,
-            mx.as<uint64_t>(), my.as<uint64_t>(), qid.as<uint32_t>(), rep_len.as<int32_t>(), seed_n.as<uint32_t>());
+            mx, my, qid, rep_len.as<int32_t>(), seed_n.as<uint32_t>());
     return HYMET_OK;
 }
 
 static int build_mini_table(MapBatch &B, const DevBuf &mp_pos) {
     hymet_ctx *ctx = B.ctx;
     hipStream_t st = ctx->stream;
-    const int n_q = B.n_q;
-    B.qbase.assign(n_q + 1, 0);
-    for (int q = 0; q < n_q; q++) {
-        B.qbase[q + 1] = B.qbase[q] + ((B.h_lens[q] + 63) & ~(int64_t)63);
-        B.max_qlen = std::max<int64_t>(B.max_qlen, B.h_lens[q]);
-    }
-    HY_HIP(B.d_qbase.alloc(8 * (size_t)(n_q + 1), st));
-    HY_HIP(hipMemcpyAsync(B.d_qbase.p, B.qbase.data(), 8 * (size_t)(n_q + 1), hipMemcpyHostToDevice, st));
-    const size_t n_words = (size_t)(B.qbase[n_q] >> 6) + 1;
+    const size_t n_words = (size_t)(B.qbase[B.n_q] >> 6) + 1;
     HY_HIP(B.pos_tab.alloc(sizeof(MiniWord) * n_words, st));
     HY_HIP(hipMemsetAsync(B.pos_tab.p, 0, sizeof(MiniWord) * n_words, st));
-    LAUNCH1(mini_bits_kernel, B.M, B.my.as<uint64_t>(), B.seed_n.as<uint32_t>(), B.qid.as<uint32_t>(), B.d_qbase.as<int64_t>(),
-            B.M, B.pos_tab.as<MiniWord>());
-    LAUNCH1(mini_base_kernel, B.M, B.my.as<uint64_t>(), B.seed_n.as<uint32_t>(), B.qid.as<uint32_t>(), B.qm_off.as<int64_t>(),
-            mp_pos.as<int64_t>(), B.d_qbase.as<int64_t>(), B.M, B.pos_tab.as<MiniWord>());
+    LAUNCH1(mini_bits_kernel, B.M, B.my, B.seed_n.as<uint32_t>(), B.qid, B.d_qbase, B.M, B.pos_tab.as<MiniWord>());
+    LAUNCH1(mini_base_kernel, B.M, B.my, B.seed_n.as<uint32_t>(), B.qid, B.qm_off, mp_pos.as<int64_t>(), B.d_qbase, B.M,
+            B.pos_tab.as<MiniWord>());
     return HYMET_OK;
 }
 
@@ -771,7 +785,10 @@
     const hymet_mm_index *idx = B.idx;
     const int n_q = B.n_q;
     const int64_t M = B.M;
-    DevBuf &mx = B.mx, &my = B.my, &qm_off = B.qm_off, &seed_n = B.seed_n, &qid = B.qid, &d_qlen = B.d_qlen;
+    const uint64_t *mx = B.mx, *my = B.my;
+    const int64_t *qm_off = B.qm_off, *d_qlen = B.d_qlen;
+    const uint32_t *qid = B.qid;
+    DevBuf &seed_n = B.seed_n;
     DevBuf a_pos, mflag, mp_pos;
     int64_t A = 0;
     int rc = scan_flags(ctx, seed_n.as<uint32_t>(), M, a_pos, &A);
@@ -786,13 +803,13 @@
     HY_HIP(B.mini_pos.alloc(8 * (size_t)(B.NM + 1), st));
     HY_HIP(B.mp_off.alloc(8 * (size_t)(n_q + 1), st));
     hipLaunchKernelGGL(sample_off_kernel, dim3((unsigned)cdiv(n_q + 1, 256)), dim3(256), 0, st, mp_pos.as<int64_t>(),
-                       qm_off.as<int64_t>(), n_q, B.NM, B.mp_off.as<int64_t>());
+                       qm_off, n_q, B.NM, B.mp_off.as<int64_t>());
     HY_CHECK_LAUNCH("sample_off_kernel");
     rc = build_mini_table(B, mp_pos);
     if (rc) return rc;
     HY_HIP(S1.d_off.alloc(8 * (size_t)(n_q + 1), st));
     hipLaunchKernelGGL(sample_off_kernel, dim3((unsigned)cdiv(n_q + 1, 256)), dim3(256), 0, st, a_pos.as<int64_t>(),
-                       qm_off.as<int64_t>(), n_q, A, S1.d_off.as<int64_t>());
+                       qm_off, n_q, A, S1.d_off.as<int64_t>());
     HY_CHECK_LAUNCH("sample_off_kernel");
     const int rb = bits_for(idx->n_seq), key1_bits = bits_for(n_q) + 1 + rb;
     HY_ARG(key1_bits <= 64, "hymet_mm_map: too many queries x targets for the sort key");
@@ -807,8 +824,8 @@
     if (ybits > 0) {
         DevBuf word;
         HY_HIP(word.alloc(8 * (size_t)(A + 1), st));
-        AnchorKeyParams P{mx.as<uint64_t>(), my.as<uint64_t>(), seed_n.as<uint32_t>(), a_pos.as<int64_t>(),
-                          qid.as<uint32_t>(), d_qlen.as<int64_t>(), idx->d_koff, idx->d_pos, M, rb, pb,
+        AnchorKeyParams P{mx, my, seed_n.as<uint32_t>(), a_pos.as<int64_t>(),
+                          qid, d_qlen, idx->d_koff, idx->d_pos, M, rb, pb,
                           ybits, word.as<uint64_t>(), mp_pos.as<int64_t>(), B.mini_pos.as<uint64_t>()};
         {
             ProfScope _ps(ctx, "mm_anchors", (double)A * (8.0 + 12.0));
@@ -823,8 +840,8 @@
     HY_HIP(k1.alloc(8 * (size_t)(A + 1), st));
     HY_HIP(k2.alloc(8 * (size_t)(A + 1), st));
     HY_HIP(val.alloc(4 * (size_t)(A + 1), st));
-    AnchorParams P{mx.as<uint64_t>(), my.as<uint64_t>(), seed_n.as<uint32_t>(), a_pos.as<int64_t>(), qid.as<uint32_t>(),
-                   d_qlen.as<int64_t>(), idx->d_koff, idx->d_pos, M, rb, x.as<uint64_t>(), k1.as<uint64_t>(),
+    AnchorParams P{mx, my, seed_n.as<uint32_t>(), a_pos.as<int64_t>(), qid,
+                   d_qlen, idx->d_koff, idx->d_pos, M, rb, x.as<uint64_t>(), k1.as<uint64_t>(),
                    k2.as<uint64_t>(), y.as<uint32_t>(), val.as<uint32_t>(), mp_pos.as<int64_t>(), B.mini_pos.as<uint64_t>()};
     ProfScope _ps(ctx, "mm_anchors", (double)A * (8.0 + 36.0));
     LAUNCH1(write_anchors_kernel, M, P);
@@ -852,7 +869,7 @@
     return dump_anchors(ctx, "HYMET_DUMP_ANCHORS2", S2, n_q, dumped);
 }
 
-static int run_regions(MapBatch &B, ChainSet &C, DevBuf &rg, DevBuf &nr, const uint32_t *skip_q, DevBuf &sumk, bool &sumk_done) {
+static int run_regions(MapBatch &B, ChainSet &C, DevBuf &rg, DevBuf &nr, const uint32_t *skip_q) {
     hipStream_t st = B.ctx->stream;
     const int64_t NC = C.n_chain;
     DevBuf z, wv, cov, tmp;
@@ -864,11 +881,10 @@
     HY_HIP(nr.alloc(4 * (size_t)B.n_q, st));
     return launch_regions(B.ctx, C.ax, C.ay, C.span, C.ids.as<int32_t>(), C.cfirst.as<int64_t>(), C.cu.as<uint64_t>(),
                           C.cboff.as<int64_t>(), C.d_qc.as<int64_t>(), C.d_qb.as<int64_t>(), B.mini_pos.as<uint64_t>(),
-                          B.mp_off.as<int64_t>(), B.d_qlen.as<int64_t>(), B.d_hash, B.rep_len.as<int32_t>(), B.idx->d_len,
+                          B.mp_off.as<int64_t>(), B.d_qlen, B.d_hash, B.rep_len.as<int32_t>(), B.idx->d_len,
                           B.n_q, B.opt, B.idx->k, z.p, rg.as<hymet_mm_reg>(), wv.as<int32_t>(), cov.as<uint64_t>(),
                           tmp.as<int32_t>(), nr.as<int32_t>(), C.n_anchor, NC, B.NM, C.cq.as<uint32_t>(),
-                          B.pos_tab.as<MiniWord>(), B.d_qbase.as<int64_t>(), skip_q, sumk.as<uint64_t>(),
-                          std::exchange(sumk_done, true));
+                          B.pos_tab.as<MiniWord>(), B.d_qbase, skip_q);
 }
 
 struct RegSet {
@@ -918,15 +934,71 @@
     return HYMET_OK;
 }
 
-static int mm_map_impl(hymet_ctx *ctx, const hymet_mm_index *idx, const hymet_mm_opt *opt, const uint32_t *d_2b,
-                       const uint32_t *d_mask, const int64_t *h_starts, const int64_t *h_lens, const uint32_t *h_name_hash,
-                       const uint32_t *d_name_hash, int32_t n_q, MapSink &sink) {
-    CallTrace call_trace;
-    HY_ARG(ctx && idx && opt && d_2b && d_mask, "hymet_mm_map: null argument");
-    HY_ARG(n_q >= 0, "hymet_mm_map: n_q < 0");
-    HY_ARG(h_name_hash || d_name_hash, "hymet_mm_map: no query name hashes");
-    HY_ARG(opt->mid_occ > 0, "hymet_mm_map: opt->mid_occ must be resolved (hymet_mm_index_max_occ + clamps)");
+static int qbatch_prepare(hymet_mm_qbatch &Q, const uint32_t *d_2b, const uint32_t *d_mask, const int64_t *h_starts,
+                          const uint32_t *h_name_hash, const uint32_t *d_name_hash) {
+    hymet_ctx *ctx = Q.ctx;
+    hipStream_t st = ctx->stream;
+    const int n_q = Q.n_q;
+    if (n_q == 0) return HYMET_OK;
+    PhaseTrace tr(ctx);
+    int rc = sketch_queries(Q, d_2b, d_mask, h_starts, h_name_hash, d_name_hash);
+    if (rc) return rc;
+    tr.mark("sketch");
+    rc = filter_minimizers(Q);
+    if (rc) return rc;
+    HY_HIP(Q.qid.alloc(4 * (size_t)(Q.M + 1), st));
+    LAUNCH1(fill_qid_kernel, Q.M, Q.qm_off.as<int64_t>(), n_q, Q.M, Q.qid.as<uint32_t>(), nullptr, nullptr);
+    Q.qbase.assign(n_q + 1, 0);
+    for (int q = 0; q < n_q; q++) {
+        Q.qbase[q + 1] = Q.qbase[q] + ((Q.h_lens[q] + 63) & ~(int64_t)63);
+        Q.max_qlen = std::max<int64_t>(Q.max_qlen, Q.h_lens[q]);
+    }
+    HY_HIP(Q.d_qbase.alloc(8 * (size_t)(n_q + 1), st));
+    HY_HIP(hipMemcpyAsync(Q.d_qbase.p, Q.qbase.data(), 8 * (size_t)(n_q + 1), hipMemcpyHostToDevice, st));
+    HY_HIP(hipStreamSynchronize(st));
+    tr.mark("mz_flt");
+    return HYMET_OK;
+}
+
+static int qbatch_create(hymet_ctx *ctx, const uint32_t *d_2b, const uint32_t *d_mask, const int64_t *h_starts,
+                         const int64_t *h_lens, const uint32_t *h_name_hash, const uint32_t *d_name_hash, int32_t n_q, int w,
+                         int k, int32_t mid_occ, float q_occ_frac, hymet_mm_qbatch **out) {
+    HY_ARG(ctx && out, "hymet_mm_qbatch_create: null argument");
+    *out = nullptr;
+    HY_ARG(n_q >= 0, "hymet_mm_qbatch_create: n_q < 0");
+    HY_ARG(n_q == 0 || (d_2b && d_mask && h_starts && h_lens), "hymet_mm_qbatch_create: null argument");
+    HY_ARG(n_q == 0 || h_name_hash || d_name_hash, "hymet_mm_qbatch_create: no query name hashes");
+    HY_ARG(mid_occ > 0, "hymet_mm_qbatch_create: mid_occ must be resolved (hymet_mm_index_max_occ + clamps)");
     HY_HIP(hipSetDevice(ctx->device));
+    hymet_mm_qbatch *Q = new hymet_mm_qbatch();
+    Q->ctx = ctx;
+    Q->stream = ctx->stream;
+    Q->device = ctx->device;
+    Q->n_q = n_q;
+    Q->w = w;
+    Q->k = k;
+    Q->mid_occ = mid_occ;
+    Q->q_occ_frac = q_occ_frac;
+    if (n_q) Q->h_lens.assign(h_lens, h_lens + n_q);
+    const int rc = qbatch_prepare(*Q, d_2b, d_mask, h_starts, h_name_hash, d_name_hash);
+    if (rc) {
+        (void)hipStreamSynchronize(ctx->stream);
+        delete Q;
+        return rc;
+    }
+    *out = Q;
+    return HYMET_OK;
+}
+
+static int map_prepared(hymet_ctx *ctx, const hymet_mm_index *idx, const hymet_mm_opt *opt, const hymet_mm_qbatch *Q,
+                        MapSink &sink) {
+    HY_ARG(ctx && idx && opt && Q, "hymet_mm_map_batch: null argument");
+    HY_ARG(Q->ctx == ctx && Q->stream == ctx->stream, "hymet_mm_map_batch: the batch was prepared by another context");
+    HY_ARG(idx->w == Q->w && idx->k == Q->k, "hymet_mm_map_batch: the batch was prepared with another (w, k) than the index");
+    HY_ARG(opt->mid_occ == Q->mid_occ && opt->q_occ_frac == Q->q_occ_frac,
+           "hymet_mm_map_batch: the batch was prepared with another mid_occ or q_occ_frac than opt's");
+    HY_HIP(hipSetDevice(ctx->device));
+    const int32_t n_q = Q->n_q;
     if (sink.res) {
         sink.res->n_q = n_q;
         sink.res->reg_off.assign(n_q + 1, 0);
@@ -936,14 +1008,10 @@
     const float pen_gap = (float)(opt->chain_gap_scale * 0.01 * idx->k);
     const float pen_skip = (float)(opt->chain_skip_scale * 0.01 * idx->k);
     PhaseTrace tr(ctx);
-    MapBatch B{ctx, idx, opt, h_lens, n_q};
-    int rc = sketch_queries(B, d_2b, d_mask, h_starts, h_name_hash, d_name_hash);
-    if (rc) return rc;
-    tr.mark("sketch");
-    rc = filter_minimizers(B);
-    if (rc) return rc;
-    tr.mark("mz_flt");
-    rc = select_seeds(B);
+    MapBatch B{ctx, idx, opt, n_q, Q->mx.as<uint64_t>(), Q->my.as<uint64_t>(), Q->qm_off.as<int64_t>(), Q->M,
+               Q->d_qlen.as<int64_t>(), Q->d_hash, Q->qid.as<uint32_t>(), Q->d_qbase.as<int64_t>(), Q->qbase.data(),
+               Q->max_qlen};
+    int rc = select_seeds(B);
     if (rc) return rc;
     tr.mark("seeds");
     AnchorSet S1;
@@ -955,7 +1023,7 @@
     if (rc) return rc;
     ChainSet C1;
     const bool long_join = opt->bw_long > opt->bw;
-    LeanJoin lj{B.d_qlen.as<int64_t>(), opt->rmq_rescue_size, opt->rmq_rescue_ratio};
+    LeanJoin lj{B.d_qlen, opt->rmq_rescue_size, opt->rmq_rescue_ratio};
     rc = chain_set(ctx, opt, pen_gap, pen_skip, opt->bw, S1, n_q, C1, long_join ? &lj : nullptr);
     if (rc) return rc;
     tr.mark("chain_set 1");
@@ -973,14 +1041,12 @@
         }
     }
     tr.mark("long join");
-    DevBuf sumk, rg1, nr1, rg2, nr2;
-    HY_HIP(sumk.alloc(8 * (size_t)(n_q + 1), ctx->stream));
-    bool sumk_done = false;
+    DevBuf rg1, nr1, rg2, nr2;
     const uint32_t *fl = joined ? flag.as<uint32_t>() : nullptr;
-    rc = run_regions(B, C1, rg1, nr1, fl, sumk, sumk_done);
+    rc = run_regions(B, C1, rg1, nr1, fl);
     if (rc) return rc;
     if (joined) {
-        rc = run_regions(B, C2, rg2, nr2, nullptr, sumk, sumk_done);
+        rc = run_regions(B, C2, rg2, nr2, nullptr);
         if (rc) return rc;
     }
     const RegSet r1{nr1.as<int32_t>(), C1.d_qc.as<int64_t>(), rg1.as<hymet_mm_reg>()};
@@ -991,7 +1057,73 @@
     return HYMET_OK;
 }
 
+static int mm_map_impl(hymet_ctx *ctx, const hymet_mm_index *idx, const hymet_mm_opt *opt, const uint32_t *d_2b,
+                       const uint32_t *d_mask, const int64_t *h_starts, const int64_t *h_lens, const uint32_t *h_name_hash,
+                       const uint32_t *d_name_hash, int32_t n_q, MapSink &sink) {
+    CallTrace call_trace;
+    HY_ARG(ctx && idx && opt && d_2b && d_mask, "hymet_mm_map: null argument");
+    HY_ARG(n_q >= 0, "hymet_mm_map: n_q < 0");
+    HY_ARG(h_name_hash || d_name_hash, "hymet_mm_map: no query name hashes");
+    HY_ARG(opt->mid_occ > 0, "hymet_mm_map: opt->mid_occ must be resolved (hymet_mm_index_max_occ + clamps)");
+    hymet_mm_qbatch *Q = nullptr;
+    int rc = qbatch_create(ctx, d_2b, d_mask, h_starts, h_lens, h_name_hash, d_name_hash, n_q, idx->w, idx->k, opt->mid_occ,
+                           opt->q_occ_frac, &Q);
+    if (rc) return rc;
+    rc = map_prepared(ctx, idx, opt, Q, sink);
+    if (rc) (void)hipStreamSynchronize(ctx->stream);
+    delete Q;
+    return rc;
+}
+
 extern "C" {
+
+int hymet_mm_qbatch_create(hymet_ctx *ctx, const uint32_t *d_2b, const uint32_t *d_mask, const int64_t *h_starts,
+                           const int64_t *h_lens, const uint32_t *h_name_hash, const uint32_t *d_name_hash, int32_t n_q,
+                           int32_t w, int32_t k, int32_t mid_occ, float q_occ_frac, hymet_mm_qbatch **out) {
+    return qbatch_create(ctx, d_2b, d_mask, h_starts, h_lens, h_name_hash, d_name_hash, n_q, w, k, mid_occ, q_occ_frac, out);
+}
+
+int hymet_mm_qbatch_info(const hymet_mm_qbatch *qb, int32_t *n_q, int64_t *n_minimizers, int64_t *n_filtered) {
+    HY_ARG(qb, "hymet_mm_qbatch_info: null batch");
+    if (n_q) *n_q = qb->n_q;
+    if (n_minimizers) *n_minimizers = qb->M;
+    if (n_filtered) *n_filtered = qb->M_sketch - qb->M;
+    return HYMET_OK;
+}
+
+int hymet_mm_qbatch_destroy(hymet_mm_qbatch *qb) {
+    if (qb) {
+        (void)hipSetDevice(qb->device);
+        delete qb;
+    }
+    return HYMET_OK;
+}
+
+int hymet_mm_map_batch(hymet_ctx *ctx, const hymet_mm_index *idx, const hymet_mm_opt *opt, const hymet_mm_qbatch *qb,
+                       hymet_mm_result **out) {
+    HY_ARG(out != nullptr, "hymet_mm_map_batch: null argument");
+    *out = nullptr;
+    MapSink sink;
+    sink.res = new hymet_mm_result();
+    const int rc = map_prepared(ctx, idx, opt, qb, sink);
+    if (rc) {
+        delete sink.res;
+        return rc;
+    }
+    *out = sink.res;
+    return HYMET_OK;
+}
+
+int hymet_mm_map_acc_batch(hymet_ctx *ctx, const hymet_mm_index *idx, const hymet_mm_opt *opt, const hymet_mm_qbatch *qb,
+                           int32_t q_base, int32_t part_id, int32_t t_base, hymet_paf_acc *acc) {
+    HY_ARG(acc, "hymet_mm_map_acc_batch: null argument");
+    MapSink sink;
+    sink.acc = acc;
+    sink.q_base = q_base;
+    sink.part_id = part_id;
+    sink.t_base = t_base;
+    return map_prepared(ctx, idx, opt, qb, sink);
+}
 
 int hymet_mm_map(hymet_ctx *ctx, const hymet_mm_index *idx, const hymet_mm_opt *opt, const uint32_t *d_2b,
                  const uint32_t *d_mask, const int64_t *h_starts, const int64_t *h_lens, const uint32_t *h_name_hash,
diff --git a/hymet_amd/csrc/mm_regs.hip b/hymet_amd/csrc/mm_regs.hip
--- a/hymet_amd/csrc/mm_regs.hip
+++ b/hymet_amd/csrc/mm_regs.hip
@@ -72,7 +72,6 @@
     int32_t *tmp;
     int32_t *n_regs;
     const int32_t *c_mlen, *c_blen, *c_st, *c_last, *c_fv;
-    const uint64_t *q_sumk;
     const uint32_t *skip_q;
     int wave_min;
     int lds_max;
@@ -300,23 +299,6 @@
     }
 }
 
-__global__ __launch_bounds__(64) void query_sumk_kernel(const uint64_t *mini_pos, const int64_t *mp_off, int n_q,
-                                                        unsigned long long *sumk) {
-    for (int q = blockIdx.x; q < n_q; q += gridDim.x) {
-        unsigned long long sk = 0;
-        const int64_t m1 = mp_off[q + 1];
-        for (int64_t m = mp_off[q] + threadIdx.x; m < m1; m += 256) {
-            uint64_t v[4];
-#pragma unroll
-            for (int j = 0; j < 4; j++) v[j] = m + 64 * j < m1 ? mini_pos[m + 64 * j] : 0;
-#pragma unroll
-            for (int j = 0; j < 4; j++) sk += v[j] >> 32 & 0xff;
-        }
-        for (int o = 32; o > 0; o >>= 1) sk += __shfl_xor(sk, o, 64);
-        if (threadIdx.x == 0) sumk[q] = sk;
-    }
-}
-
 constexpr int kRegWave = 16;
 constexpr int kRegSmall = 256;
 constexpr int kRegEntryBytes = 16 + 16 + 4 * 3 + 8;
@@ -457,7 +439,7 @@
         const int64_t m0 = P.mp_off[q];
         const int32_t nm = (int32_t)(P.mp_off[q + 1] - m0);
         if (nm > 0) {
-            const uint64_t sum_k = P.q_sumk[q];
+            const uint64_t sum_k = (uint64_t)P.span * (uint64_t)(P.mp_off[q + 1] - P.mp_off[q]);
             const float avg_k = __fdiv_rn((float)sum_k, (float)nm);
             for (int i = 0; i < n; ++i) {
                 hymet_mm_reg *ri = &r[i];
@@ -950,7 +932,7 @@
         const int64_t m0 = P.mp_off[q];
         const int32_t nm = (int32_t)(P.mp_off[q + 1] - m0);
         if (nm > 0) {
-            const uint64_t sum_k = P.q_sumk[q];
+            const uint64_t sum_k = (uint64_t)P.span * (uint64_t)(P.mp_off[q + 1] - P.mp_off[q]);
             const float avg_k = __fdiv_rn((float)sum_k, (float)nm);
             for (int i = lane; i < n; i += 64) {
                 hymet_mm_reg *ri = &r[i];
@@ -1050,7 +1032,7 @@
                    const uint32_t *name_hash, const int32_t *rep_len, const int64_t *ref_len, int n_q, const hymet_mm_opt *o,
                    int k, void *z, hymet_mm_reg *regs, int32_t *w, uint64_t *cov, int32_t *tmp, int32_t *n_regs,
                    int64_t NB, int64_t NC, int64_t NM, const uint32_t *cq,
-                   const MiniWord *mtab, const int64_t *qbase, const uint32_t *skip_q, uint64_t *sumk, bool sumk_done) {
+                   const MiniWord *mtab, const int64_t *qbase, const uint32_t *skip_q) {
     if (n_q <= 0) return HYMET_OK;
     hipStream_t st = ctx->stream;
     DevBuf cst, blk;
@@ -1073,16 +1055,10 @@
                                (const int32_t *)blk.as<int32_t>(), c_fv);
             HY_CHECK_LAUNCH("chain_stats_flat_kernel");
         }
-        if (!sumk_done) {
-            const int nqb = n_q < ctx->n_cu * 64 ? n_q : ctx->n_cu * 64;
-            hipLaunchKernelGGL(query_sumk_kernel, dim3((unsigned)nqb), dim3(64), 0, st, mini_pos, mp_off, n_q,
-                               (unsigned long long *)sumk);
-            HY_CHECK_LAUNCH("query_sumk_kernel");
-        }
     }
     RegParams P{ax, ay, span, ids, cfirst, cu, cboff, qc, qb, mini_pos, mp_off, qlen, name_hash, rep_len, ref_len, n_q, o->seed, k,
                 o->mask_level, o->pri_ratio, o->mask_len, o->best_n, o->max_gap, o->min_chain_score, (U128 *)z, regs, w, cov,
-                tmp, n_regs, c_mlen, c_blen, c_st, c_last, c_fv, sumk, skip_q, kRegWave, kRegSmall, nullptr, 64};
+                tmp, n_regs, c_mlen, c_blen, c_st, c_last, c_fv, skip_q, kRegWave, kRegSmall, nullptr, 64};
     P.wave_min = (int)env_int("HYMET_REG_WAVE", P.wave_min, 0, INT32_MAX);
     P.lds_max = (int)env_int("HYMET_REG_LDS", P.lds_max, 32, kRegSmall);
     P.prim_regs = (int)env_int("HYMET_REG_PRIM", P.prim_regs, 0, 64);
diff --git a/hymet_amd/pipeline.py b/hymet_amd/pipeline.py
--- a/hymet_amd/pipeline.py
+++ b/hymet_amd/pipeline.py
@@ -143,42 +143,90 @@
     return ix
 
 
-def map_shard(gpu, ix: IndexSet, sh: QueryShard, acc: PafAcc) -> int:
-    acc.reset()
+def paf_segment_order(segs):
+    return [segs[key] for key in sorted(segs)]
+
+
+class BatchClaims:
+
+    def __init__(self, n_batches: int, n_workers: int):
+        import threading
+        self.n, self.workers = n_batches, max(1, n_workers)
+        self.taken = [False] * n_batches
+        self.lock = threading.Lock()
+
+    def claim(self, w: int):
+        with self.lock:
+            free = [i for i in range(self.n) if not self.taken[i]]
+            if not free:
+                return None
+            own = [i for i in free if i % self.workers == w]
+            i = (own or free)[0]
+            self.taken[i] = True
+            return i
+
+
+def _map_batch(g, a: PafAcc, w: int, ix: IndexSet, sh: QueryShard, starts, lens, bi: int, b0: int, b1: int, segs):
+    qb = _c.c_void_p()
+    opt = ix.opt
+    g.call("hymet_mm_qbatch_create", ptr(sh.mm.w2b), ptr(sh.mm.wmask), _c.c_void_p(starts.ctypes.data + 8 * b0),
+           _c.c_void_p(lens.ctypes.data + 8 * b0), None, _c.c_void_p(sh.name_hash.data_ptr() + 4 * b0), b1 - b0,
+           ix.parts[0].w, ix.parts[0].k, opt.mid_occ, _c.c_float(opt.q_occ_frac), _c.byref(qb))
+    try:
+        after = a.n
+        for pi, part in enumerate(ix.parts):
+            before = after
+            g.call("hymet_mm_map_acc_batch", part.h, _c.byref(opt), qb, b0, pi, ix.part_first[pi], a.h)
+            after = a.n
+            segs[(pi, bi)] = (w, before, after)
+    finally:
+        g.lib.hymet_mm_qbatch_destroy(qb)
+
+
+def map_shard(gpu, ix: IndexSet, sh: QueryShard, acc: PafAcc, tmp: Optional[PafAcc] = None) -> int:
     starts = np.ascontiguousarray(sh.starts, np.int64)
     lens = np.ascontiguousarray(sh.lengths, np.int64)
-    hbase = sh.name_hash.data_ptr()
-    for pi, part in enumerate(ix.parts):
-        for b0, b1 in sh.batches:
-            n = b1 - b0
-            if n <= 0:
-                continue
-            gpu.call("hymet_mm_map_acc", part.h, _c.byref(ix.opt), ptr(sh.mm.w2b), ptr(sh.mm.wmask),
-                     _c.c_void_p(starts.ctypes.data + 8 * b0), _c.c_void_p(lens.ctypes.data + 8 * b0),
-                     _c.c_void_p(hbase + 4 * b0), n, b0, pi, ix.part_first[pi], acc.h)
+    direct = len(ix.parts) <= 1
+    own = None
+    if not direct and tmp is None:
+        tmp = own = PafAcc(gpu)
+    a = acc if direct else tmp
+    try:
+        a.reset()
+        segs = {}
+        for bi, (b0, b1) in enumerate(sh.batches):
+            if b1 > b0:
+                _map_batch(gpu, a, 0, ix, sh, starts, lens, bi, b0, b1, segs)
+        if not direct:
+            acc.reset()
+            for _, b, e in paf_segment_order(segs):
+                gpu.call("hymet_paf_acc_append", acc.h, a.h, b, e)
+    finally:
+        if own is not None:
+            gpu.sync()
+            own.close()
     return acc.n
 
 
 def map_shard_streams(gpus, accs, ix: IndexSet, sh: QueryShard, acc: PafAcc) -> int:
     import threading
-    tasks = [(pi, b0, b1) for pi in range(len(ix.parts)) for b0, b1 in sh.batches if b1 > b0]
-    segs = [None] * len(tasks)
+    batches = [(bi, b0, b1) for bi, (b0, b1) in enumerate(sh.batches) if b1 > b0]
+    segs = {}
     errs = []
     starts = np.ascontiguousarray(sh.starts, np.int64)
     lens = np.ascontiguousarray(sh.lengths, np.int64)
-    hbase = sh.name_hash.data_ptr()
+    claims = BatchClaims(len(batches), len(gpus))
 
     def work(w):
         g, a = gpus[w], accs[w]
         try:
             a.reset()
-            for ti in range(w, len(tasks), len(gpus)):
-                pi, b0, b1 = tasks[ti]
-                before = a.n
-                g.call("hymet_mm_map_acc", ix.parts[pi].h, _c.byref(ix.opt), ptr(sh.mm.w2b), ptr(sh.mm.wmask),
-                       _c.c_void_p(starts.ctypes.data + 8 * b0), _c.c_void_p(lens.ctypes.data + 8 * b0),
-                       _c.c_void_p(hbase + 4 * b0), b1 - b0, b0, pi, ix.part_first[pi], a.h)
-                segs[ti] = (w, before, a.n)
+            while not errs:
+                i = claims.claim(w)
+                if i is None:
+                    break
+                bi, b0, b1 = batches[i]
+                _map_batch(g, a, w, ix, sh, starts, lens, bi, b0, b1, segs)
         except Exception as e:
             errs.append(e)
 
@@ -191,7 +239,7 @@
         raise errs[0]
     acc.reset()
     g0 = acc.gpu
-    for w, b, e in segs:
+    for w, b, e in paf_segment_order(segs):
         g0.call("hymet_paf_acc_append", acc.h, accs[w].h, b, e)
     return acc.n
 
@@ -284,6 +332,7 @@
         self.acc = PafAcc(gpu)
         self.map_gpus = [gpu.fork() for _ in range(self.cfg.map_streams)] if self.cfg.map_streams > 1 else []
         self.map_accs = [PafAcc(g) for g in self.map_gpus]
+        self.map_tmp: Optional[PafAcc] = None
         self._bufs: Dict[str, object] = {}
         self._paf_pin = [None, None]
         self._paf_holders = [None, None]
@@ -513,7 +562,9 @@
         if self.map_gpus:
             self.gpu.sync()
             return map_shard_streams(self.map_gpus, self.map_accs, ix, sh, self.acc)
-        return map_shard(self.gpu, ix, sh, self.acc)
+        if len(ix.parts) > 1 and self.map_tmp is None:
+            self.map_tmp = PafAcc(self.gpu)
+        return map_shard(self.gpu, ix, sh, self.acc, self.map_tmp)
 
     def classify_rows(self, ix: IndexSet, sh: QueryShard):
         gpu, torch = self.gpu, self.gpu.torch
diff --git a/include/hymet_gpu.h b/include/hymet_gpu.h
--- a/include/hymet_gpu.h
+++ b/include/hymet_gpu.h
@@ -173,6 +173,16 @@
 int hymet_mm_map_acc(hymet_ctx *ctx, const hymet_mm_index *idx, const hymet_mm_opt *opt, const uint32_t *d_2b,
                      const uint32_t *d_mask, const int64_t *h_starts, const int64_t *h_lens, const uint32_t *d_name_hash,
                      int32_t n_q, int32_t q_base, int32_t part_id, int32_t t_base, hymet_paf_acc *acc);
+typedef struct hymet_mm_qbatch hymet_mm_qbatch;
+int hymet_mm_qbatch_create(hymet_ctx *ctx, const uint32_t *d_2b, const uint32_t *d_mask, const int64_t *h_starts,
+                           const int64_t *h_lens, const uint32_t *h_name_hash, const uint32_t *d_name_hash, int32_t n_q,
+                           int32_t w, int32_t k, int32_t mid_occ, float q_occ_frac, hymet_mm_qbatch **out);
+int hymet_mm_qbatch_info(const hymet_mm_qbatch *qb, int32_t *n_q, int64_t *n_minimizers, int64_t *n_filtered);
+int hymet_mm_qbatch_destroy(hymet_mm_qbatch *qb);
+int hymet_mm_map_batch(hymet_ctx *ctx, const hymet_mm_index *idx, const hymet_mm_opt *opt, const hymet_mm_qbatch *qb,
+                       hymet_mm_result **out);
+int hymet_mm_map_acc_batch(hymet_ctx *ctx, const hymet_mm_index *idx, const hymet_mm_opt *opt, const hymet_mm_qbatch *qb,
+                           int32_t q_base, int32_t part_id, int32_t t_base, hymet_paf_acc *acc);
 int hymet_emit_paf(hymet_ctx *ctx, const hymet_paf_acc *acc, const uint8_t *d_qname, const int64_t *d_qname_off,
                    const int64_t *d_qlen, const uint8_t *d_tname, const int64_t *d_tname_off, const int64_t *d_tlen,
                    char *d_out, int64_t cap, int64_t *n_bytes, int64_t *d_line_off);
```

New measurement: 137,400, median of 4. 2.4% higher.
